# nolan-h-hamilton/ROCCO

Hardware: AMD Instinct MI355X
Metric: loci/sec to converged solve, hg38 50bp K=100; BED3 intervals bit-exact (higher is better)
Workload: dtype f64

## Files before the change

include/rocco_hip.h:

```cpp
#ifndef ROCCO_HIP_H
#define ROCCO_HIP_H

#include <stddef.h>
#include <stdint.h>

#ifdef __cplusplus
extern "C" {
#endif

#define ROCCO_HIP_OK 0
#define ROCCO_HIP_ENOMEM (-1)
#define ROCCO_HIP_EINVAL (-2)
#define ROCCO_HIP_EHIP (-3)

#define ROCCO_HIP_PATH_CERTIFIED 1
#define ROCCO_HIP_PATH_EXACT 2
#define ROCCO_HIP_PATH_TRIVIAL 3
#define ROCCO_HIP_PATH_SPINE 4

typedef struct rocco_hip_solver rocco_hip_solver;

int rocco_hip_abi_version(void);

const char *rocco_hip_last_error(void);

int rocco_hip_solver_create(rocco_hip_solver **solver_out, int device);
void rocco_hip_solver_destroy(rocco_hip_solver *solver);

int rocco_hip_solver_set(rocco_hip_solver *solver, const char *key, long long value);

int rocco_hip_score_median(rocco_hip_solver *solver, const void *matrix_dev, int dtype, size_t K,
                           size_t n, size_t row_stride, double *scores_dev, void *stream);

int rocco_hip_score_median_batch(rocco_hip_solver *solver, const void *const *matrices_dev, int dtype, size_t K,
                                 const size_t *n, const size_t *row_strides, double *const *scores_dev, size_t count,
                                 void *stream);

int rocco_hip_score_median_batch_stats(rocco_hip_solver *solver, const void *const *matrices_dev, int dtype, size_t K,
                                       const size_t *n, const size_t *row_strides, double *const *scores_dev,
                                       size_t count, double *stats_dev, void *stream);

int rocco_hip_score_order_statistic(rocco_hip_solver *solver, const void *matrix_dev, int dtype, size_t K, size_t n,
                                    size_t row_stride, int rank, double *scores_dev, void *stream);
int rocco_hip_score_mean(rocco_hip_solver *solver, const void *matrix_dev, int dtype, size_t K, size_t n,
                         size_t row_stride, double *scores_dev, void *stream);

int rocco_hip_score_trimmed_mean(rocco_hip_solver *solver, const void *matrix_dev, int dtype, size_t K, size_t n,
                                 size_t row_stride, int rank_lo, int rank_hi, double *scores_dev, void *stream);

int rocco_hip_power_f64(rocco_hip_solver *solver, const double *x_dev, double power, double *out_dev, size_t n, void *stream);

int rocco_hip_score_mad(rocco_hip_solver *solver, const void *matrix_dev, int dtype, size_t K, size_t n, size_t row_stride,
                        double *scores_dev, void *stream);

int rocco_hip_score_percentile_range(rocco_hip_solver *solver, const void *matrix_dev, int dtype, size_t K, size_t n,
                                     size_t row_stride, int index_lo, double g_lo, int index_hi, double g_hi,
                                     double *scores_dev, void *stream);

int rocco_hip_score_std(rocco_hip_solver *solver, const void *matrix_dev, int dtype, size_t K, size_t n, size_t row_stride,
                        int pairwise_order, double *scores_dev, void *stream);

int rocco_hip_score_trimmed_std(rocco_hip_solver *solver, const void *matrix_dev, int dtype, size_t K, size_t n,
                                size_t row_stride, int rank_lo, int rank_hi, int take_root, double *scores_dev, void *stream);

int rocco_hip_solve_penalized_chain_f64(rocco_hip_solver *solver, const double *scores_dev,
                                        const double *switch_costs_dev, double gamma, size_t n,
                                        double selection_penalty, uint8_t *solution_dev,
                                        double *value_out, long long *count_out, int *path_out,
                                        void *stream);

typedef struct {
    const double *scores_dev;
    const double *switch_costs_dev;
    double gamma;
    size_t n;
    long long target_count;
    double sum_costs;
    int max_iter;
    uint8_t *solution_dev;
} rocco_hip_budget_task;

typedef struct {
    double selection_penalty;
    double penalized_value;
    long long selected_count;
    int evaluations;
    int path;
    int passes;
    int zone_iters;
    long long n_diff;
    int maps;
} rocco_hip_budget_result;

int rocco_hip_solve_budget_batch_f64(rocco_hip_solver *solver, size_t n_tasks,
                                     const rocco_hip_budget_task *tasks,
                                     rocco_hip_budget_result *results, void *stream);

int rocco_hip_solve_budget_batch_stats_f64(rocco_hip_solver *solver, size_t n_tasks,
                                           const rocco_hip_budget_task *tasks, const double *score_stats_host,
                                           rocco_hip_budget_result *results, void *stream);

typedef struct {
    long long count;
    long long uncertain;
    long long effect;
    long long max_run;
} rocco_hip_probe_stats;

int rocco_hip_delta_probe_f64(rocco_hip_solver *solver, const double *scores_dev,
                              const double *switch_costs_dev, double gamma, size_t n,
                              const uint8_t *emap_dev, const double *lambdas, size_t n_lambdas,
                              rocco_hip_probe_stats *stats_out, void *stream);

int rocco_hip_delta_build_map_f64(rocco_hip_solver *solver, const double *scores_dev,
                                  const double *switch_costs_dev, double gamma, size_t n,
                                  double lambda_ref, double margin, uint8_t *emap_dev, void *stream);

int rocco_hip_delta_build_map_lean_f64(rocco_hip_solver *solver, const double *scores_dev, double gamma, size_t n,
                                       double lambda_ref, double margin, uint8_t *emap_dev, void *stream);

typedef struct {
    long long count_lo, count_hi;
    long long n_diff;
    int diff_adjacent;
    int overflow;
    long long max_run;
    long long diff_locus[16];
    double diff_margin_lo[16], diff_margin_hi[16];
    long long diff_run[16];
    int diff_cls_lo[16], diff_cls_hi[16];
} rocco_hip_window_stats;

int rocco_hip_delta_window_f64(rocco_hip_solver *solver, const double *scores_dev,
                               const double *switch_costs_dev, double gamma, size_t n,
                               const uint8_t *emap_dev, double lambda_lo, double lambda_hi,
                               uint8_t *solution_dev, rocco_hip_window_stats *stats_out, void *stream);

int rocco_hip_delta_model_lean_f64(rocco_hip_solver *solver, const double *scores_dev, double gamma, size_t n,
                                   const uint8_t *emap_dev, const double *lambdas, size_t n_lambdas,
                                   long long *counts_out, long long *open_out, void *stream);

int rocco_hip_delta_bound_rounds_f64(rocco_hip_solver *solver, const double *scores_dev, double gamma, size_t n,
                                     const double *lambdas, const int *round_sizes, int n_rounds,
                                     double *lambdas_used_out, long long *counts_out, long long *level_len_out,
                                     void *stream);

int rocco_hip_delta_spine_f64(rocco_hip_solver *solver, const double *scores_dev,
                              const double *switch_costs_dev, double gamma, size_t n,
                              const uint8_t *emap_dev, const double *lambdas, size_t n_lambdas,
                              int solution_index, uint8_t *solution_dev, long long *counts_out,
                              void *stream);

int rocco_hip_objective_value_f64(rocco_hip_solver *solver, const uint8_t *solution_dev,
                                  const double *scores_dev, const double *switch_costs_dev,
                                  double gamma, size_t n, double *objective_out, void *stream);

int rocco_hip_decode_runs(rocco_hip_solver *solver, const uint8_t *solution_dev, size_t n,
                          int64_t *run_begin_dev, int64_t *run_end_dev, size_t capacity,
                          size_t *n_runs_out, void *stream);

int rocco_hip_decode_runs_table(rocco_hip_solver *solver, size_t count, const uint8_t *const *solutions_dev, const size_t *n,
                                const long long *units, int64_t *table_dev, size_t capacity_rows, size_t eager_rows,
                                size_t *row_offsets_out, const int64_t **table_host_out, void *stream);
int rocco_hip_decode_runs_batch(rocco_hip_solver *solver, size_t count, const uint8_t *const *solutions_dev, const size_t *n,
                                int64_t *const *run_begin_dev, int64_t *const *run_end_dev, const size_t *capacities,
                                size_t *n_runs_out, void *stream);

int rocco_hip_crossfit_whittaker_baseline_matrix_f64(rocco_hip_solver *solver, const double *matrix_dev,
                                                     size_t rows, size_t cols, double penalty_lambda,
                                                     double *baseline_out_dev, void *stream);
int rocco_hip_crossfit_whittaker_baseline_batch_f64(rocco_hip_solver *solver, size_t count, const double *const *matrices_dev,
                                                    const size_t *rows, const size_t *cols, double penalty_lambda,
                                                    double *const *baselines_dev, void *stream);
int rocco_hip_crossfit_whittaker_residual_batch_f64(rocco_hip_solver *solver, size_t count, const double *const *matrices_dev,
                                                    const double *const *row_offsets_dev, const size_t *rows, const size_t *cols,
                                                    double penalty_lambda, double *const *centered_out_dev, void *stream);

size_t rocco_hip_whittaker_batch_scratch_bytes(size_t count, const size_t *rows, const size_t *cols);
int rocco_hip_crossfit_whittaker_residual_batch_scratch_f64(rocco_hip_solver *solver, size_t count, const double *const *matrices_dev,
                                                            const double *const *row_offsets_dev, const size_t *rows,
                                                            const size_t *cols, double penalty_lambda, double *const *centered_out_dev,
                                                            void *scratch_dev, size_t scratch_bytes, void *stream);

int rocco_hip_score_centered_wls_f64(rocco_hip_solver *solver, const double *centered_dev, size_t K, size_t n,
                                     double lower_bound_z, double prior_df, double min_effect, int use_min_effect,
                                     int spatial_window, double precision_floor_ratio, double *mean_dev,
                                     double *raw_var_dev, double *prior_var_dev, double *mod_var_dev, double *se_dev,
                                     double *scores_dev, double *df_out, int *window_out, void *stream);
int rocco_hip_wls_rolling_variances_batch_f64(rocco_hip_solver *solver, size_t count, const double *const *centered_dev,
                                              const size_t *K, const size_t *n, int spatial_window, double *const *variances_dev,
                                              void *stream);
int rocco_hip_score_centered_wls_given_variances_f64(rocco_hip_solver *solver, const double *centered_dev, size_t K, size_t n,
                                                     double lower_bound_z, double prior_df, double min_effect, int use_min_effect,
                                                     int spatial_window, double precision_floor_ratio, const double *variances_dev,
                                                     double *mean_dev, double *raw_var_dev, double *prior_var_dev, double *mod_var_dev,
                                                     double *se_dev, double *scores_dev, double *df_out, int *window_out, void *stream);

int rocco_hip_log2_selfcheck(rocco_hip_solver *solver, int family, unsigned long long seed, unsigned long long first, size_t count,
                             unsigned long long *mismatches_out, void *stream);

int rocco_hip_wls_sorted_rows(const rocco_hip_solver *solver);

int rocco_hip_log_scale_f64(rocco_hip_solver *solver, const double *values_dev, size_t count, double pseudocount, double *out_dev,
                            void *stream);

int rocco_hip_log_scale_center_rows_f64(rocco_hip_solver *solver, const double *counts_dev, size_t K, size_t n,
                                        double pseudocount, int apply_log2, double *centered_out_dev,
                                        double *row_offsets_out_dev, void *stream);

int rocco_hip_log_scale_row_offsets_f64(rocco_hip_solver *solver, const double *counts_dev, size_t K, size_t n,
                                        double pseudocount, int apply_log2, double *log_out_dev, double *row_offsets_out_dev,
                                        void *stream);

int rocco_hip_subtract_f64(rocco_hip_solver *solver, const double *a_dev, const double *b_dev, double *out_dev,
                           size_t count, void *stream);
int rocco_hip_subtract_finite_f64(rocco_hip_solver *solver, const double *a_dev, const double *b_dev, double *out_dev,
                                  size_t count, void *stream);

int rocco_hip_narrowpeak_summit_offsets(rocco_hip_solver *solver, const int64_t *intervals_dev, size_t n_intervals,
                                        const int64_t *centers_dev, const double *effect_mean_dev, size_t n_mean, const int64_t *peak_start_dev,
                                        const int64_t *peak_end_dev, size_t n_peaks, int64_t *offsets_out_dev,
                                        void *stream);

int rocco_hip_union_intervals(rocco_hip_solver *solver, const int64_t *values_dev, size_t count,
                              int64_t *unique_out_dev, size_t *n_unique_out, int *fixed_step_out, void *stream);
int rocco_hip_scatter_tracks(rocco_hip_solver *solver, const int64_t *common_dev, size_t m,
                             const int64_t *intervals_concat_dev, const double *vals_concat_dev,
                             const size_t *offsets_host, size_t K, int out_dtype, void *matrix_out_dev, void *stream);

int rocco_hip_numpy_sum_f64(rocco_hip_solver *solver, const double *x_dev, size_t n, double *sum_out, void *stream);
int rocco_hip_budget_null_draw_stats_f64(rocco_hip_solver *solver, const double *scores_dev, size_t n,
                                         double null_center, double null_soft_scale, double null_threshold,
                                         double *stats_out, void *stream);
int rocco_hip_multiply_f64(rocco_hip_solver *solver, const double *a_dev, const double *b_dev, double *out_dev,
                           size_t count, void *stream);
int rocco_hip_subtract_positive_row_f64(rocco_hip_solver *solver, const double *matrix_dev, const double *row_dev,
                                        size_t K, size_t n, double *out_dev, void *stream);

int rocco_hip_count_path_reserve(rocco_hip_solver *solver, size_t count, const size_t *rows, const size_t *cols,
                                 double penalty_lambda, void *stream);
int rocco_hip_count_path_reserve_ex(rocco_hip_solver *solver, size_t count, const size_t *rows, const size_t *cols,
                                    double penalty_lambda, int sweeps_scratch_is_the_callers, void *stream);
long long rocco_hip_buffer_growths(void);
long long rocco_hip_whittaker_seam_repairs(void);
long long rocco_hip_solver_device_bytes(const rocco_hip_solver *solver);
void rocco_hip_model_chain_counters(long long out[4]);
void rocco_hip_model_chain_written_counters(long long out[2]);

int rocco_hip_pcg64_standard_normal_f64(rocco_hip_solver *solver, unsigned long long state_hi, unsigned long long state_lo,
                                        unsigned long long inc_hi, unsigned long long inc_lo, size_t count, double *values_dev,
                                        unsigned long long *raw_draws_out, void *stream);
int rocco_hip_bartlett_multipliers_f64(rocco_hip_solver *solver, const double *innovations_dev, size_t rows, size_t n,
                                       const double *taps_host, size_t n_taps, double *weights_dev, int *degenerate_out,
                                       void *stream);

int rocco_hip_sort_f64(rocco_hip_solver *solver, const double *x_dev, size_t n, double *sorted_out_dev, void *stream);
int rocco_hip_sorted_probe_f64(rocco_hip_solver *solver, const double *sorted_dev, size_t n, const long long *ranks,
                               size_t n_ranks, double *values_out, double shift, const double *thresholds,
                               size_t n_thresholds, long long *counts_le_out, long long *counts_lt_out, void *stream);
int rocco_hip_autocovariance_sums_f64(rocco_hip_solver *solver, const double *x_dev, size_t n, double mean, int max_lag,
                                      double *sums_out, void *stream);
int rocco_hip_negative_part_f64(rocco_hip_solver *solver, const double *scores_dev, double *out_dev, size_t n, void *stream);
int rocco_hip_soft_counts_f64(rocco_hip_solver *solver, const double *scores_dev, double center, double scale, double *out_dev,
                              size_t n, void *stream);

int rocco_hip_peak_signal_stat_f64(rocco_hip_solver *solver, const double *counts_dev, const double *lengths_dev, size_t n_peaks,
                                   size_t n_samples, double row_scale, double pc, double percentile, double *stat_out_dev, void *stream);
int rocco_hip_ecdf_survival_f64(rocco_hip_solver *solver, const double *stat_dev, const int *bin_dev, const double *null_values_dev,
                                const long long *null_offsets_dev, size_t n_peaks, double *pvals_out_dev, void *stream);
int rocco_hip_bh_adjust_f64(rocco_hip_solver *solver, const double *pvals_dev, size_t m, double *qvals_out_dev, void *stream);

int rocco_hip_select_ranks_batch_f64(rocco_hip_solver *solver, size_t count, const double *const *vectors_dev, const size_t *n,
                                     size_t n_ranks, const long long *ranks, int mode, const double *centers,
                                     double *values_out_dev, long long *counts_out_dev, void *stream);
int rocco_hip_bh_last_passing_rank_f64(rocco_hip_solver *solver, const double *sorted_dev, size_t m, double fdr,
                                       long long *rank_out_dev, void *stream);
int rocco_hip_threshold_mask_f64(rocco_hip_solver *solver, const double *x_dev, size_t n, double divisor, double threshold,
                                 double floor_value, int use_floor, uint8_t *mask_out_dev, void *stream);
int rocco_hip_at_most_mask_f64(rocco_hip_solver *solver, const double *x_dev, size_t n, double cutoff, uint8_t *mask_out_dev,
                               void *stream);
int rocco_hip_divide_finite_f64(rocco_hip_solver *solver, const double *x_dev, size_t n, double divisor, double *out_dev,
                                void *stream);

int rocco_hip_bigwig_dense_fill_f64(rocco_hip_solver *solver, const int64_t *starts_dev, const int64_t *ends_dev,
                                    const double *vals_dev, size_t count, double const_scale, int round_digits,
                                    double *full_out_dev, size_t capacity, int64_t *first_start_out, int64_t *step_out,
                                    size_t *n_full_out, int *flags_out, void *stream);

typedef struct rocco_hip_count_options {
    int32_t flag_include, flag_exclude, min_mapq, read_length, extend_bp, paired_end_mode, min_template_length,
        max_insert_size, shift_fwd, shift_rev, one_read_per_bin;
} rocco_hip_count_options;
typedef struct rocco_hip_count_region {
    int32_t start, end, step, n_bins;
} rocco_hip_count_region;
#define ROCCO_COUNT_CHUNK_RECORDS 512
#define ROCCO_COUNT_MAX_GRID 512
#define ROCCO_COUNT_SCAN_TILE 2048
#define ROCCO_COUNT_WINDOW_BINS 1024
int rocco_hip_count_alignment_records_batch(rocco_hip_solver *solver, const int32_t *pos_dev, const int32_t *end_dev,
                                            const int32_t *isize_dev, const uint16_t *flag_dev, const uint8_t *mapq_dev,
                                            const uint8_t *mate_same_dev, const int64_t *rec_offsets_host, size_t K,
                                            const rocco_hip_count_options *options_host,
                                            const rocco_hip_count_region *regions_host, const int64_t *out_offsets_host,
                                            int accumulate, float *out_dev, int64_t *max_magnitude_out_host, void *stream);
void rocco_hip_count_alignment_shape(int *shape_out);
int rocco_hip_alignment_chrom_range(rocco_hip_solver *solver, const int32_t *pos_dev, const int32_t *end_dev,
                                    const uint16_t *flag_dev, size_t n, int64_t chrom_len, int flag_exclude,
                                    int64_t *start_out, int64_t *end_out, void *stream);
int rocco_hip_alignment_count_tail_f64(rocco_hip_solver *solver, const float *counts_dev, size_t n, double norm_scale,
                                       int scale_by_step, double step, double const_scale, int round_digits,
                                       double *vals_out_dev, int64_t *first_out, int64_t *last_out, void *stream);

#define ROCCO_TRACK_MATRIX_THREADS 256
#define ROCCO_TRACK_MATRIX_UNIT 1024
#define ROCCO_TRACK_MATRIX_MAX_GRID 2048
#define ROCCO_TRACK_MATRIX_ROW_WORDS 6
int rocco_hip_alignment_chrom_range_batch(rocco_hip_solver *solver, const int32_t *pos_dev, const int32_t *end_dev,
                                          const uint16_t *flag_dev, const int64_t *rec_offsets_host, size_t K, int64_t chrom_len,
                                          int flag_exclude, int64_t *range_out_host, void *stream);
int rocco_hip_track_supports(rocco_hip_solver *solver, const int32_t *pos_dev, const int32_t *end_dev, const int32_t *isize_dev,
                             const uint16_t *flag_dev, const uint8_t *mapq_dev, const uint8_t *mate_same_dev,
                             const int64_t *rec_offsets_host, size_t K, const rocco_hip_count_options *options_host,
                             const rocco_hip_count_region *regions_host, const int64_t *out_offsets_host,
                             const double *norm_scale_host, int scale_by_step, double step, double const_scale, float *out_dev,
                             int64_t *max_magnitude_out_host, int64_t *support_out_host, void *stream);
int rocco_hip_track_matrix_fill(rocco_hip_solver *solver, const float *counts_dev, size_t counts_len, const int64_t *rows_dev,
                                size_t n_rows, const int64_t *segs_dev, size_t n_segs, size_t m, int scale_by_step, double step,
                                double const_scale, int round_digits, int out_dtype, void *matrix_out_dev, void *stream);
void rocco_hip_track_matrix_shape(int *out);

#define ROCCO_COUNT_INTERVALS_UNIT 256
#define ROCCO_COUNT_INTERVALS_MAX_GRID 1024
#define ROCCO_COUNT_INTERVALS_WAVES_PER_GROUP 4
int rocco_hip_count_alignment_intervals_batch(rocco_hip_solver *solver, const int32_t *pos_dev, const int32_t *end_dev,
                                              const int32_t *isize_dev, const uint16_t *flag_dev, const uint8_t *mapq_dev,
                                              const uint8_t *mate_same_dev, const int64_t *rec_offsets_host, size_t F, size_t C,
                                              const rocco_hip_count_options *options_host, const int32_t *contig_id_dev,
                                              const int32_t *start_dev, const int32_t *end_region_dev, size_t P, int32_t *out_dev,
                                              int32_t *track_facts_out_host, void *stream);
void rocco_hip_count_intervals_shape(int *shape_out);

#define ROCCO_FRAGMENT_THREADS 256
#define ROCCO_FRAGMENT_DENSITY_RECORDS 2048
#define ROCCO_FRAGMENT_DENSITY_WINDOW 2048
#define ROCCO_FRAGMENT_MAX_BLOCK_SIZE 20224
int rocco_hip_record_flag_facts(rocco_hip_solver *solver, const int32_t *pos_dev, const uint16_t *flag_dev,
                                const int64_t *rec_offsets_host, size_t T, int64_t *mapped_out_host, int32_t *unsorted_out_host,
                                void *stream);
int rocco_hip_fragment_block_centers(rocco_hip_solver *solver, const int32_t *pos_dev, const uint16_t *flag_dev,
                                     const int64_t *rec_offsets_host, size_t T, const int64_t *contig_len_host, int flag_exclude,
                                     int max_iterations, int block_size, int rolling_chunk_size, int32_t *centers_out_host,
                                     int32_t *center_count_out_host, const int64_t *chunk_offsets_host, int32_t *density_out_dev,
                                     int32_t *rank_out_dev, void *stream);
int rocco_hip_strand_xcorr_blocks(rocco_hip_solver *solver, const int32_t *pos_dev, const int32_t *end_dev, const uint16_t *flag_dev,
                                  const int64_t *rec_offsets_host, size_t T, const int32_t *block_track_host,
                                  const int64_t *block_start_host, size_t n_blocks, const int32_t *min_lag_host, int flag_exclude,
                                  int block_size, int max_insert_size, int lag_step, int32_t *best_lag_out_host,
                                  double *best_score_out_host, int32_t *fwd_sum_out_host, int32_t *rev_sum_out_host, void *stream);
int rocco_hip_template_lengths(rocco_hip_solver *solver, const int32_t *isize_dev, const uint16_t *flag_dev, const uint8_t *mate_same_dev,
                               const int64_t *rec_offsets_host, size_t T, const int32_t *min_insert_host, int flag_exclude,
                               int max_insert_size, int32_t *lengths_tmp_dev, int32_t *lengths_out_dev, int64_t *count_out_host,
                               void *stream);
void rocco_hip_fragment_length_shape(int *shape_out);

#define ROCCO_BAM_GUESS_DEPTH 3
#define ROCCO_BAM_SEGMENT_BYTES 16384
#define ROCCO_BAM_RUNOFF_BYTES 65536
#define ROCCO_BAM_THREADS 256
#define ROCCO_BAM_WALK_REPORT 8
#define ROCCO_BAM_ERR_BLOCK_SIZE 1
#define ROCCO_BAM_ERR_TRUNCATED 2
#define ROCCO_BAM_ERR_SIZES 3
#define ROCCO_BAM_ERR_READ_NAME 4
#define ROCCO_BAM_ERR_REF_ID 5
#define ROCCO_BAM_ERR_CIGAR_SEQ 6
#define ROCCO_BAM_ERR_POSITION 7
#define ROCCO_BAM_ERR_END 8
#define ROCCO_BAM_ERR_CG_TAG 9
#define ROCCO_BAM_ERR_ORDER 10
#define ROCCO_BAM_ERR_OFFSET 11
int rocco_hip_bam_walk_records(rocco_hip_solver *solver, const uint8_t *bytes_dev, size_t n_bytes, int64_t entry0, int n_ref,
                               size_t segment_bytes, int guess_mode, int64_t *offsets_out_dev, size_t capacity,
                               int64_t *segment_entry_out_dev, int64_t *report_out_host, void *stream);
int rocco_hip_bam_record_fields(rocco_hip_solver *solver, const uint8_t *bytes_dev, size_t n_bytes, const int64_t *offsets_dev, size_t n,
                                int n_ref, int32_t *tid_out_dev, int32_t *pos_out_dev, int32_t *end_out_dev, int32_t *isize_out_dev,
                                uint16_t *flag_out_dev, uint8_t *mapq_out_dev, uint8_t *mate_same_out_dev, int32_t *qlen_out_dev,
                                int64_t *contig_first_out_host, int64_t *report_out_host, void *stream);
void rocco_hip_bam_shape(int *shape_out);

#define ROCCO_BGZF_THREADS 64
#define ROCCO_BGZF_TABLE_COLUMNS 5
#define ROCCO_BGZF_MAX_ISIZE 65536
#define ROCCO_BGZF_REPORT 4
#define ROCCO_BGZF_STREAM_REASONS 12
#define ROCCO_BGZF_ERR_STREAM 1
#define ROCCO_BGZF_ERR_LENGTH 2
#define ROCCO_BGZF_ERR_CRC 3
#define ROCCO_BGZF_ERR_TABLE 4
#define ROCCO_BGZF_MAX_GRID (1 << 20)
// ... 29 lines not shown
```

rocco_amd/_native.py:

```python
from __future__ import annotations

import contextlib
import ctypes
import os
import threading
from typing import Optional

_HERE = os.path.dirname(os.path.abspath(__file__))
LIB_PATH = os.environ.get("ROCCO_HIP_LIBRARY") or os.path.join(_HERE, "librocco_hip.so")

OK, ENOMEM, EINVAL, EHIP = 0, -1, -2, -3
PATH_CERTIFIED, PATH_EXACT, PATH_TRIVIAL, PATH_SPINE = 1, 2, 3, 4

c_double_p = ctypes.POINTER(ctypes.c_double)
c_ll_p = ctypes.POINTER(ctypes.c_longlong)
c_int_p = ctypes.POINTER(ctypes.c_int)
c_size_p = ctypes.POINTER(ctypes.c_size_t)


class BudgetTask(ctypes.Structure):
    _fields_ = [
        ("scores_dev", ctypes.c_void_p),
        ("switch_costs_dev", ctypes.c_void_p),
        ("gamma", ctypes.c_double),
        ("n", ctypes.c_size_t),
        ("target_count", ctypes.c_longlong),
        ("sum_costs", ctypes.c_double),
        ("max_iter", ctypes.c_int),
        ("solution_dev", ctypes.c_void_p),
    ]


class BudgetResult(ctypes.Structure):
    _fields_ = [
        ("selection_penalty", ctypes.c_double),
        ("penalized_value", ctypes.c_double),
        ("selected_count", ctypes.c_longlong),
        ("evaluations", ctypes.c_int),
        ("path", ctypes.c_int),
        ("passes", ctypes.c_int),
        ("zone_iters", ctypes.c_int),
        ("n_diff", ctypes.c_longlong),
        ("maps", ctypes.c_int),
    ]


class ProbeStats(ctypes.Structure):
    _fields_ = [
        ("count", ctypes.c_longlong),
        ("uncertain", ctypes.c_longlong),
        ("effect", ctypes.c_longlong),
        ("max_run", ctypes.c_longlong),
    ]


class WindowStats(ctypes.Structure):
    _fields_ = [
        ("count_lo", ctypes.c_longlong),
        ("count_hi", ctypes.c_longlong),
        ("n_diff", ctypes.c_longlong),
        ("diff_adjacent", ctypes.c_int),
        ("overflow", ctypes.c_int),
        ("max_run", ctypes.c_longlong),
        ("diff_locus", ctypes.c_longlong * 16),
        ("diff_margin_lo", ctypes.c_double * 16),
        ("diff_margin_hi", ctypes.c_double * 16),
        ("diff_run", ctypes.c_longlong * 16),
        ("diff_cls_lo", ctypes.c_int * 16),
        ("diff_cls_hi", ctypes.c_int * 16),
    ]


PROTOTYPES = [
    ("rocco_hip_abi_version", ctypes.c_int, []),
    ("rocco_hip_last_error", ctypes.c_char_p, []),
    ("rocco_hip_solver_create", ctypes.c_int, [ctypes.POINTER(ctypes.c_void_p), ctypes.c_int]),
    ("rocco_hip_solver_destroy", None, [ctypes.c_void_p]),
    ("rocco_hip_solver_set", ctypes.c_int, [ctypes.c_void_p, ctypes.c_char_p, ctypes.c_longlong]),
    ("rocco_hip_score_trimmed_mean", ctypes.c_int,
     [ctypes.c_void_p, ctypes.c_void_p, ctypes.c_int, ctypes.c_size_t, ctypes.c_size_t, ctypes.c_size_t, ctypes.c_int, ctypes.c_int,
      ctypes.c_void_p, ctypes.c_void_p]),
    ("rocco_hip_power_f64", ctypes.c_int,
     [ctypes.c_void_p, ctypes.c_void_p, ctypes.c_double, ctypes.c_void_p, ctypes.c_size_t, ctypes.c_void_p]),
    ("rocco_hip_score_median_batch", ctypes.c_int,
     [ctypes.c_void_p, ctypes.POINTER(ctypes.c_void_p), ctypes.c_int, ctypes.c_size_t, c_size_p, c_size_p,
      ctypes.POINTER(ctypes.c_void_p), ctypes.c_size_t, ctypes.c_void_p]),
    ("rocco_hip_score_median_batch_stats", ctypes.c_int,
     [ctypes.c_void_p, ctypes.POINTER(ctypes.c_void_p), ctypes.c_int, ctypes.c_size_t, c_size_p, c_size_p,
      ctypes.POINTER(ctypes.c_void_p), ctypes.c_size_t, ctypes.c_void_p, ctypes.c_void_p]),
    ("rocco_hip_score_median", ctypes.c_int,
     [ctypes.c_void_p, ctypes.c_void_p, ctypes.c_int, ctypes.c_size_t, ctypes.c_size_t, ctypes.c_size_t,
      ctypes.c_void_p, ctypes.c_void_p]),
    ("rocco_hip_score_order_statistic", ctypes.c_int,
     [ctypes.c_void_p, ctypes.c_void_p, ctypes.c_int, ctypes.c_size_t, ctypes.c_size_t, ctypes.c_size_t, ctypes.c_int,
      ctypes.c_void_p, ctypes.c_void_p]),
    ("rocco_hip_score_mean", ctypes.c_int,
     [ctypes.c_void_p, ctypes.c_void_p, ctypes.c_int, ctypes.c_size_t, ctypes.c_size_t, ctypes.c_size_t,
      ctypes.c_void_p, ctypes.c_void_p]),
    ("rocco_hip_score_mad", ctypes.c_int,
     [ctypes.c_void_p, ctypes.c_void_p, ctypes.c_int, ctypes.c_size_t, ctypes.c_size_t, ctypes.c_size_t,
      ctypes.c_void_p, ctypes.c_void_p]),
    ("rocco_hip_score_percentile_range", ctypes.c_int,
     [ctypes.c_void_p, ctypes.c_void_p, ctypes.c_int, ctypes.c_size_t, ctypes.c_size_t, ctypes.c_size_t, ctypes.c_int,
      ctypes.c_double, ctypes.c_int, ctypes.c_double, ctypes.c_void_p, ctypes.c_void_p]),
    ("rocco_hip_score_std", ctypes.c_int,
     [ctypes.c_void_p, ctypes.c_void_p, ctypes.c_int, ctypes.c_size_t, ctypes.c_size_t, ctypes.c_size_t, ctypes.c_int,
      ctypes.c_void_p, ctypes.c_void_p]),
    ("rocco_hip_score_trimmed_std", ctypes.c_int,
     [ctypes.c_void_p, ctypes.c_void_p, ctypes.c_int, ctypes.c_size_t, ctypes.c_size_t, ctypes.c_size_t, ctypes.c_int, ctypes.c_int,
      ctypes.c_int, ctypes.c_void_p, ctypes.c_void_p]),
    ("rocco_hip_solve_penalized_chain_f64", ctypes.c_int,
     [ctypes.c_void_p, ctypes.c_void_p, ctypes.c_void_p, ctypes.c_double, ctypes.c_size_t,
      ctypes.c_double, ctypes.c_void_p, c_double_p, c_ll_p, c_int_p, ctypes.c_void_p]),
    ("rocco_hip_solve_budget_batch_f64", ctypes.c_int,
     [ctypes.c_void_p, ctypes.c_size_t, ctypes.POINTER(BudgetTask), ctypes.POINTER(BudgetResult),
      ctypes.c_void_p]),
    ("rocco_hip_solve_budget_batch_stats_f64", ctypes.c_int,
     [ctypes.c_void_p, ctypes.c_size_t, ctypes.POINTER(BudgetTask), ctypes.c_void_p, ctypes.POINTER(BudgetResult),
      ctypes.c_void_p]),
    ("rocco_hip_delta_model_lean_f64", ctypes.c_int,
     [ctypes.c_void_p, ctypes.c_void_p, ctypes.c_double, ctypes.c_size_t, ctypes.c_void_p, c_double_p, ctypes.c_size_t,
      c_ll_p, c_ll_p, ctypes.c_void_p]),
    ("rocco_hip_delta_probe_f64", ctypes.c_int,
     [ctypes.c_void_p, ctypes.c_void_p, ctypes.c_void_p, ctypes.c_double, ctypes.c_size_t, ctypes.c_void_p,
      c_double_p, ctypes.c_size_t, ctypes.POINTER(ProbeStats), ctypes.c_void_p]),
    ("rocco_hip_delta_build_map_f64", ctypes.c_int,
     [ctypes.c_void_p, ctypes.c_void_p, ctypes.c_void_p, ctypes.c_double, ctypes.c_size_t,
      ctypes.c_double, ctypes.c_double, ctypes.c_void_p, ctypes.c_void_p]),
    ("rocco_hip_delta_build_map_lean_f64", ctypes.c_int,
     [ctypes.c_void_p, ctypes.c_void_p, ctypes.c_double, ctypes.c_size_t, ctypes.c_double, ctypes.c_double, ctypes.c_void_p,
      ctypes.c_void_p]),
    ("rocco_hip_delta_bound_rounds_f64", ctypes.c_int,
     [ctypes.c_void_p, ctypes.c_void_p, ctypes.c_double, ctypes.c_size_t, c_double_p, c_int_p, ctypes.c_int,
      c_double_p, c_ll_p, c_ll_p, ctypes.c_void_p]),
    ("rocco_hip_delta_spine_f64", ctypes.c_int,
     [ctypes.c_void_p, ctypes.c_void_p, ctypes.c_void_p, ctypes.c_double, ctypes.c_size_t, ctypes.c_void_p,
      c_double_p, ctypes.c_size_t, ctypes.c_int, ctypes.c_void_p, c_ll_p, ctypes.c_void_p]),
    ("rocco_hip_delta_window_f64", ctypes.c_int,
     [ctypes.c_void_p, ctypes.c_void_p, ctypes.c_void_p, ctypes.c_double, ctypes.c_size_t, ctypes.c_void_p,
      ctypes.c_double, ctypes.c_double, ctypes.c_void_p, ctypes.POINTER(WindowStats), ctypes.c_void_p]),
    ("rocco_hip_objective_value_f64", ctypes.c_int,
     [ctypes.c_void_p, ctypes.c_void_p, ctypes.c_void_p, ctypes.c_void_p, ctypes.c_double,
      ctypes.c_size_t, c_double_p, ctypes.c_void_p]),
    ("rocco_hip_sort_f64", ctypes.c_int, [ctypes.c_void_p, ctypes.c_void_p, ctypes.c_size_t, ctypes.c_void_p, ctypes.c_void_p]),
    ("rocco_hip_sorted_probe_f64", ctypes.c_int,
     [ctypes.c_void_p, ctypes.c_void_p, ctypes.c_size_t, c_ll_p, ctypes.c_size_t, c_double_p, ctypes.c_double, c_double_p,
      ctypes.c_size_t, c_ll_p, c_ll_p, ctypes.c_void_p]),
    ("rocco_hip_select_ranks_batch_f64", ctypes.c_int,
     [ctypes.c_void_p, ctypes.c_size_t, ctypes.POINTER(ctypes.c_void_p), c_size_p, ctypes.c_size_t, c_ll_p, ctypes.c_int, c_double_p,
      ctypes.c_void_p, ctypes.c_void_p, ctypes.c_void_p]),
    ("rocco_hip_bh_last_passing_rank_f64", ctypes.c_int,
     [ctypes.c_void_p, ctypes.c_void_p, ctypes.c_size_t, ctypes.c_double, ctypes.c_void_p, ctypes.c_void_p]),
    ("rocco_hip_threshold_mask_f64", ctypes.c_int,
     [ctypes.c_void_p, ctypes.c_void_p, ctypes.c_size_t, ctypes.c_double, ctypes.c_double, ctypes.c_double, ctypes.c_int,
      ctypes.c_void_p, ctypes.c_void_p]),
    ("rocco_hip_at_most_mask_f64", ctypes.c_int,
     [ctypes.c_void_p, ctypes.c_void_p, ctypes.c_size_t, ctypes.c_double, ctypes.c_void_p, ctypes.c_void_p]),
    ("rocco_hip_divide_finite_f64", ctypes.c_int,
     [ctypes.c_void_p, ctypes.c_void_p, ctypes.c_size_t, ctypes.c_double, ctypes.c_void_p, ctypes.c_void_p]),
    ("rocco_hip_autocovariance_sums_f64", ctypes.c_int,
     [ctypes.c_void_p, ctypes.c_void_p, ctypes.c_size_t, ctypes.c_double, ctypes.c_int, c_double_p, ctypes.c_void_p]),
    ("rocco_hip_negative_part_f64", ctypes.c_int, [ctypes.c_void_p, ctypes.c_void_p, ctypes.c_void_p, ctypes.c_size_t, ctypes.c_void_p]),
    ("rocco_hip_soft_counts_f64", ctypes.c_int,
     [ctypes.c_void_p, ctypes.c_void_p, ctypes.c_double, ctypes.c_double, ctypes.c_void_p, ctypes.c_size_t, ctypes.c_void_p]),
    ("rocco_hip_peak_signal_stat_f64", ctypes.c_int,
     [ctypes.c_void_p, ctypes.c_void_p, ctypes.c_void_p, ctypes.c_size_t, ctypes.c_size_t, ctypes.c_double, ctypes.c_double,
      ctypes.c_double, ctypes.c_void_p, ctypes.c_void_p]),
    ("rocco_hip_ecdf_survival_f64", ctypes.c_int,
     [ctypes.c_void_p, ctypes.c_void_p, ctypes.c_void_p, ctypes.c_void_p, ctypes.c_void_p, ctypes.c_size_t, ctypes.c_void_p,
      ctypes.c_void_p]),
    ("rocco_hip_bh_adjust_f64", ctypes.c_int, [ctypes.c_void_p, ctypes.c_void_p, ctypes.c_size_t, ctypes.c_void_p, ctypes.c_void_p]),
    ("rocco_hip_log_scale_f64", ctypes.c_int,
     [ctypes.c_void_p, ctypes.c_void_p, ctypes.c_size_t, ctypes.c_double, ctypes.c_void_p, ctypes.c_void_p]),
    ("rocco_hip_decode_runs_table", ctypes.c_int,
     [ctypes.c_void_p, ctypes.c_size_t, ctypes.POINTER(ctypes.c_void_p), c_size_p, c_ll_p, ctypes.c_void_p, ctypes.c_size_t,
      ctypes.c_size_t, c_size_p, ctypes.POINTER(ctypes.c_void_p), ctypes.c_void_p]),
    ("rocco_hip_decode_runs_batch", ctypes.c_int,
     [ctypes.c_void_p, ctypes.c_size_t, ctypes.POINTER(ctypes.c_void_p), c_size_p, ctypes.POINTER(ctypes.c_void_p),
      ctypes.POINTER(ctypes.c_void_p), c_size_p, c_size_p, ctypes.c_void_p]),
    ("rocco_hip_decode_runs", ctypes.c_int,
     [ctypes.c_void_p, ctypes.c_void_p, ctypes.c_size_t, ctypes.c_void_p, ctypes.c_void_p,
      ctypes.c_size_t, c_size_p, ctypes.c_void_p]),
    ("rocco_hip_crossfit_whittaker_baseline_batch_f64", ctypes.c_int,
     [ctypes.c_void_p, ctypes.c_size_t, ctypes.POINTER(ctypes.c_void_p), c_size_p, c_size_p, ctypes.c_double,
      ctypes.POINTER(ctypes.c_void_p), ctypes.c_void_p]),
    ("rocco_hip_crossfit_whittaker_residual_batch_f64", ctypes.c_int,
     [ctypes.c_void_p, ctypes.c_size_t, ctypes.POINTER(ctypes.c_void_p), ctypes.POINTER(ctypes.c_void_p), c_size_p, c_size_p,
      ctypes.c_double, ctypes.POINTER(ctypes.c_void_p), ctypes.c_void_p]),
    ("rocco_hip_crossfit_whittaker_baseline_matrix_f64", ctypes.c_int,
     [ctypes.c_void_p, ctypes.c_void_p, ctypes.c_size_t, ctypes.c_size_t, ctypes.c_double, ctypes.c_void_p,
      ctypes.c_void_p]),
    ("rocco_hip_score_centered_wls_f64", ctypes.c_int,
     [ctypes.c_void_p, ctypes.c_void_p, ctypes.c_size_t, ctypes.c_size_t, ctypes.c_double, ctypes.c_double,
      ctypes.c_double, ctypes.c_int, ctypes.c_int, ctypes.c_double, ctypes.c_void_p, ctypes.c_void_p,
      ctypes.c_void_p, ctypes.c_void_p, ctypes.c_void_p, ctypes.c_void_p, c_double_p, c_int_p, ctypes.c_void_p]),
    ("rocco_hip_wls_rolling_variances_batch_f64", ctypes.c_int,
     [ctypes.c_void_p, ctypes.c_size_t, ctypes.POINTER(ctypes.c_void_p), c_size_p, c_size_p, ctypes.c_int,
      ctypes.POINTER(ctypes.c_void_p), ctypes.c_void_p]),
    ("rocco_hip_score_centered_wls_given_variances_f64", ctypes.c_int,
     [ctypes.c_void_p, ctypes.c_void_p, ctypes.c_size_t, ctypes.c_size_t, ctypes.c_double, ctypes.c_double,
      ctypes.c_double, ctypes.c_int, ctypes.c_int, ctypes.c_double, ctypes.c_void_p, ctypes.c_void_p, ctypes.c_void_p,
      ctypes.c_void_p, ctypes.c_void_p, ctypes.c_void_p, ctypes.c_void_p, c_double_p, c_int_p, ctypes.c_void_p]),
    ("rocco_hip_log_scale_center_rows_f64", ctypes.c_int,
     [ctypes.c_void_p, ctypes.c_void_p, ctypes.c_size_t, ctypes.c_size_t, ctypes.c_double, ctypes.c_int,
      ctypes.c_void_p, ctypes.c_void_p, ctypes.c_void_p]),
    ("rocco_hip_log_scale_row_offsets_f64", ctypes.c_int,
     [ctypes.c_void_p, ctypes.c_void_p, ctypes.c_size_t, ctypes.c_size_t, ctypes.c_double, ctypes.c_int,
      ctypes.c_void_p, ctypes.c_void_p, ctypes.c_void_p]),
    ("rocco_hip_wls_sorted_rows", ctypes.c_int, [ctypes.c_void_p]),
    ("rocco_hip_log2_selfcheck", ctypes.c_int,
     [ctypes.c_void_p, ctypes.c_int, ctypes.c_uint64, ctypes.c_uint64, ctypes.c_size_t, ctypes.POINTER(ctypes.c_uint64), ctypes.c_void_p]),
    ("rocco_hip_subtract_finite_f64", ctypes.c_int,
     [ctypes.c_void_p, ctypes.c_void_p, ctypes.c_void_p, ctypes.c_void_p, ctypes.c_size_t, ctypes.c_void_p]),
    ("rocco_hip_subtract_f64", ctypes.c_int,
     [ctypes.c_void_p, ctypes.c_void_p, ctypes.c_void_p, ctypes.c_void_p, ctypes.c_size_t, ctypes.c_void_p]),
    ("rocco_hip_narrowpeak_summit_offsets", ctypes.c_int,
     [ctypes.c_void_p, ctypes.c_void_p, ctypes.c_size_t, ctypes.c_void_p, ctypes.c_void_p, ctypes.c_size_t,
      ctypes.c_void_p, ctypes.c_void_p, ctypes.c_size_t, ctypes.c_void_p, ctypes.c_void_p]),
    ("rocco_hip_union_intervals", ctypes.c_int,
     [ctypes.c_void_p, ctypes.c_void_p, ctypes.c_size_t, ctypes.c_void_p, c_size_p, c_int_p, ctypes.c_void_p]),
    ("rocco_hip_scatter_tracks", ctypes.c_int,
     [ctypes.c_void_p, ctypes.c_void_p, ctypes.c_size_t, ctypes.c_void_p, ctypes.c_void_p, c_size_p, ctypes.c_size_t,
      ctypes.c_int, ctypes.c_void_p, ctypes.c_void_p]),
    ("rocco_hip_numpy_sum_f64", ctypes.c_int,
     [ctypes.c_void_p, ctypes.c_void_p, ctypes.c_size_t, c_double_p, ctypes.c_void_p]),
    ("rocco_hip_budget_null_draw_stats_f64", ctypes.c_int,
     [ctypes.c_void_p, ctypes.c_void_p, ctypes.c_size_t, ctypes.c_double, ctypes.c_double, ctypes.c_double,
      c_double_p, ctypes.c_void_p]),
    ("rocco_hip_count_path_reserve", ctypes.c_int,
     [ctypes.c_void_p, ctypes.c_size_t, ctypes.POINTER(ctypes.c_size_t), ctypes.POINTER(ctypes.c_size_t), ctypes.c_double,
      ctypes.c_void_p]),
    ("rocco_hip_count_path_reserve_ex", ctypes.c_int,
     [ctypes.c_void_p, ctypes.c_size_t, ctypes.POINTER(ctypes.c_size_t), ctypes.POINTER(ctypes.c_size_t), ctypes.c_double,
      ctypes.c_int, ctypes.c_void_p]),
    ("rocco_hip_whittaker_batch_scratch_bytes", ctypes.c_size_t, [ctypes.c_size_t, c_size_p, c_size_p]),
    ("rocco_hip_crossfit_whittaker_residual_batch_scratch_f64", ctypes.c_int,
     [ctypes.c_void_p, ctypes.c_size_t, ctypes.POINTER(ctypes.c_void_p), ctypes.POINTER(ctypes.c_void_p), c_size_p, c_size_p,
      ctypes.c_double, ctypes.POINTER(ctypes.c_void_p), ctypes.c_void_p, ctypes.c_size_t, ctypes.c_void_p]),
    ("rocco_hip_buffer_growths", ctypes.c_longlong, []),
    ("rocco_hip_whittaker_seam_repairs", ctypes.c_longlong, []),
    ("rocco_hip_model_chain_counters", None, [ctypes.POINTER(ctypes.c_longlong)]),
    ("rocco_hip_model_chain_written_counters", None, [ctypes.POINTER(ctypes.c_longlong)]),
    ("rocco_hip_solver_device_bytes", ctypes.c_longlong, [ctypes.c_void_p]),
    ("rocco_hip_pcg64_standard_normal_f64", ctypes.c_int,
     [ctypes.c_void_p, ctypes.c_ulonglong, ctypes.c_ulonglong, ctypes.c_ulonglong, ctypes.c_ulonglong, ctypes.c_size_t,
      ctypes.c_void_p, ctypes.POINTER(ctypes.c_ulonglong), ctypes.c_void_p]),
    ("rocco_hip_bartlett_multipliers_f64", ctypes.c_int,
     [ctypes.c_void_p, ctypes.c_void_p, ctypes.c_size_t, ctypes.c_size_t, c_double_p, ctypes.c_size_t, ctypes.c_void_p,
      ctypes.POINTER(ctypes.c_int), ctypes.c_void_p]),
    ("rocco_hip_multiply_f64", ctypes.c_int,
     [ctypes.c_void_p, ctypes.c_void_p, ctypes.c_void_p, ctypes.c_void_p, ctypes.c_size_t, ctypes.c_void_p]),
    ("rocco_hip_subtract_positive_row_f64", ctypes.c_int,
     [ctypes.c_void_p, ctypes.c_void_p, ctypes.c_void_p, ctypes.c_size_t, ctypes.c_size_t, ctypes.c_void_p,
      ctypes.c_void_p]),
    ("rocco_hip_bigwig_dense_fill_f64", ctypes.c_int,
     [ctypes.c_void_p, ctypes.c_void_p, ctypes.c_void_p, ctypes.c_void_p, ctypes.c_size_t, ctypes.c_double, ctypes.c_int,
      ctypes.c_void_p, ctypes.c_size_t, c_ll_p, c_ll_p, c_size_p, c_int_p, ctypes.c_void_p]),
    ("rocco_hip_count_alignment_records_batch", ctypes.c_int,
     [ctypes.c_void_p, ctypes.c_void_p, ctypes.c_void_p, ctypes.c_void_p, ctypes.c_void_p, ctypes.c_void_p, ctypes.c_void_p,
      c_ll_p, ctypes.c_size_t, ctypes.c_void_p, ctypes.c_void_p, c_ll_p, ctypes.c_int, ctypes.c_void_p, c_ll_p,
      ctypes.c_void_p]),
    ("rocco_hip_count_alignment_shape", None, [c_int_p]),
    ("rocco_hip_alignment_chrom_range", ctypes.c_int,
     [ctypes.c_void_p, ctypes.c_void_p, ctypes.c_void_p, ctypes.c_void_p, ctypes.c_size_t, ctypes.c_longlong, ctypes.c_int,
      c_ll_p, c_ll_p, ctypes.c_void_p]),
    ("rocco_hip_alignment_count_tail_f64", ctypes.c_int,
     [ctypes.c_void_p, ctypes.c_void_p, ctypes.c_size_t, ctypes.c_double, ctypes.c_int, ctypes.c_double, ctypes.c_double,
      ctypes.c_int, ctypes.c_void_p, c_ll_p, c_ll_p, ctypes.c_void_p]),
    ("rocco_hip_alignment_chrom_range_batch", ctypes.c_int,
     [ctypes.c_void_p, ctypes.c_void_p, ctypes.c_void_p, ctypes.c_void_p, c_ll_p, ctypes.c_size_t, ctypes.c_longlong, ctypes.c_int,
      c_ll_p, ctypes.c_void_p]),
    ("rocco_hip_track_supports", ctypes.c_int,
     [ctypes.c_void_p, ctypes.c_void_p, ctypes.c_void_p, ctypes.c_void_p, ctypes.c_void_p, ctypes.c_void_p, ctypes.c_void_p,
      c_ll_p, ctypes.c_size_t, ctypes.c_void_p, ctypes.c_void_p, c_ll_p, ctypes.POINTER(ctypes.c_double), ctypes.c_int,
      ctypes.c_double, ctypes.c_double, ctypes.c_void_p, c_ll_p, c_ll_p, ctypes.c_void_p]),
    ("rocco_hip_track_matrix_fill", ctypes.c_int,
     [ctypes.c_void_p, ctypes.c_void_p, ctypes.c_size_t, ctypes.c_void_p, ctypes.c_size_t, ctypes.c_void_p, ctypes.c_size_t,
      ctypes.c_size_t, ctypes.c_int, ctypes.c_double, ctypes.c_double, ctypes.c_int, ctypes.c_int, ctypes.c_void_p, ctypes.c_void_p]),
    ("rocco_hip_track_matrix_shape", None, [c_int_p]),
    ("rocco_hip_count_alignment_intervals_batch", ctypes.c_int,
     [ctypes.c_void_p, ctypes.c_void_p, ctypes.c_void_p, ctypes.c_void_p, ctypes.c_void_p, ctypes.c_void_p, ctypes.c_void_p,
      c_ll_p, ctypes.c_size_t, ctypes.c_size_t, ctypes.c_void_p, ctypes.c_void_p, ctypes.c_void_p, ctypes.c_void_p,
      ctypes.c_size_t, ctypes.c_void_p, c_int_p, ctypes.c_void_p]),
    ("rocco_hip_count_intervals_shape", None, [c_int_p]),
    ("rocco_hip_record_flag_facts", ctypes.c_int,
     [ctypes.c_void_p, ctypes.c_void_p, ctypes.c_void_p, c_ll_p, ctypes.c_size_t, c_ll_p, c_int_p, ctypes.c_void_p]),
    ("rocco_hip_fragment_block_centers", ctypes.c_int,
     [ctypes.c_void_p, ctypes.c_void_p, ctypes.c_void_p, c_ll_p, ctypes.c_size_t, c_ll_p, ctypes.c_int, ctypes.c_int, ctypes.c_int,
      ctypes.c_int, c_int_p, c_int_p, c_ll_p, ctypes.c_void_p, ctypes.c_void_p, ctypes.c_void_p]),
    ("rocco_hip_strand_xcorr_blocks", ctypes.c_int,
     [ctypes.c_void_p, ctypes.c_void_p, ctypes.c_void_p, ctypes.c_void_p, c_ll_p, ctypes.c_size_t, c_int_p, c_ll_p, ctypes.c_size_t,
      c_int_p, ctypes.c_int, ctypes.c_int, ctypes.c_int, ctypes.c_int, c_int_p, c_double_p, c_int_p, c_int_p, ctypes.c_void_p]),
    ("rocco_hip_template_lengths", ctypes.c_int,
     [ctypes.c_void_p, ctypes.c_void_p, ctypes.c_void_p, ctypes.c_void_p, c_ll_p, ctypes.c_size_t, c_int_p, ctypes.c_int, ctypes.c_int,
      ctypes.c_void_p, ctypes.c_void_p, c_ll_p, ctypes.c_void_p]),
    ("rocco_hip_fragment_length_shape", None, [c_int_p]),
    ("rocco_hip_bam_walk_records", ctypes.c_int,
     [ctypes.c_void_p, ctypes.c_void_p, ctypes.c_size_t, ctypes.c_longlong, ctypes.c_int, ctypes.c_size_t, ctypes.c_int, ctypes.c_void_p,
      ctypes.c_size_t, ctypes.c_void_p, c_ll_p, ctypes.c_void_p]),
    ("rocco_hip_bam_record_fields", ctypes.c_int,
     [ctypes.c_void_p, ctypes.c_void_p, ctypes.c_size_t, ctypes.c_void_p, ctypes.c_size_t, ctypes.c_int, ctypes.c_void_p, ctypes.c_void_p,
      ctypes.c_void_p, ctypes.c_void_p, ctypes.c_void_p, ctypes.c_void_p, ctypes.c_void_p, ctypes.c_void_p, c_ll_p, c_ll_p,
      ctypes.c_void_p]),
    ("rocco_hip_bam_shape", None, [c_int_p]),
    ("rocco_hip_bgzf_inflate", ctypes.c_int,
     [ctypes.c_void_p, ctypes.c_void_p, ctypes.c_size_t, ctypes.c_void_p, ctypes.c_size_t, ctypes.c_void_p, ctypes.c_size_t,
      ctypes.c_void_p, c_ll_p, ctypes.c_void_p]),
    ("rocco_hip_bgzf_inflate_host", ctypes.c_int,
     [ctypes.c_void_p, ctypes.c_void_p, ctypes.c_size_t, ctypes.c_void_p, ctypes.c_size_t, ctypes.c_void_p, ctypes.c_size_t,
      ctypes.c_void_p, c_ll_p]),
    ("rocco_hip_bgzf_shape", None, [c_int_p]),
    ("rocco_hip_launch_caps", None, [c_int_p]),
    ("rocco_hip_synth_matrix", ctypes.c_int,
     [ctypes.c_void_p, ctypes.c_void_p, ctypes.c_int, ctypes.c_size_t, ctypes.c_size_t,
      ctypes.c_size_t, ctypes.c_uint64, ctypes.c_void_p]),
]

LAUNCH_CAP_NAMES = (
    "select_grid_target", "select_chunk_values", "select_threads", "bh_max_grid", "bh_threads", "chrom_range_max_grid",
    "count_tail_max_grid", "count_threads", "interval_facts_max_grid", "count_intervals_threads", "fragment_max_grid",
    "fragment_threads", "fragment_density_records", "fragment_density_window", "bam_max_grid", "bam_threads")

class _Library:

    def __init__(self, cdll: ctypes.CDLL):
        object.__setattr__(self, "_cdll", cdll)
        object.__setattr__(self, "_wrapped", {})

    def __getattr__(self, name):
        wrapped = self._wrapped.get(name)
        if wrapped is not None:
            return wrapped
        fn = getattr(self._cdll, name)
        if getattr(fn, "restype", None) is not ctypes.c_int:
            self._wrapped[name] = fn
            return fn

        def call(*args, _fn=fn):
            rc = _fn(*args)
            if rc == ENOMEM:
                import torch

                if torch.cuda.is_available():
                    torch.cuda.synchronize()
                    torch.cuda.empty_cache()
                    rc = _fn(*args)
            return rc

        call.__name__ = name
        self._wrapped[name] = call
        return call


_lib: Optional[_Library] = None


def load() -> _Library:
    global _lib
    if _lib is not None:
        return _lib
    import torch

    if not os.path.isfile(LIB_PATH):
        raise RuntimeError(
            "Make sure native HIP extension is built and available "
            f"({LIB_PATH} missing; run `python -c 'import __graft_entry__ as g; g.build()'`)")
    try:
        lib = ctypes.CDLL(LIB_PATH)
    except OSError as exc:
        raise RuntimeError(f"Make sure native HIP extension is built and available: {exc}") from exc
    for name, restype, argtypes in PROTOTYPES:
        fn = getattr(lib, name)
        fn.restype = restype
        fn.argtypes = argtypes
    _lib = _Library(lib)
    return _lib


def launch_caps() -> dict:
    caps = (ctypes.c_int * len(LAUNCH_CAP_NAMES))()
    load().rocco_hip_launch_caps(caps)
    return {name: int(value) for name, value in zip(LAUNCH_CAP_NAMES, caps)}


def last_error() -> str:
    msg = load().rocco_hip_last_error()
    return msg.decode("utf-8", "replace") if msg else ""


def check(rc: int, what: str) -> None:
    if rc == OK:
        return
    if rc == ENOMEM:
        raise MemoryError(f"{what}: device/host allocation failed ({last_error()})")
    if rc == EINVAL:
# ... 67 lines not shown
```

rocco_amd/csrc/api.hip:

```cpp
#include <map>
#include <memory>
#include <mutex>
#include "kernels.h"
#include <atomic>

#include "budget.h"

#include <algorithm>
#include <cmath>
#include <new>

namespace rocco {

static thread_local std::string g_last_error;

void set_last_error(const std::string &msg) { g_last_error = msg; }

static std::atomic<long long> g_buffer_growths{0};

int DeviceBuffer::reserve(size_t want)
{
    if (want <= bytes) {
        return ROCCO_HIP_OK;
    }
// ... 208 lines not shown
                           size_t n, size_t row_stride, double *scores_dev, void *stream)
{
    if (solver == nullptr || matrix_dev == nullptr || scores_dev == nullptr || K == 0 ||
        row_stride < n || (dtype != 0 && dtype != 1)) {
        return ROCCO_HIP_EINVAL;
    }
    ROCCO_HIP_TRY(hipSetDevice(solver->device)); (void)hipGetLastError();
    return launch_median(matrix_dev, dtype, K, n, row_stride, scores_dev, (hipStream_t)stream);
}

int rocco_hip_score_order_statistic(rocco_hip_solver *solver, const void *matrix_dev, int dtype, size_t K, size_t n,
                                    size_t row_stride, int rank, double *scores_dev, void *stream)
{
    if (solver == nullptr || (n > 0 && (matrix_dev == nullptr || scores_dev == nullptr)) || K == 0 || row_stride < n ||
        (dtype != 0 && dtype != 1) || rank < 0 || (size_t)rank >= K) {
        return ROCCO_HIP_EINVAL;
    }
    ROCCO_HIP_TRY(hipSetDevice(solver->device)); (void)hipGetLastError();
    return launch_order_statistic(matrix_dev, dtype, K, n, row_stride, rank, scores_dev, (hipStream_t)stream);
}

int rocco_hip_score_trimmed_mean(rocco_hip_solver *solver, const void *matrix_dev, int dtype, size_t K, size_t n,
                                 size_t row_stride, int rank_lo, int rank_hi, double *scores_dev, void *stream)
{
    if (solver == nullptr || matrix_dev == nullptr || scores_dev == nullptr || K == 0 || row_stride < n ||
        (dtype != 0 && dtype != 1) || rank_lo < 0 || rank_hi < rank_lo || rank_hi >= (int)K) {
        return ROCCO_HIP_EINVAL;
    }
    ROCCO_HIP_TRY(hipSetDevice(solver->device)); (void)hipGetLastError();
    return launch_trimmed_mean(matrix_dev, dtype, K, n, row_stride, rank_lo, rank_hi, scores_dev, (hipStream_t)stream);
}

int rocco_hip_power_f64(rocco_hip_solver *solver, const double *x_dev, double power, double *out_dev, size_t n, void *stream)
{
    if (solver == nullptr || (n > 0 && (x_dev == nullptr || out_dev == nullptr))) {
        return ROCCO_HIP_EINVAL;
    }
    ROCCO_HIP_TRY(hipSetDevice(solver->device)); (void)hipGetLastError();
    return launch_power(x_dev, power, out_dev, n, (hipStream_t)stream);
}

int rocco_hip_score_mean(rocco_hip_solver *solver, const void *matrix_dev, int dtype, size_t K, size_t n,
                         size_t row_stride, double *scores_dev, void *stream)
{
    if (solver == nullptr || (n > 0 && (matrix_dev == nullptr || scores_dev == nullptr)) || K == 0 || row_stride < n ||
        (dtype != 0 && dtype != 1)) {
        return ROCCO_HIP_EINVAL;
    }
    ROCCO_HIP_TRY(hipSetDevice(solver->device)); (void)hipGetLastError();
    return launch_column_mean(matrix_dev, dtype, K, n, row_stride, scores_dev, (hipStream_t)stream);
}

static bool dispersion_args_ok(const rocco_hip_solver *solver, const void *matrix_dev, int dtype, size_t K, size_t n, size_t row_stride,
                               const double *scores_dev)
{
    return solver != nullptr && (n == 0 || (matrix_dev != nullptr && scores_dev != nullptr)) && K >= 2 && K <= 0x7FFFFFFF &&
           row_stride >= n && (dtype == 0 || dtype == 1);
}

int rocco_hip_score_mad(rocco_hip_solver *solver, const void *matrix_dev, int dtype, size_t K, size_t n, size_t row_stride,
                        double *scores_dev, void *stream)
{
    if (!dispersion_args_ok(solver, matrix_dev, dtype, K, n, row_stride, scores_dev)) {
        return ROCCO_HIP_EINVAL;
    }
    ROCCO_HIP_TRY(hipSetDevice(solver->device)); (void)hipGetLastError();
    return launch_mad(matrix_dev, dtype, K, n, row_stride, scores_dev, (hipStream_t)stream);
}

int rocco_hip_score_percentile_range(rocco_hip_solver *solver, const void *matrix_dev, int dtype, size_t K, size_t n,
                                     size_t row_stride, int index_lo, double g_lo, int index_hi, double g_hi,
                                     double *scores_dev, void *stream)
{
    if (!dispersion_args_ok(solver, matrix_dev, dtype, K, n, row_stride, scores_dev) || index_lo < 0 || index_hi < 0 ||
        (size_t)index_lo >= K || (size_t)index_hi >= K || !(g_lo >= 0.0 && g_lo < 1.0) || !(g_hi >= 0.0 && g_hi < 1.0)) {
        return ROCCO_HIP_EINVAL;
    }
    ROCCO_HIP_TRY(hipSetDevice(solver->device)); (void)hipGetLastError();
    return launch_percentile_range(matrix_dev, dtype, K, n, row_stride, index_lo, g_lo, index_hi, g_hi, scores_dev,
                                   (hipStream_t)stream);
}

int rocco_hip_score_std(rocco_hip_solver *solver, const void *matrix_dev, int dtype, size_t K, size_t n, size_t row_stride,
                        int pairwise_order, double *scores_dev, void *stream)
{
    if (!dispersion_args_ok(solver, matrix_dev, dtype, K, n, row_stride, scores_dev)) {
        return ROCCO_HIP_EINVAL;
    }
    ROCCO_HIP_TRY(hipSetDevice(solver->device)); (void)hipGetLastError();
    return launch_std(matrix_dev, dtype, K, n, row_stride, pairwise_order, scores_dev, (hipStream_t)stream);
}

int rocco_hip_score_trimmed_std(rocco_hip_solver *solver, const void *matrix_dev, int dtype, size_t K, size_t n,
                                size_t row_stride, int rank_lo, int rank_hi, int take_root, double *scores_dev, void *stream)
{
    if (!dispersion_args_ok(solver, matrix_dev, dtype, K, n, row_stride, scores_dev) || rank_lo < 0 || rank_hi < rank_lo ||
        (size_t)rank_hi >= K) {
        return ROCCO_HIP_EINVAL;
    }
    ROCCO_HIP_TRY(hipSetDevice(solver->device)); (void)hipGetLastError();
    return launch_trimmed_std(matrix_dev, dtype, K, n, row_stride, rank_lo, rank_hi, take_root, scores_dev, (hipStream_t)stream);
}

int rocco_hip_solve_penalized_chain_f64(rocco_hip_solver *solver, const double *scores_dev,
                                        const double *switch_costs_dev, double gamma, size_t n,
                                        double selection_penalty, uint8_t *solution_dev,
                                        double *value_out, long long *count_out, int *path_out,
                                        void *stream)
{
    if (solver == nullptr || scores_dev == nullptr || n == 0 || n >= ((size_t)1 << 31)) {
        return ROCCO_HIP_EINVAL;
    }
    ROCCO_HIP_TRY(hipSetDevice(solver->device)); (void)hipGetLastError();
    return solve_fixed_penalty(solver, scores_dev, switch_costs_dev, gamma, n, selection_penalty,
                               solution_dev, value_out, count_out, path_out, (hipStream_t)stream);
}

int rocco_hip_solve_budget_batch_f64(rocco_hip_solver *solver, size_t n_tasks,
                                     const rocco_hip_budget_task *tasks,
                                     rocco_hip_budget_result *results, void *stream)
{
    if (solver == nullptr || (n_tasks > 0 && (tasks == nullptr || results == nullptr))) {
        return ROCCO_HIP_EINVAL;
    }
    for (size_t t = 0; t < n_tasks; ++t) {
        if (tasks[t].scores_dev == nullptr || tasks[t].n == 0 || tasks[t].n >= ((size_t)1 << 31) ||
            tasks[t].solution_dev == nullptr || tasks[t].max_iter < 0) {
            return ROCCO_HIP_EINVAL;
        }
    }
    ROCCO_HIP_TRY(hipSetDevice(solver->device)); (void)hipGetLastError();
    return solve_budget_batch(solver, n_tasks, tasks, results, (hipStream_t)stream);
}

int rocco_hip_solve_budget_batch_stats_f64(rocco_hip_solver *solver, size_t n_tasks, const rocco_hip_budget_task *tasks,
                                           const double *score_stats_host, rocco_hip_budget_result *results, void *stream)
{
    if (solver == nullptr || (n_tasks > 0 && (tasks == nullptr || results == nullptr))) {
        return ROCCO_HIP_EINVAL;
    }
    for (size_t t = 0; t < n_tasks; ++t) {
        if (tasks[t].scores_dev == nullptr || tasks[t].n == 0 || tasks[t].n >= ((size_t)1 << 31) ||
            tasks[t].solution_dev == nullptr || tasks[t].max_iter < 0) {
            return ROCCO_HIP_EINVAL;
        }
        if (score_stats_host != nullptr && !(score_stats_host[3 * t] <= score_stats_host[3 * t + 1])) {
            return ROCCO_HIP_EINVAL;
        }
    }
    ROCCO_HIP_TRY(hipSetDevice(solver->device)); (void)hipGetLastError();
    return solve_budget_batch(solver, n_tasks, tasks, results, (hipStream_t)stream, score_stats_host);
}

int rocco_hip_delta_model_lean_f64(rocco_hip_solver *solver, const double *scores_dev, double gamma, size_t n,
                                   const uint8_t *emap_dev, const double *lambdas, size_t n_lambdas, long long *counts_out,
                                   long long *open_out, void *stream)
{
    if (solver == nullptr || scores_dev == nullptr || emap_dev == nullptr || n < 2 || n >= ((size_t)1 << 31) ||
        (n_lambdas > 0 && (lambdas == nullptr || counts_out == nullptr || open_out == nullptr))) {
        return ROCCO_HIP_EINVAL;
    }
    ROCCO_HIP_TRY(hipSetDevice(solver->device)); (void)hipGetLastError();
    return delta_model_lean(solver, scores_dev, gamma, n, emap_dev, lambdas, n_lambdas, counts_out, open_out, (hipStream_t)stream);
}

int rocco_hip_delta_probe_f64(rocco_hip_solver *solver, const double *scores_dev,
                              const double *switch_costs_dev, double gamma, size_t n,
                              const uint8_t *emap_dev, const double *lambdas, size_t n_lambdas,
                              rocco_hip_probe_stats *stats_out, void *stream)
{
    if (solver == nullptr || scores_dev == nullptr || n == 0 || n >= ((size_t)1 << 31) ||
        (n_lambdas > 0 && (lambdas == nullptr || stats_out == nullptr))) {
        return ROCCO_HIP_EINVAL;
    }
    ROCCO_HIP_TRY(hipSetDevice(solver->device)); (void)hipGetLastError();
    return delta_probe(solver, scores_dev, switch_costs_dev, gamma, n, emap_dev, lambdas, n_lambdas,
                       stats_out, (hipStream_t)stream);
}

int rocco_hip_delta_bound_rounds_f64(rocco_hip_solver *solver, const double *scores_dev, double gamma, size_t n,
                                     const double *lambdas, const int *round_sizes, int n_rounds,
                                     double *lambdas_used_out, long long *counts_out, long long *level_len_out,
                                     void *stream)
{
    if (solver == nullptr || scores_dev == nullptr || n < 2 || n >= ((size_t)1 << 31) || n_rounds < 0 ||
        (n_rounds > 0 && (lambdas == nullptr || round_sizes == nullptr || lambdas_used_out == nullptr ||
                          counts_out == nullptr || level_len_out == nullptr))) {
        return ROCCO_HIP_EINVAL;
    }
    ROCCO_HIP_TRY(hipSetDevice(solver->device)); (void)hipGetLastError();
    return delta_bound_rounds(solver, scores_dev, gamma, n, lambdas, round_sizes, n_rounds, lambdas_used_out, counts_out,
                              level_len_out, (hipStream_t)stream);
}

int rocco_hip_delta_spine_f64(rocco_hip_solver *solver, const double *scores_dev,
                              const double *switch_costs_dev, double gamma, size_t n,
                              const uint8_t *emap_dev, const double *lambdas, size_t n_lambdas,
                              int solution_index, uint8_t *solution_dev, long long *counts_out,
                              void *stream)
{
    if (solver == nullptr || scores_dev == nullptr || n == 0 || n >= ((size_t)1 << 31) || emap_dev == nullptr ||
        lambdas == nullptr || counts_out == nullptr || n_lambdas == 0 || n_lambdas > 64 ||
        solution_index >= (int)n_lambdas || (solution_index >= 0 && solution_dev == nullptr)) {
        return ROCCO_HIP_EINVAL;
    }
    ROCCO_HIP_TRY(hipSetDevice(solver->device)); (void)hipGetLastError();
    return delta_spine(solver, scores_dev, switch_costs_dev, gamma, n, emap_dev, lambdas, n_lambdas,
                       solution_index, solution_dev, counts_out, (hipStream_t)stream);
}

int rocco_hip_delta_build_map_f64(rocco_hip_solver *solver, const double *scores_dev,
                                  const double *switch_costs_dev, double gamma, size_t n,
                                  double lambda_ref, double margin, uint8_t *emap_dev, void *stream)
{
    if (solver == nullptr || scores_dev == nullptr || n == 0 || n >= ((size_t)1 << 31) || emap_dev == nullptr ||
        !(margin >= 0.0)) {
        return ROCCO_HIP_EINVAL;
    }
    ROCCO_HIP_TRY(hipSetDevice(solver->device)); (void)hipGetLastError();
    return delta_build_map(solver, scores_dev, switch_costs_dev, gamma, n, lambda_ref, margin, emap_dev,
                           (hipStream_t)stream);
}

int rocco_hip_delta_build_map_lean_f64(rocco_hip_solver *solver, const double *scores_dev, double gamma, size_t n,
                                       double lambda_ref, double margin, uint8_t *emap_dev, void *stream)
{
    if (solver == nullptr || scores_dev == nullptr || n < 2 || n >= ((size_t)1 << 31) || emap_dev == nullptr || !(margin >= 0.0)) {
        return ROCCO_HIP_EINVAL;
    }
    ROCCO_HIP_TRY(hipSetDevice(solver->device)); (void)hipGetLastError();
    return delta_build_map_lean(solver, scores_dev, gamma, n, lambda_ref, margin, emap_dev, (hipStream_t)stream);
}

int rocco_hip_delta_window_f64(rocco_hip_solver *solver, const double *scores_dev,
                               const double *switch_costs_dev, double gamma, size_t n,
                               const uint8_t *emap_dev, double lambda_lo, double lambda_hi,
                               uint8_t *solution_dev, rocco_hip_window_stats *stats_out, void *stream)
{
    if (solver == nullptr || scores_dev == nullptr || n == 0 || n >= ((size_t)1 << 31) ||
        solution_dev == nullptr || stats_out == nullptr || !(lambda_lo <= lambda_hi)) {
        return ROCCO_HIP_EINVAL;
    }
    ROCCO_HIP_TRY(hipSetDevice(solver->device)); (void)hipGetLastError();
    return delta_window(solver, scores_dev, switch_costs_dev, gamma, n, emap_dev, lambda_lo, lambda_hi,
                        solution_dev, stats_out, (hipStream_t)stream);
}

int rocco_hip_objective_value_f64(rocco_hip_solver *solver, const uint8_t *solution_dev,
                                  const double *scores_dev, const double *switch_costs_dev,
                                  double gamma, size_t n, double *objective_out, void *stream)
{
    if (solver == nullptr || objective_out == nullptr || (n > 0 && (solution_dev == nullptr || scores_dev == nullptr))) {
        return ROCCO_HIP_EINVAL;
    }
    ROCCO_HIP_TRY(hipSetDevice(solver->device)); (void)hipGetLastError();
    int rc = solver->dev_misc.reserve(objective_scratch_bytes(n));
    if (rc != ROCCO_HIP_OK) {
        return rc;
    }
    rc = solver->host_back.reserve(64);
    if (rc != ROCCO_HIP_OK) {
        return rc;
    }
    double *back = (double *)solver->host_back.ptr;
    rc = launch_objective(solution_dev, scores_dev, switch_costs_dev, gamma, n, solver->dev_misc.ptr,
                          back, (hipStream_t)stream);
    if (rc == ROCCO_HIP_OK) {
        *objective_out = *back;
    }
    return rc;
}

int rocco_hip_peak_signal_stat_f64(rocco_hip_solver *solver, const double *counts_dev, const double *lengths_dev, size_t n_peaks,
                                   size_t n_samples, double row_scale, double pc, double percentile, double *stat_out_dev, void *stream)
{
    if (solver == nullptr || n_samples == 0 || n_samples > 4096 || !(percentile >= 0.0 && percentile <= 100.0) ||
        (n_peaks > 0 && (counts_dev == nullptr || lengths_dev == nullptr || stat_out_dev == nullptr))) {
        return ROCCO_HIP_EINVAL;
    }
    ROCCO_HIP_TRY(hipSetDevice(solver->device)); (void)hipGetLastError();
    const int rc = solver->dev_misc.reserve(n_peaks * n_samples * sizeof(double) + 256);
    if (rc != ROCCO_HIP_OK) return rc;
    return launch_peak_signal(counts_dev, lengths_dev, n_peaks, n_samples, row_scale, pc, percentile, stat_out_dev, solver->dev_misc.ptr,
                              (hipStream_t)stream);
}

int rocco_hip_ecdf_survival_f64(rocco_hip_solver *solver, const double *stat_dev, const int *bin_dev, const double *null_values_dev,
                                const long long *null_offsets_dev, size_t n_peaks, double *pvals_out_dev, void *stream)
{
    if (solver == nullptr || (n_peaks > 0 && (stat_dev == nullptr || bin_dev == nullptr || null_values_dev == nullptr ||
                                              null_offsets_dev == nullptr || pvals_out_dev == nullptr))) {
        return ROCCO_HIP_EINVAL;
    }
    ROCCO_HIP_TRY(hipSetDevice(solver->device)); (void)hipGetLastError();
    return launch_ecdf_survival(stat_dev, bin_dev, null_values_dev, null_offsets_dev, n_peaks, pvals_out_dev, (hipStream_t)stream);
}

int rocco_hip_bh_adjust_f64(rocco_hip_solver *solver, const double *pvals_dev, size_t m, double *qvals_out_dev, void *stream)
{
    if (solver == nullptr || m >= ((size_t)1 << 31) || (m > 0 && (pvals_dev == nullptr || qvals_out_dev == nullptr))) {
        return ROCCO_HIP_EINVAL;
    }
    ROCCO_HIP_TRY(hipSetDevice(solver->device)); (void)hipGetLastError();
    const int rc = solver->dev_misc.reserve(bh_scratch_bytes(m));
    if (rc != ROCCO_HIP_OK) return rc;
    return launch_bh_adjust(pvals_dev, m, qvals_out_dev, solver->dev_misc.ptr, (hipStream_t)stream);
// ... 359 lines not shown

int whittaker_batch(rocco_hip_solver *solver, size_t count, const double *const *matrices_dev, const double *const *offsets_dev,
                    const size_t *rows, const size_t *cols, double penalty_lambda, double *const *baselines_dev, int residual,
                    void *stream, void *scratch_dev = nullptr, size_t scratch_bytes = 0)
{
    if (solver == nullptr || (count > 0 && (matrices_dev == nullptr || rows == nullptr || cols == nullptr || baselines_dev == nullptr))) {
        return ROCCO_HIP_EINVAL;
    }
    size_t longest = 0;
    for (size_t i = 0; i < count; ++i) {
        if (rows[i] * cols[i] > 0 && (matrices_dev[i] == nullptr || baselines_dev[i] == nullptr || (residual != 0 && baselines_dev[i] == matrices_dev[i]))) {
            return ROCCO_HIP_EINVAL;
        }
        if (rows[i] > 0) {
            longest = std::max(longest, cols[i]);
        }
    }
    ROCCO_HIP_TRY(hipSetDevice(solver->device)); (void)hipGetLastError();
    int rc;
    if (scratch_dev != nullptr) {
        if (scratch_bytes < whittaker_batch_scratch_bytes(rows, cols, count) || ((uintptr_t)scratch_dev & 255u) != 0) {
            set_last_error("the sweeps' scratch block is too small or not aligned to 256 bytes");
            return ROCCO_HIP_EINVAL;
        }
    } else if ((rc = solver->dev_misc.reserve(whittaker_batch_scratch_bytes(rows, cols, count))) != ROCCO_HIP_OK) {
        return rc;
    }
    if ((rc = solver->host_stage.reserve(whittaker_batch_stage_bytes(rows, cols, count))) != ROCCO_HIP_OK) return rc;
    if ((rc = ensure_whittaker_factor(solver, longest, penalty_lambda, (hipStream_t)stream)) != ROCCO_HIP_OK) return rc;
    const rocco::SharedFactor *factor = (longest >= 25) ? solver->factor.get() : nullptr;
    rc = launch_crossfit_whittaker_batch(matrices_dev, rows, cols, count, penalty_lambda,
                                         factor != nullptr ? (const double *)factor->buf.ptr : nullptr,
                                         factor != nullptr ? factor->cap : 0, baselines_dev,
                                         scratch_dev != nullptr ? scratch_dev : solver->dev_misc.ptr,
                                         solver->host_stage.ptr, (hipStream_t)stream, offsets_dev, residual);
    if (rc != ROCCO_HIP_OK) {
        return rc;
    }
    ROCCO_HIP_TRY(hipStreamSynchronize((hipStream_t)stream));
    if (whittaker_collect_repairs(solver->host_stage.ptr) != 0 && residual != 0) {
        set_last_error("Local baseline fit produced non-finite values");
        return ROCCO_HIP_EINVAL;
    }
    return ROCCO_HIP_OK;
}

}

int rocco_hip_crossfit_whittaker_baseline_batch_f64(rocco_hip_solver *solver, size_t count, const double *const *matrices_dev,
                                                    const size_t *rows, const size_t *cols, double penalty_lambda,
                                                    double *const *baselines_dev, void *stream)
{
    return whittaker_batch(solver, count, matrices_dev, nullptr, rows, cols, penalty_lambda, baselines_dev, 0, stream);
}

int rocco_hip_crossfit_whittaker_residual_batch_f64(rocco_hip_solver *solver, size_t count, const double *const *matrices_dev,
                                                    const double *const *row_offsets_dev, const size_t *rows, const size_t *cols,
                                                    double penalty_lambda, double *const *centered_out_dev, void *stream)
{
    return whittaker_batch(solver, count, matrices_dev, row_offsets_dev, rows, cols, penalty_lambda, centered_out_dev, 1, stream);
}

size_t rocco_hip_whittaker_batch_scratch_bytes(size_t count, const size_t *rows, const size_t *cols)
{
    return (rows == nullptr || cols == nullptr) ? 0 : whittaker_batch_scratch_bytes(rows, cols, count);
}

int rocco_hip_crossfit_whittaker_residual_batch_scratch_f64(rocco_hip_solver *solver, size_t count, const double *const *matrices_dev,
                                                            const double *const *row_offsets_dev, const size_t *rows,
                                                            const size_t *cols, double penalty_lambda, double *const *centered_out_dev,
                                                            void *scratch_dev, size_t scratch_bytes, void *stream)
{
    if (scratch_dev == nullptr) {
        return ROCCO_HIP_EINVAL;
    }
    return whittaker_batch(solver, count, matrices_dev, row_offsets_dev, rows, cols, penalty_lambda, centered_out_dev, 1, stream,
                           scratch_dev, scratch_bytes);
}

int rocco_hip_crossfit_whittaker_baseline_matrix_f64(rocco_hip_solver *solver, const double *matrix_dev,
                                                     size_t rows, size_t cols, double penalty_lambda,
                                                     double *baseline_out_dev, void *stream)
{
    if (solver == nullptr || ((matrix_dev == nullptr || baseline_out_dev == nullptr) && rows * cols > 0)) {
        return ROCCO_HIP_EINVAL;
    }
    return rocco_hip_crossfit_whittaker_baseline_batch_f64(solver, 1, &matrix_dev, &rows, &cols, penalty_lambda, &baseline_out_dev,
                                                           stream);
}

int rocco_hip_wls_rolling_variances_batch_f64(rocco_hip_solver *solver, size_t count, const double *const *centered_dev,
                                              const size_t *K, const size_t *n, int spatial_window, double *const *variances_dev,
                                              void *stream)
{
    if (solver == nullptr || (count > 0 && (centered_dev == nullptr || K == nullptr || n == nullptr || variances_dev == nullptr))) {
        return ROCCO_HIP_EINVAL;
    }
    ROCCO_HIP_TRY(hipSetDevice(solver->device)); (void)hipGetLastError();
    size_t rows = 0;
    for (size_t i = 0; i < count; ++i) {
        const int window = wls_spatial_window(n[i], spatial_window);
        if (window > wls_max_window()) {
            set_last_error("rocco_hip_wls_rolling_variances_batch_f64: spatial windows above 63 loci go through the single-matrix call");
            return ROCCO_HIP_EINVAL;
        }
        if (window > 0 && n[i] >= 4) {
            if (centered_dev[i] == nullptr || variances_dev[i] == nullptr) {
                return ROCCO_HIP_EINVAL;
            }
            rows += K[i];
        }
    }
    if (rows == 0) {
        return ROCCO_HIP_OK;
    }
    wls_set_rolling_group_min(solver->rolling_group_min);
    const size_t group = (size_t)wls_rolling_group_rows(rows);
    int rc;
    if ((rc = solver->dev_tasks.reserve(rows * sizeof(WlsRollingTask))) != ROCCO_HIP_OK) return rc;
    if ((rc = solver->host_stage.reserve(rows * sizeof(WlsRollingTask))) != ROCCO_HIP_OK) return rc;
    WlsRollingTask *host = (WlsRollingTask *)solver->host_stage.ptr;
    size_t t = 0;
    for (size_t i = 0; i < count; ++i) {
        const int window = wls_spatial_window(n[i], spatial_window);
        if (window <= 0 || n[i] < 4) {
            continue;
        }
        const size_t stride = n[i] - (size_t)window + 1;
        for (size_t k = 0; k < K[i]; k += group, ++t) {
            host[t].row = centered_dev[i] + k * n[i];
            host[t].n = (long long)n[i];
            host[t].window = window;
            host[t].rows = (int)std::min(group, K[i] - k);
            host[t].out = variances_dev[i] + k * stride;
        }
    }
    ROCCO_HIP_TRY(hipMemcpyAsync(solver->dev_tasks.ptr, host, t * sizeof(WlsRollingTask), hipMemcpyHostToDevice, (hipStream_t)stream));
    if ((rc = launch_wls_rolling_batch((const WlsRollingTask *)solver->dev_tasks.ptr, t, (int)group, (hipStream_t)stream)) != ROCCO_HIP_OK) return rc;
    ROCCO_HIP_TRY(hipStreamSynchronize((hipStream_t)stream));
    return ROCCO_HIP_OK;
}

long long rocco_hip_buffer_growths(void) { return g_buffer_growths.load(std::memory_order_relaxed); }

long long rocco_hip_whittaker_seam_repairs(void) { return whittaker_seam_repairs(); }

void rocco_hip_model_chain_counters(long long out[4])
{
    if (out != nullptr) {
        rocco::model_chain_counters(out);
    }
}

void rocco_hip_model_chain_written_counters(long long out[2])
{
    if (out != nullptr) {
        rocco::model_chain_written_counters(out);
    }
}

long long rocco_hip_solver_device_bytes(const rocco_hip_solver *solver)
{
    if (solver == nullptr) {
        return 0;
    }
    const rocco::DeviceBuffer *all[] = {&solver->dev_tasks, &solver->dev_params, &solver->dev_results, &solver->dev_bits, &solver->dev_misc,
                                        &solver->dev_median_partials, &solver->dev_solution, &solver->dev_maps, &solver->dev_frozen,
                                        &solver->dev_lean_pool, &solver->dev_lean_round, &solver->dev_lean_look, &solver->dev_lean_desc,
                                        &solver->dev_lean_wcap, &solver->dev_chain};
    long long total = 0;
    for (const rocco::DeviceBuffer *b : all) {
        total += (long long)b->bytes;
    }
    return total;
}

int rocco_hip_count_path_reserve(rocco_hip_solver *solver, size_t count, const size_t *rows, const size_t *cols, double penalty_lambda,
                                 void *stream)
{
    return rocco_hip_count_path_reserve_ex(solver, count, rows, cols, penalty_lambda, 0, stream);
}

int rocco_hip_count_path_reserve_ex(rocco_hip_solver *solver, size_t count, const size_t *rows, const size_t *cols, double penalty_lambda,
                                    int sweeps_scratch_is_the_callers, void *stream)
{
    if (solver == nullptr || (count > 0 && (rows == nullptr || cols == nullptr))) {
        return ROCCO_HIP_EINVAL;
    }
    ROCCO_HIP_TRY(hipSetDevice(solver->device)); (void)hipGetLastError();
    size_t misc = (sweeps_scratch_is_the_callers != 0) ? 0 : whittaker_batch_scratch_bytes(rows, cols, count);
    size_t stage_single = 0, total_rows = 0, most_rows = 0, longest = 0;
    for (size_t i = 0; i < count; ++i) {
        if (rows[i] == 0 || cols[i] == 0) {
            continue;
        }
        misc = std::max(misc, wls_scratch_bytes(rows[i], cols[i], 31, true));
        misc = std::max(misc, wls_scratch_bytes(rows[i], cols[i], 31, false));
        misc = std::max(misc, log_scale_scratch_bytes(rows[i], cols[i]));
        if (sweeps_scratch_is_the_callers == 0) {
            misc = std::max(misc, whittaker_batch_scratch_bytes(&rows[i], &cols[i], 1));
        }
        stage_single = std::max(stage_single, whittaker_batch_stage_bytes(&rows[i], &cols[i], 1));
        total_rows += rows[i];
        most_rows = std::max(most_rows, rows[i]);
        longest = std::max(longest, cols[i]);
    }
    int rc;
    if ((rc = solver->dev_misc.reserve(misc)) != ROCCO_HIP_OK) return rc;
    if ((rc = solver->dev_tasks.reserve(total_rows * sizeof(WlsRollingTask) + 256)) != ROCCO_HIP_OK) return rc;
    if ((rc = solver->host_stage.reserve(std::max(std::max(whittaker_batch_stage_bytes(rows, cols, count), stage_single), total_rows * sizeof(WlsRollingTask) + 256))) != ROCCO_HIP_OK) return rc;
    if ((rc = solver->host_back.reserve(256 + most_rows * sizeof(int))) != ROCCO_HIP_OK) return rc;
    if ((rc = solver->dev_results.reserve(256)) != ROCCO_HIP_OK) return rc;
    if (penalty_lambda > 0.0 && (rc = ensure_whittaker_factor(solver, longest, penalty_lambda, (hipStream_t)stream)) != ROCCO_HIP_OK) return rc;
    return ROCCO_HIP_OK;
}

int rocco_hip_score_centered_wls_f64(rocco_hip_solver *solver, const double *centered_dev, size_t K, size_t n,
                                     double lower_bound_z, double prior_df, double min_effect, int use_min_effect,
                                     int spatial_window, double precision_floor_ratio, double *mean_dev,
                                     double *raw_var_dev, double *prior_var_dev, double *mod_var_dev, double *se_dev,
                                     double *scores_dev, double *df_out, int *window_out, void *stream)
{
    return rocco_hip_score_centered_wls_given_variances_f64(solver, centered_dev, K, n, lower_bound_z, prior_df, min_effect,
                                                            use_min_effect, spatial_window, precision_floor_ratio, nullptr, mean_dev,
                                                            raw_var_dev, prior_var_dev, mod_var_dev, se_dev, scores_dev, df_out,
                                                            window_out, stream);
}

int rocco_hip_score_centered_wls_given_variances_f64(rocco_hip_solver *solver, const double *centered_dev, size_t K, size_t n,
                                                     double lower_bound_z, double prior_df, double min_effect, int use_min_effect,
                                                     int spatial_window, double precision_floor_ratio, const double *variances_dev,
                                                     double *mean_dev, double *raw_var_dev, double *prior_var_dev, double *mod_var_dev,
                                                     double *se_dev, double *scores_dev, double *df_out, int *window_out, void *stream)
{
    if (solver == nullptr || centered_dev == nullptr || mean_dev == nullptr || raw_var_dev == nullptr ||
        prior_var_dev == nullptr || mod_var_dev == nullptr || se_dev == nullptr || scores_dev == nullptr || K == 0 ||
        n == 0 || n > (size_t)0x7fffffff) {
        set_last_error("rocco_hip_score_centered_wls_f64: null buffer, empty matrix or more than 2^31-1 loci");
        return ROCCO_HIP_EINVAL;
    }
    ROCCO_HIP_TRY(hipSetDevice(solver->device)); (void)hipGetLastError();
    int rc;
    if ((rc = solver->dev_misc.reserve(wls_scratch_bytes(K, n, spatial_window, variances_dev == nullptr))) != ROCCO_HIP_OK) {
        return rc;
    }
    if ((rc = solver->host_back.reserve(256 + K * sizeof(int))) != ROCCO_HIP_OK) {
        return rc;
    }
    if (variances_dev != nullptr && wls_spatial_window(n, spatial_window) > wls_max_window()) {
        set_last_error("rocco_hip_score_centered_wls_given_variances_f64: windows above 63 loci compute their own variances");
        return ROCCO_HIP_EINVAL;
    }
    wls_set_rolling_group_min(solver->rolling_group_min);
    return launch_score_centered_wls(centered_dev, K, n, lower_bound_z, prior_df, min_effect, use_min_effect,
                                     spatial_window, precision_floor_ratio, mean_dev, raw_var_dev, prior_var_dev,
                                     mod_var_dev, se_dev, scores_dev, solver->dev_misc.ptr, df_out, window_out,
                                     (hipStream_t)stream, (int *)solver->host_back.ptr, variances_dev, &solver->wls_sorted_rows);
}

int rocco_hip_wls_sorted_rows(const rocco_hip_solver *solver) { return solver != nullptr ? solver->wls_sorted_rows : -1; }

int rocco_hip_log2_selfcheck(rocco_hip_solver *solver, int family, unsigned long long seed, unsigned long long first, size_t count,
                             unsigned long long *mismatches_out, void *stream)
{
    if (solver == nullptr || mismatches_out == nullptr || family < 0 || family > 4 || count > ((size_t)1 << 39)) {
        return ROCCO_HIP_EINVAL;
    }
    ROCCO_HIP_TRY(hipSetDevice(solver->device)); (void)hipGetLastError();
    int rc;
    if ((rc = solver->dev_results.reserve(256)) != ROCCO_HIP_OK) return rc;
    if ((rc = solver->host_back.reserve(256)) != ROCCO_HIP_OK) return rc;
    unsigned long long *out = (unsigned long long *)solver->dev_results.ptr;
    ROCCO_HIP_TRY(hipMemsetAsync(out, 0, sizeof(unsigned long long), (hipStream_t)stream));
    if ((rc = launch_log2_selfcheck(family, seed, first, count, out, (hipStream_t)stream)) != ROCCO_HIP_OK) return rc;
    ROCCO_HIP_TRY(hipMemcpyAsync(solver->host_back.ptr, out, sizeof(unsigned long long), hipMemcpyDeviceToHost, (hipStream_t)stream));
    ROCCO_HIP_TRY(hipStreamSynchronize((hipStream_t)stream));
    *mismatches_out = *(unsigned long long *)solver->host_back.ptr;
    return ROCCO_HIP_OK;
}

int rocco_hip_log_scale_f64(rocco_hip_solver *solver, const double *values_dev, size_t count, double pseudocount, double *out_dev,
                            void *stream)
{
    if (solver == nullptr || (count > 0 && (values_dev == nullptr || out_dev == nullptr))) {
        return ROCCO_HIP_EINVAL;
    }
    ROCCO_HIP_TRY(hipSetDevice(solver->device)); (void)hipGetLastError();
    int rc = solver->dev_results.reserve(256);
    if (rc != ROCCO_HIP_OK) return rc;
    int *bad = (int *)solver->dev_results.ptr;
    ROCCO_HIP_TRY(hipMemsetAsync(bad, 0, sizeof(int), (hipStream_t)stream));
    if ((rc = launch_log_scale(values_dev, out_dev, count, pseudocount, bad, (hipStream_t)stream)) != ROCCO_HIP_OK) return rc;
    if ((rc = solver->host_back.reserve(256)) != ROCCO_HIP_OK) return rc;
    int &bad_host = *(int *)solver->host_back.ptr;
    bad_host = 0;
    ROCCO_HIP_TRY(hipMemcpyAsync(&bad_host, bad, sizeof(int), hipMemcpyDeviceToHost, (hipStream_t)stream));
    ROCCO_HIP_TRY(hipStreamSynchronize((hipStream_t)stream));
    if (bad_host != 0) {
        set_last_error("`chrom_matrix` contains non-finite values");
        return ROCCO_HIP_EINVAL;
    }
    return ROCCO_HIP_OK;
}

int rocco_hip_log_scale_center_rows_f64(rocco_hip_solver *solver, const double *counts_dev, size_t K, size_t n,
                                        double pseudocount, int apply_log2, double *centered_out_dev,
// ... 571 lines not shown
```

rocco_amd/csrc/budget.h:

```cpp
#pragma once

#include "kernels.h"

namespace rocco {

int solve_fixed_penalty(rocco_hip_solver *solver, const double *scores_dev,
                        const double *switch_costs_dev, double gamma, size_t n, double lambda,
                        uint8_t *solution_dev, double *value_out, long long *count_out, int *path_out,
                        hipStream_t stream);

int solve_budget_batch(rocco_hip_solver *solver, size_t n_tasks, const rocco_hip_budget_task *tasks,
                       rocco_hip_budget_result *results, hipStream_t stream, const double *score_stats_host = nullptr);

}

namespace rocco {

int delta_probe(rocco_hip_solver *solver, const double *scores_dev, const double *switch_costs_dev,
                double gamma, size_t n, const uint8_t *emap_dev, const double *lambdas, size_t n_lambdas,
                rocco_hip_probe_stats *stats_out, hipStream_t stream);

int delta_spine(rocco_hip_solver *solver, const double *scores_dev, const double *switch_costs_dev,
                double gamma, size_t n, const uint8_t *emap_dev, const double *lambdas, size_t n_lambdas,
                int solution_index, uint8_t *solution_dev, long long *counts_out, hipStream_t stream);

int delta_build_map(rocco_hip_solver *solver, const double *scores_dev, const double *switch_costs_dev,
                    double gamma, size_t n, double lambda_ref, double margin, uint8_t *emap_dev,
                    hipStream_t stream);

int delta_bound_rounds(rocco_hip_solver *solver, const double *scores_dev, double gamma, size_t n,
                       const double *lambdas, const int *round_sizes, int n_rounds, double *lambdas_used_out,
                       long long *counts_out, long long *level_len_out, hipStream_t stream);

int delta_window(rocco_hip_solver *solver, const double *scores_dev, const double *switch_costs_dev,
                 double gamma, size_t n, const uint8_t *emap_dev, double lambda_lo, double lambda_hi,
                 uint8_t *solution_dev, rocco_hip_window_stats *stats_out, hipStream_t stream);

int delta_model_lean(rocco_hip_solver *solver, const double *scores_dev, double gamma, size_t n, const uint8_t *emap_dev,
                     const double *lambdas, size_t n_lambdas, long long *counts_out, long long *open_out, hipStream_t stream);

int delta_build_map_lean(rocco_hip_solver *solver, const double *scores_dev, double gamma, size_t n, double lambda_ref,
                         double margin, uint8_t *emap_dev, hipStream_t stream);

void model_chain_counters(long long out[4]);
void model_chain_written_counters(long long out[2]);

}
```

rocco_amd/csrc/budget.hip:

```cpp
#include "budget.h"

#include <algorithm>
#include <atomic>
#include <chrono>
#include <cmath>
#include <cstdio>
#include <cstdlib>
#include <cstring>
#include <thread>

#include "chain.h"
#include "model_chain.h"
#include "chain_fast.h"
#include "lean.h"
#include "lean_tasks.h"
#include "search.h"

namespace rocco {

namespace {

struct DevProblem {
    const double *scores = nullptr;
    const double *costs = nullptr;
    double gamma = 0.0;
    size_t n = 0;
    uint8_t *solution = nullptr;
    int qexp = 0;
    double cmax = 0.0, sabs = 0.0;
    uint8_t *emap = nullptr;
    FrozenArrays frz = {};
    bool frz_valid = false;
    double frz_lo = 0.0, frz_hi = 0.0;
    std::vector<uint8_t> frz_flags;
    std::vector<int> active_blocks;
    double smin = 0.0, smax = 0.0;
    bool compacted = false;
    bool solution_in_orig = false;
    bool scattered = false;
    const double *orig_scores = nullptr;
    size_t orig_n = 0;
    uint8_t *orig_solution = nullptr;
    const int *lean_orig = nullptr;
    int map_version = 0;
    int wcap_version = -1;
};

struct LeanLevel {
    const double *s = nullptr;
    const int *orig = nullptr;
    long long m = 0;
    double base = -INFINITY;
    double sep = 0.0;
    bool has_eval = false;
    std::vector<double> pts;
    std::vector<long long> child_len;
    unsigned *bits = nullptr;
    unsigned *tile_off = nullptr;
    int cap_points = 0;
    size_t pool_mark = 0;
};

struct LeanState {
    std::vector<LeanLevel> levels;
    size_t pool_begin = 0, pool_end = 0, pool_at = 0;
};

struct LeanReq {
    size_t problem = 0;
    std::vector<double> lambdas;
    ProbeRequest *probe = nullptr;
    CompactRequest *comp = nullptr;
    bool pilot = false;
    bool model = false;
    double pilot_scale = 1.0;
    int result_begin = 0;
    double *out_s = nullptr;
    int *out_orig = nullptr;
    long long capacity = 0;
    double sep = 0.0;
    size_t mark = 0;
};

bool lambda_ties_some_grid(double lambda, int qexp)
{
    if (lambda == 0.0) {
        return false;
    }
    for (int e = qexp + 52; e <= 62; ++e) {
        const double magic_u = std::ldexp(1.5, e);
        volatile double t = -lambda + magic_u;
        const double r = t - magic_u;
        if (std::fabs(-lambda - r) == std::ldexp(1.0, e - 53)) {
            return true;
        }
    }
    return false;
}

int grid_exponent(double cmax, double lo, double hi)
{
    const double r = cmax + (hi - lo) + 2.0;
    return (int)std::ceil(std::log2(8.0 * r)) - 52;
}

std::atomic<long long> g_model_chain_counters[6];

class HipEvaluator : public Evaluator {
public:
    HipEvaluator(rocco_hip_solver *solver, hipStream_t stream) : solver_(solver), stream_(stream) {}

    mutable std::vector<std::pair<const char *, const char *>> env_cache_;
    const char *env(const char *name) const
    {
        for (const auto &e : env_cache_) {
            if (e.first == name || std::strcmp(e.first, name) == 0) {
                return e.second;
            }
        }
        const char *value = std::getenv(name);
        env_cache_.emplace_back(name, value);
        return value;
    }
    bool env_set(const char *name) const { return env(name) != nullptr; }
    int env_int(const char *name, int unset) const
    {
        const char *e = env(name);
        return e != nullptr ? std::atoi(e) : unset;
    }
    long long env_ll(const char *name, long long unset) const
    {
        const char *e = env(name);
        return e != nullptr ? std::atoll(e) : unset;
    }
    bool env_flag(const char *name, bool unset) const { return env_int(name, unset ? 1 : 0) != 0; }
    double env_double(const char *name, double unset) const
    {
        const char *e = env(name);
        return e != nullptr ? std::atof(e) : unset;
    }
    bool env_list(const char *name, std::vector<double> &out) const
    {
        const char *e = env(name);
        if (e == nullptr) {
            return false;
        }
        out.clear();
        for (const char *q = e; *q != '\0';) {
            char *end = nullptr;
            const double v = std::strtod(q, &end);
            if (end == q) break;
            if (v > 0.0) out.push_back(v);
            q = (*end == ',') ? end + 1 : end;
        }
        return true;
    }

    std::vector<DevProblem> probs;

    struct RoundTask {
        size_t problem = 0;
        bool window = false;
        bool map = false;
        bool record = false;
        bool survey = false;
        bool bound = false;
        bool use_frozen = false;
        int solution_index = -1;
        int select_depth = 0;
        bool select_has_upper = true;
        long long select_target = 0;
        double margin = 0.0;
        std::vector<double> lambdas;
        ProbeRequest *probe = nullptr;
        WindowRequest *win = nullptr;
        SpineRequest *spine = nullptr;
    };

    void add_probe_tasks(std::vector<ProbeRequest> &reqs, std::vector<RoundTask> &tasks)
    {
        for (ProbeRequest &r : reqs) {
            if (lean_takes(*this, r)) {
                continue;
            }
            r.results.assign(r.lambdas.size(), ProbeResult());
            if (r.lambdas.empty()) {
                continue;
            }
            RoundTask t;
            t.problem = r.problem;
            t.window = false;
            t.bound = r.bound;
            t.lambdas = r.lambdas;
            t.probe = &r;
            tasks.push_back(t);
        }
    }

    int probe(std::vector<ProbeRequest> &reqs) override
    {
        std::vector<CompactRequest> none;
        int rc;
        if ((rc = lean_submit(none, reqs)) != ROCCO_HIP_OK) return rc;
        std::vector<RoundTask> tasks;
        add_probe_tasks(reqs, tasks);
        if (tasks.empty()) {
            if (lean_wait_needed()) {
                ROCCO_HIP_TRY(hipStreamSynchronize(stream_));
            }
        } else if ((rc = run_round(tasks)) != ROCCO_HIP_OK) {
            return rc;
        }
        if ((rc = lean_consume()) != ROCCO_HIP_OK) return rc;
        return model_fallback();
    }

    std::vector<char> window_answered_;

    void add_window_tasks(std::vector<WindowRequest> &reqs, std::vector<RoundTask> &tasks)
    {
        for (size_t i = 0; i < reqs.size(); ++i) {
            WindowRequest &r = reqs[i];
            if (i < window_answered_.size() && window_answered_[i]) {
                continue;
            }
            RoundTask t;
            t.problem = r.problem;
            t.window = true;
            t.lambdas = {r.lambda_lo, r.lambda_hi};
            t.win = &r;
            tasks.push_back(t);
        }
    }

    int window(std::vector<WindowRequest> &reqs) override
    {
        window_answered_.clear();
        std::vector<RoundTask> tasks;
        add_window_tasks(reqs, tasks);
        return run_round(tasks);
    }

    int add_survey_tasks(std::vector<WindowRequest> &reqs, std::vector<RoundTask> &tasks)
    {
        if (solver_->active_set == 0 || reqs.empty()) {
            return ROCCO_HIP_OK;
        }
        int rc;
        if (!frozen_allocated_) {
            size_t total_blocks = 0;
            for (const DevProblem &p : probs) {
                total_blocks += align_up((p.n + kFastBlockLoci - 1) / kFastBlockLoci, 32);
            }
            const size_t per_block = 8 * 8 + 4 * 4 + 3;
            if ((rc = solver_->dev_frozen.reserve(total_blocks * per_block + 4096)) != ROCCO_HIP_OK) return rc;
            char *base = (char *)solver_->dev_frozen.ptr;
            double *dbl = (double *)base;
            int *i32 = (int *)(base + total_blocks * 64);
            uint8_t *u8 = (uint8_t *)(base + total_blocks * 80);
// ... 1621 lines not shown
                        all = facts_answer(q, res);
                    }
                    if (all) {
                        q.results = res;
                        model_chain_hits += (long long)q.lambdas.size();
                        lean_model_points += (long long)q.lambdas.size();
                        model_tiles_answered_ += lean_tiles(probs[q.problem].n);
                        continue;
                    }
                }
                LeanReq r;
                r.problem = q.problem;
                r.lambdas = q.lambdas;
                r.probe = &q;
                r.model = !q.bound;
                r.pilot = q.bound && q.pilot && can_pilot(q.problem);
                reqs.push_back(r);
            }
        }
        if (reqs.empty() && model_tiles_answered_ > 0) {
            model_tiles_last_round_ = model_tiles_answered_;
        }
        return lean_enqueue(reqs);
    }

    static bool lean_takes(const HipEvaluator &ev, const ProbeRequest &q)
    {
        if (q.lambdas.empty() || q.lambdas.size() > (size_t)kLeanMaxPoints) {
            return false;
        }
        return q.bound ? ev.lean_eligible(q.problem) : (!q.pilot && ev.model_eligible(q.problem));
    }

    int round_all(std::vector<CompactRequest> &compacts, std::vector<MapRequest> &maps, std::vector<WindowRequest> &surveys,
                  std::vector<ProbeRequest> &probes, std::vector<WindowRequest> &windows,
                  std::vector<SpineRequest> &spines) override
    {
        int rc;
        const double tr0 = now_us();
        struct Total {
            double &acc;
            double t0;
            ~Total() { acc += now_us() - t0; }
        } total{t_round_, tr0};
        mark("round begins");
        if ((rc = lean_submit(compacts, probes)) != ROCCO_HIP_OK) return rc;
        mark("round: lean part submitted");
        window_answered_.assign(windows.size(), 0);
        std::vector<size_t> answered_problems;
        if (!windows.empty()) {
            bool any_in_chain = false;
            for (const WindowRequest &w : windows) {
                any_in_chain = any_in_chain || in_running_chain(w.problem);
            }
            if (any_in_chain && (rc = model_chain_drain()) != ROCCO_HIP_OK) return rc;
            for (size_t i = 0; i < windows.size(); ++i) {
                WindowRequest &w = windows[i];
                if (w.problem < written_.size() && written_[w.problem].valid && w.lambda_lo == w.lambda_hi &&
                    w.lambda_lo == written_[w.problem].penalty) {
                    w.result = WindowResult();
                    w.result.count_lo = w.result.count_hi = written_[w.problem].count;
                    w.result.n_diff = 0;
                    window_answered_[i] = 1;
                    answered_problems.push_back(w.problem);
                    ++model_chain_windows_answered;
                }
            }
        }
        std::vector<RoundTask> tasks;
        if ((rc = add_map_tasks(maps, tasks)) != ROCCO_HIP_OK) return rc;
        if ((rc = add_survey_tasks(surveys, tasks)) != ROCCO_HIP_OK) return rc;
        add_probe_tasks(probes, tasks);
        add_window_tasks(windows, tasks);
        if ((rc = add_spine_tasks(spines, tasks)) != ROCCO_HIP_OK) return rc;
        if (tasks.empty()) {
            if (lean_wait_needed()) {
                const double ts0 = now_us();
                ROCCO_HIP_TRY(hipStreamSynchronize(stream_));
                t_wait_ += now_us() - ts0;
            }
        } else {
            std::vector<size_t> final_problems;
            const size_t open_windows = windows.size() - answered_problems.size();
            if (env_flag("ROCCO_HIP_PREFETCH_OBJECTIVE", true) && open_windows > 0 && tasks.size() == open_windows && lean_inflight_.empty()) {
                for (size_t i = 0; i < windows.size(); ++i) {
                    if (!window_answered_[i] && windows[i].lambda_lo == windows[i].lambda_hi) {
                        final_problems.push_back(windows[i].problem);
                    }
                }
                if (final_problems.size() != open_windows) {
                    final_problems.clear();
                }
            }
            if ((rc = run_round(tasks, !lean_wait_needed(), final_problems.empty() ? nullptr : &final_problems)) != ROCCO_HIP_OK) {
                return rc;
            }
            if (!final_problems.empty()) {
                std::vector<char> certified;
                for (size_t i = 0; i < windows.size(); ++i) {
                    if (!window_answered_[i]) {
                        certified.push_back((!windows[i].result.overflow && windows[i].result.n_diff == 0) ? 1 : 0);
                    }
                }
                objective_collect(certified);
            }
        }
        const double tc0 = now_us();
        mark("round: device work waited for");
        if ((rc = lean_consume()) != ROCCO_HIP_OK) return rc;
        if ((rc = model_fallback()) != ROCCO_HIP_OK) return rc;
        adopt_maps(maps);
        t_consume_ += now_us() - tc0;
        mark("round ends");
        ++rounds_all;
        return ROCCO_HIP_OK;
    }

    int compute_stats(std::vector<double> &out)
    {
        const size_t B = probs.size();
        out.assign(5 * B, 0.0);
        if (B == 0) {
            return ROCCO_HIP_OK;
        }
        std::vector<int2> blockmap;
        for (size_t b = 0; b < B; ++b) {
            const int nb = (int)((probs[b].n + kFastBlockLoci - 1) / kFastBlockLoci);
            for (int k = 0; k < nb; ++k) {
                blockmap.push_back(make_int2((int)b, k));
            }
        }
        const size_t nbt = blockmap.size();
        const size_t bytes_tasks = align_up(B * sizeof(StatsTask), 256);
        const size_t bytes_map = align_up(nbt * sizeof(int2), 256);
        const size_t bytes_part = align_up(nbt * 5 * sizeof(double), 256);
        const size_t bytes_out = align_up(B * 5 * sizeof(double), 256);
        int rc;
        if ((rc = solver_->dev_misc.reserve(bytes_tasks + bytes_map + bytes_part + bytes_out)) != ROCCO_HIP_OK) return rc;
        if ((rc = stage_wait()) != ROCCO_HIP_OK) return rc;
        if ((rc = solver_->host_stage.reserve(bytes_tasks + bytes_map)) != ROCCO_HIP_OK) return rc;
        if ((rc = solver_->host_back.reserve(bytes_out)) != ROCCO_HIP_OK) return rc;
        char *h = (char *)solver_->host_stage.ptr;
        StatsTask *ht = (StatsTask *)h;
        for (size_t b = 0; b < B; ++b) {
            ht[b].scores = probs[b].scores;
            ht[b].switch_costs = probs[b].costs;
            ht[b].n = (long long)probs[b].n;
        }
        std::memcpy(h + bytes_tasks, blockmap.data(), nbt * sizeof(int2));
        char *dv = (char *)solver_->dev_misc.ptr;
        ROCCO_HIP_TRY(hipMemcpyAsync(dv, h, bytes_tasks + bytes_map, hipMemcpyHostToDevice, stream_));
        double *d_part = (double *)(dv + bytes_tasks + bytes_map);
        double *d_out = (double *)(dv + bytes_tasks + bytes_map + bytes_part);
        if ((rc = launch_stats((const StatsTask *)dv, (int)B, (const int2 *)(dv + bytes_tasks), (int)nbt, d_part,
                               d_out, stream_)) != ROCCO_HIP_OK) {
            return rc;
        }
        ROCCO_HIP_TRY(hipMemcpyAsync(solver_->host_back.ptr, d_out, B * 5 * sizeof(double), hipMemcpyDeviceToHost, stream_));
        ROCCO_HIP_TRY(hipStreamSynchronize(stream_));
        std::memcpy(out.data(), solver_->host_back.ptr, B * 5 * sizeof(double));
        return ROCCO_HIP_OK;
    }

    int chain_rounds_run = 0;
    int chain_search(const std::vector<ChainProblem> &problems, const SearchOptions &opt, std::vector<double> &stats_out,
                     std::vector<Presearch> &pre, bool &ran)
    {
        ran = false;
        const double tc0 = now_us();
        const size_t B = probs.size();
        const bool forced = env_set("ROCCO_HIP_CHAIN");
        if (!env_flag("ROCCO_HIP_CHAIN", true) || solver_->lean == 0 || B == 0 || B > (size_t)kChainMaxProblems ||
            !opt.use_bounds || opt.force_exact || !opt.use_compaction) {
            return ROCCO_HIP_OK;
        }
        bool any = false;
        long long tiles0 = 0;
        for (size_t b = 0; b < B; ++b) {
            any = any || lean_eligible(b);
            tiles0 += lean_tiles(probs[b].n);
            if (probs[b].n >= ((size_t)1 << 31)) {
                return ROCCO_HIP_OK;
            }
        }
        if (!any) {
            return ROCCO_HIP_OK;
        }
        if (tiles0 < env_ll("ROCCO_HIP_CHAIN_MIN_TILES", 4096) && !forced) {
            return ROCCO_HIP_OK;
        }
        int rc;
        if ((rc = lean_prepare()) != ROCCO_HIP_OK) return rc;
        ChainTuning tune;
        tune.pilot_rounds = env_int("ROCCO_HIP_CHAIN_PILOT_ROUNDS", 6);
        tune.pilot_points = env_int("ROCCO_HIP_CHAIN_PILOT_POINTS", 8);
        if (opt.pilot_rounds <= 0) {
            tune.pilot_rounds = 0;
        }
        tune.wgs = std::max(64, env_int("ROCCO_HIP_CHAIN_WGS", 512));
        tune.pilot_wgs = std::max(64, env_int("ROCCO_HIP_CHAIN_PILOT_WGS", 512));
        tune.pilot_tiles = std::max(2, env_int("ROCCO_HIP_CHAIN_PILOT_TILES", 16));
        tune.big_points = env_int("ROCCO_HIP_CHAIN_BIG_POINTS", 2);
        tune.search_gate = opt.search_gate;
        tune.survey_gate = opt.survey_gate;
        tune.interpolate = env_int("ROCCO_HIP_CHAIN_INTERP", 0);
        tune.spread = env_double("ROCCO_HIP_CHAIN_SPREAD", 0.005);
        if (!(tune.spread > 0.0 && tune.spread < 0.5)) {
            tune.spread = 0.005;
        }
        tune.soft_mult = env_double("ROCCO_HIP_CHAIN_SOFT", 0.8);
        {
            std::vector<double> mults = {2.2, 1.2};
            env_list("ROCCO_HIP_CHAIN_LEVELS", mults);
            tune.n_mults = (int)std::min(mults.size(), (size_t)kChainMaxMults);
            for (int k = 0; k < kChainMaxMults; ++k) {
                tune.mults[k] = (k < tune.n_mults) ? mults[(size_t)k] : 0.0;
            }
        }
        const int R = std::max(1, env_int("ROCCO_HIP_CHAIN_ROUNDS", 12));

        std::vector<int2> blockmap;
        for (size_t b = 0; b < B; ++b) {
            const int nb = (int)((probs[b].n + kFastBlockLoci - 1) / kFastBlockLoci);
            for (int k = 0; k < nb; ++k) {
                blockmap.push_back(make_int2((int)b, k));
            }
        }
        const size_t nbt = blockmap.size();
        Layout lay;
        const size_t o_ctl = lay.at(sizeof(LeanRoundCtl));
        const size_t o_in = lay.at(B * sizeof(ChainInput));
        const size_t o_stasks = lay.at(B * sizeof(StatsTask));
        const size_t o_bmap = lay.at(nbt * sizeof(int2));
        lay.end_upload();
        const size_t up_bytes = lay.uploaded;
        const size_t o_probs = lay.at(B * sizeof(ChainProb));
        const size_t o_stats = lay.at(B * 5 * sizeof(double));
        const size_t o_ctl_back = lay.at(sizeof(LeanRoundCtl));
        const size_t down_bytes = lay.bytes() - o_probs;
        const size_t o_hot = lay.at(B * sizeof(ChainHot));
        const size_t o_pilot = lay.at(B * sizeof(ChainPilot));
        const size_t o_evals = lay.at(B * sizeof(ChainEvals));
        const size_t o_tasks = lay.at(B * sizeof(LeanTask));
        const size_t o_points = lay.at(B * kLeanMaxPoints * sizeof(double));
        const size_t o_results = lay.at(B * kLeanMaxPoints * sizeof(LeanResult));
        const size_t o_pre = lay.at(B * sizeof(LeanCompactTask));
        const size_t o_part = lay.at(nbt * 5 * sizeof(double));
        const bool want_trace = env_set("ROCCO_HIP_CHAIN_TRACE");
        const size_t o_trace = lay.at((size_t)(R + 2) * 8 * sizeof(long long));
        if ((rc = solver_->dev_chain.reserve(lay.bytes() + 256)) != ROCCO_HIP_OK) return rc;
        if ((rc = solver_->host_chain.reserve(std::max(up_bytes, down_bytes) + 256)) != ROCCO_HIP_OK) return rc;
        char *dv = (char *)solver_->dev_chain.ptr;
        char *h = (char *)solver_->host_chain.ptr;
        std::memset(h, 0, o_in);
        ChainInput *hin = (ChainInput *)(h + o_in);
        StatsTask *hst = (StatsTask *)(h + o_stasks);
        for (size_t b = 0; b < B; ++b) {
            const DevProblem &p = probs[b];
            hin[b].scores = p.scores;
            hin[b].n = (long long)p.n;
            hin[b].gamma = p.gamma;
            hin[b].target = std::max(0LL, std::min(problems[b].target_count, (long long)p.n));
            hin[b].pool_begin = lean_[b].pool_begin;
            hin[b].pool_end = lean_[b].pool_end;
            hin[b].allowed = lean_eligible(b) ? 1 : 0;
            hin[b].can_pilot = can_pilot(b) ? 1 : 0;
            hst[b].scores = p.scores;
            hst[b].switch_costs = p.costs;
            hst[b].n = (long long)p.n;
        }
        std::memcpy(h + o_bmap, blockmap.data(), nbt * sizeof(int2));
        ROCCO_HIP_TRY(hipMemcpyAsync(dv, h, up_bytes, hipMemcpyHostToDevice, stream_));
        if ((rc = launch_stats((const StatsTask *)(dv + o_stasks), (int)B, (const int2 *)(dv + o_bmap), (int)nbt, (double *)(dv + o_part),
                               (double *)(dv + o_stats), stream_)) != ROCCO_HIP_OK) {
            return rc;
        }

        const long long rec_cap = 8 * (tiles0 + (long long)tune.wgs) + 64 * (long long)B;
        if ((rc = reserve_round_scratch(rec_cap, false)) != ROCCO_HIP_OK) return rc;

        ChainArgs A;
        A.n_problems = (int)B;
        A.rec_capacity = (int)std::min<long long>(rec_cap, 0x7FFFFFFF);
        A.inputs = (const ChainInput *)(dv + o_in);
        A.probs = (ChainProb *)(dv + o_probs);
        A.hot = (ChainHot *)(dv + o_hot);
        A.pilot = (ChainPilot *)(dv + o_pilot);
        A.evals = (ChainEvals *)(dv + o_evals);
        A.stats = (const double *)(dv + o_stats);
        A.ctl = (LeanRoundCtl *)(dv + o_ctl);
        A.tasks = (LeanTask *)(dv + o_tasks);
        A.points = (double *)(dv + o_points);
        A.results = (LeanResult *)(dv + o_results);
        A.pre = (LeanCompactTask *)(dv + o_pre);
        A.pool = (char *)solver_->dev_lean_pool.ptr;
        A.trace = want_trace ? (long long *)(dv + o_trace) : nullptr;
        A.tune = tune;
        const bool follow = env_flag("ROCCO_HIP_CHAIN_FOLLOW", true);
        A.follow = nullptr;
        A.follow_words = (int)((o_ctl_back - o_probs) / 8);
        A.follow_ctl_word = A.follow_words;
        if (follow) {
            solver_->host_follow.coherent = true;
            if ((rc = solver_->host_follow.reserve(256 + down_bytes + 256)) != ROCCO_HIP_OK) return rc;
            A.follow = (unsigned long long *)solver_->host_follow.ptr;
            std::memset(solver_->host_follow.ptr, 0, 256);
        }

        LeanLaunch L = round_launch(A.tasks, A.points, A.results);
        L.ctl = A.ctl;
        const int eval_grid = (int)std::min<long long>(512, std::max<long long>(1, tiles0 * 8));
        const int compact_grid = (int)std::min<long long>(1024, std::max<long long>(1, tiles0));
        const int finish_grid = (int)std::min<size_t>(2048, B * (size_t)kLeanMaxPoints);
        solver_->lean_look_dirty = 1;
        for (int r = 0; r < R; ++r) {
            if ((rc = launch_chain_director(A, r, 0, stream_)) != ROCCO_HIP_OK) return rc;
            if ((rc = launch_lean_compact_chain(A.pre, A.ctl, compact_grid, stream_)) != ROCCO_HIP_OK) return rc;
            if ((rc = launch_lean_eval_chain(L, eval_grid, stream_)) != ROCCO_HIP_OK) return rc;
            if ((rc = launch_lean_finish_chain(L, finish_grid, stream_)) != ROCCO_HIP_OK) return rc;
        }
        if ((rc = launch_chain_director(A, R, 1, stream_)) != ROCCO_HIP_OK) return rc;
        ROCCO_HIP_TRY(hipGetLastError());
        const double ts0 = now_us();
        if (follow) {
            const unsigned long long *flag = A.follow;
            for (long long spins = 1;; ++spins) {
                if (__atomic_load_n(flag, __ATOMIC_ACQUIRE) != 0ull) {
                    break;
                }
                if (spins > 200000) {
                    std::this_thread::yield();
                }
                if ((spins & 1023) == 0) {
                    const hipError_t q = hipStreamQuery(stream_);
                    if (q != hipErrorNotReady) {
                        if (q == hipSuccess && __atomic_load_n(flag, __ATOMIC_ACQUIRE) != 0ull) {
                            break;
                        }
                        set_last_error(q != hipSuccess ? "chained search: the stream reports an error" : "chained search: the stream ended without the chain's report");
                        return ROCCO_HIP_EHIP;
                    }
                }
            }
            h = (char *)solver_->host_follow.ptr + 256;
        } else {
            ROCCO_HIP_TRY(hipMemcpyAsync(dv + o_ctl_back, dv + o_ctl, sizeof(LeanRoundCtl), hipMemcpyDeviceToDevice, stream_));
            ROCCO_HIP_TRY(hipMemcpyAsync(h, dv + o_probs, down_bytes, hipMemcpyDeviceToHost, stream_));
            ROCCO_HIP_TRY(hipStreamSynchronize(stream_));
        }
        const double ts1 = now_us();
        mark("threshold chain waited for");
        t_wait_ += ts1 - ts0;
        t_chain_submit_ = ts0 - tc0;
        t_chain_wait_ = ts1 - ts0;
        struct Parse {
            double &acc;
            double t0;
            ~Parse() { acc = now_us() - t0; }
        } parse{t_chain_parse_, ts1};
        solver_->lean_look_dirty = 0;
        const ChainProb *rep = (const ChainProb *)h;
        const double *hstats = (const double *)(h + (o_stats - o_probs));
        const LeanRoundCtl *ctl = (const LeanRoundCtl *)(h + (o_ctl_back - o_probs));
        if (ctl->error != 0u) {
            solver_->lean_look_dirty = 1;
            set_last_error((ctl->error & 1u) ? "chained search: a tile waited for its predecessor beyond the spin limit"
                                             : "chained search: a compaction overflowed its level");
            return ROCCO_HIP_EHIP;
        }
        ran = true;
        chain_rounds_run = ctl->round;
        if (want_trace) {
            std::vector<long long> tr((size_t)(R + 1) * 8);
            ROCCO_HIP_TRY(hipMemcpy(tr.data(), dv + o_trace, tr.size() * sizeof(long long), hipMemcpyDeviceToHost));
            for (int r = 0; r <= R; ++r) {
                const long long *t = tr.data() + 8 * r;
                std::fprintf(stderr, "[chain] director %d: state in %.2f us, results + compaction %.2f, groups %.2f, penalties %.2f, offsets %.2f, descriptors + state out %.2f; since the chain began %.2f\n",
                             r, 0.01 * (double)(t[1] - t[0]), 0.01 * (double)(t[2] - t[1]), 0.0, 0.01 * (double)(t[3] - t[2]),
                             0.01 * (double)(t[4] - t[3]), 0.01 * (double)(t[5] - t[4]), 0.01 * (double)(t[0] - tr[0]));
            }
        }
        stats_out.assign(hstats, hstats + 5 * B);
        pre.assign(B, Presearch());
        const bool debug = env_set("ROCCO_HIP_DEBUG");
        const bool chain_debug = env_set("ROCCO_HIP_CHAIN_DEBUG");
        bool grid_ok = true;
        for (size_t b = 0; b < B; ++b) {
            const ChainProb &r = rep[b];
            if (r.searching == 0) {
                continue;
            }
            const double cmax = (probs[b].costs != nullptr && probs[b].n > 1) ? hstats[5 * b + 3] : probs[b].gamma;
            if (r.qexp != grid_exponent(std::max(cmax, 0.0), hstats[5 * b + 0], hstats[5 * b + 1])) {
                grid_ok = false;
            }
        }
        if (!grid_ok) {
            if (debug) {
                std::fprintf(stderr, "[chain] grid exponent differs from the host's: the chain's work is discarded\n");
            }
            pre.assign(B, Presearch());
            return ROCCO_HIP_OK;
        }
        for (size_t b = 0; b < B; ++b) {
            const ChainProb &r = rep[b];
            if (r.searching == 0 || r.n_evals == 0) {
                continue;
            }
            Presearch &ps = pre[b];
            for (int i = 0; i < r.n_above; ++i) {
                ps.evals.emplace_back(r.above_x[i], r.above_c[i]);
            }
            for (int i = 0; i < r.n_below; ++i) {
                ps.evals.emplace_back(r.below_x[i], r.below_c[i]);
            }
            ps.rounds = r.rounds + r.pilots;
            ps.done = (r.done == 1);
            LeanState &ls = lean_[b];
            ls.levels.clear();
            for (int k = 0; k < r.n_levels; ++k) {
                LeanLevel lv;
                lv.s = r.levels[k].s;
                lv.orig = r.levels[k].orig;
                lv.m = r.levels[k].m;
                lv.base = r.levels[k].base;
                lv.sep = r.levels[k].sep;
                lv.has_eval = false;
                lv.bits = r.levels[k].bits;
                lv.tile_off = r.levels[k].tile_off;
                lv.cap_points = r.levels[k].cap_points;
                lv.pool_mark = (size_t)r.levels[k].pool_mark;
                ls.levels.push_back(lv);
            }
            ls.pool_at = (size_t)r.pool_at;
            if (chain_debug) {
                std::vector<ChainEvals> all(1);
                ROCCO_HIP_TRY(hipMemcpy(all.data(), dv + o_evals + b * sizeof(ChainEvals), sizeof(ChainEvals), hipMemcpyDeviceToHost));
                for (int i = 0; i < r.n_evals; ++i) {
                    std::fprintf(stderr, "[chain] problem %zu count(%.17g) = %lld%s\n", b, all[0].x[i], all[0].c[i],
                                 all[0].c[i] > std::max(0LL, std::min(problems[b].target_count, (long long)probs[b].n)) ? "  >" : "");
                }
            }
            if (debug) {
                std::fprintf(stderr, "[chain] problem %zu (n=%zu): %d pilot + %d certified rounds, %d counts, %d levels (deepest m=%lld, base %.17g)%s\n",
                             b, probs[b].n, r.pilots, r.rounds, r.n_evals, r.n_levels, r.levels[r.n_levels - 1].m,
                             r.levels[r.n_levels - 1].base, r.done == 1 ? ", ended" : (r.done == 2 ? ", given up" : ", out of rounds"));
            }
        }
        return ROCCO_HIP_OK;
    }

    int rounds = 0;
    long long blocks_launched = 0;

private:

public:
    double t_prep_ = 0.0, t_launch_ = 0.0, t_wait_ = 0.0, t_consume_ = 0.0, t_round_ = 0.0;
    double t_lean_cpu_ = 0.0, t_lean_h2d_ = 0.0, t_lean_launch_ = 0.0;
    double t_chain_submit_ = 0.0, t_chain_wait_ = 0.0, t_chain_parse_ = 0.0;
    int rounds_all = 0;
    static double now_us()
    {
        return std::chrono::duration<double, std::micro>(std::chrono::steady_clock::now().time_since_epoch()).count();
    }

private:
    int run_round(std::vector<RoundTask> &rt, bool may_defer = false, const std::vector<size_t> *prefetch = nullptr)
    {
        const size_t T = rt.size();
        if (T == 0) {
            return ROCCO_HIP_OK;
        }
        ++rounds;
        for (size_t t = 0; t < T; ++t) {
            objective_invalidate(rt[t].problem);
        }
        {
            const int rcw = stage_wait();
            if (rcw != ROCCO_HIP_OK) return rcw;
        }
        const double tt0 = now_us();
        std::vector<FastTask> tasks(T);
        std::vector<FastChain> chains;
        std::vector<FastSlot> slots;
        std::vector<int2> blockmap, blockmap_all;
        std::vector<std::vector<int>> launched(T);
        std::vector<char> launched_all(T, 0);
        std::vector<long long> skip_off(T, -1);
        std::vector<uint8_t> skip_bytes;
        long long chain_chunks = 0, chain_blocks = 0, slot_chunks = 0, slot_blocks = 0, rec_entries = 0;
        long long rec_groups = 0;
        bool any_record = false, any_select = false;
        std::vector<int> solution_slot(T, -1);
        bool any_costs = false, any_plain = false, any_window = false, any_map = false;
        for (size_t t = 0; t < T; ++t) {
            const DevProblem &p = probs[rt[t].problem];
            FastTask &ft = tasks[t];
            const long long nchunks = (long long)((p.n + kChunk - 1) / kChunk);
            const int nblocks = (int)((p.n + kFastBlockLoci - 1) / kFastBlockLoci);
            ft.scores = p.scores;
            ft.switch_costs = p.costs;
            ft.gamma = p.gamma;
            ft.n = (long long)p.n;
            ft.qexp = p.qexp;
            ft.emap = p.emap;
            ft.emap_out = rt[t].map ? map_ptrs_[rt[t].problem] : nullptr;
            ft.map_margin = rt[t].margin;
            ft.magic = std::ldexp(1.5, 52 + p.qexp);
            ft.big = std::ldexp(1.0, 50 + p.qexp);
            ft.qstep = std::ldexp(1.0, p.qexp);
            ft.cmax = p.cmax;
            ft.sabs = p.sabs;
            ft.n_blocks = nblocks;
            ft.solution = p.solution;
            ft.frz = FrozenArrays{};
            ft.frz_out = FrozenArrays{};
            bool use_frozen = p.frz_valid && !no_frozen_ && solver_->active_set != 0 && !rt[t].bound;
            if (use_frozen) {
                for (double lam : rt[t].lambdas) {
                    if (!(lam >= p.frz_lo && lam <= p.frz_hi) || lambda_ties_some_grid(lam, p.qexp)) {
                        use_frozen = false;
                    }
                }
            }
            rt[t].use_frozen = use_frozen;
            launched[t].clear();
            if (use_frozen) {
                ft.frz = p.frz;
                skip_off[t] = (long long)skip_bytes.size();
                std::vector<uint8_t> skip(p.frz_flags);
                if (rt[t].record) {
                    for (int k : p.active_blocks) {
                        if (k + 1 < nblocks) {
                            skip[k + 1] = 0;
                        }
// ... 324 lines not shown
            if (rt[t].map) {
                continue;
            }
            if (rt[t].record) {
                rt[t].spine->counts.resize(rt[t].lambdas.size());
                rt[t].spine->stepped.resize(rt[t].lambdas.size());
                for (int k = 0; k < ft.slot_count; ++k) {
                    rt[t].spine->counts[k] = hr[ft.slot_begin + k].count_lo;
                    rt[t].spine->stepped[k] = hr[ft.slot_begin + k].uncertain;
                }
                rt[t].spine->selected = (ft.sel_depth > 0) ? hr[ft.slot_begin].e_global : -1;
                if (env_set("ROCCO_HIP_DEBUG")) {
                    std::fprintf(stderr, "[spine] problem %zu: lane 0 stepped %lld chunks of %lld\n", rt[t].problem,
                                 (long long)hr[ft.slot_begin].uncertain, (long long)((p.n + kChunk - 1) / kChunk));
                    std::fprintf(stderr, "[spine] prof (100 MHz ticks): fetch %lld loop %lld (steps %lld) slow groups %lld\n",
                                 hr[ft.slot_begin].p16, hr[ft.slot_begin].npos, hr[ft.slot_begin].max_run,
                                 hr[ft.slot_begin].n_diff);
                }
                continue;
            }
            if (rt[t].window) {
                const FastSlotResult &r = hr[ft.slot_begin];
                WindowResult &w = rt[t].win->result;
                w.count_lo = r.count_lo;
                w.count_hi = r.count_hi;
                w.n_diff = r.n_diff;
                w.diff_adjacent = (r.nonadjacent == 0);
                w.overflow = (r.overflow != 0);
                w.max_run = r.max_run;
                w.diffs.clear();
                const long long listed = std::min<long long>(r.n_diff, kMaxDiffs);
                for (long long k = 0; k < listed; ++k) {
                    WindowDiff d;
                    d.locus = r.diffs[k].locus;
                    d.margin_lo = r.diffs[k].margin_lo;
                    d.margin_hi = r.diffs[k].margin_hi;
                    d.run = r.diffs[k].run;
                    d.cls_lo = r.diffs[k].cls_lo;
                    d.cls_hi = r.diffs[k].cls_hi;
                    w.diffs.push_back(d);
                }
                std::sort(w.diffs.begin(), w.diffs.end(),
                          [](const WindowDiff &a, const WindowDiff &b) { return a.locus < b.locus; });
            } else {
                for (int k = 0; k < ft.slot_count; ++k) {
                    const FastSlotResult &r = hr[ft.slot_begin + k];
                    ProbeResult &o = rt[t].probe->results[k];
                    o.count = r.count_lo;
                    o.uncertain = rt[t].bound ? 0 : r.uncertain;
                    o.effect = rt[t].bound ? 0 : (r.overflow ? (long long)p.n + 1 : r.effect);
                    o.max_run = r.max_run;
                }
            }
        }
        return ROCCO_HIP_OK;
    }

    rocco_hip_solver *solver_;
    hipStream_t stream_;
    bool maps_allocated_ = false;
    bool frozen_allocated_ = false;
    bool no_frozen_ = false;
    std::vector<uint8_t *> map_ptrs_;
};

int prepare(HipEvaluator &ev, std::vector<ChainProblem> &problems, const std::vector<double> *fixed_lambdas,
            const double *score_stats_host = nullptr, const std::vector<double> *stats5 = nullptr)
{
    std::vector<double> stats;
    if (stats5 != nullptr && stats5->size() == 5 * problems.size()) {
        stats = *stats5;
    }
    bool given = (score_stats_host != nullptr) && stats.empty();
    for (size_t b = 0; given && b < problems.size(); ++b) {
        given = (ev.probs[b].costs == nullptr || ev.probs[b].n <= 1);
    }
    if (given) {
        stats.assign(5 * problems.size(), 0.0);
        for (size_t b = 0; b < problems.size(); ++b) {
            stats[5 * b + 0] = score_stats_host[3 * b + 0];
            stats[5 * b + 1] = score_stats_host[3 * b + 1];
            stats[5 * b + 4] = score_stats_host[3 * b + 2];
        }
    } else if (stats.empty()) {
        const int rc = ev.compute_stats(stats);
        if (rc != ROCCO_HIP_OK) {
            return rc;
        }
    }
    for (size_t b = 0; b < problems.size(); ++b) {
        ChainProblem &p = problems[b];
        DevProblem &d = ev.probs[b];
        p.score_min = stats[5 * b + 0];
        p.score_max = stats[5 * b + 1];
        p.score_abs_sum = stats[5 * b + 4];
        if (d.costs != nullptr && d.n > 1) {
            p.cost_min = stats[5 * b + 2];
            p.cost_max = stats[5 * b + 3];
            p.has_cost_vector = true;
        } else {
            p.cost_min = p.cost_max = d.gamma;
            p.has_cost_vector = false;
        }
        double lo = p.score_min, hi = p.score_max;
        if (fixed_lambdas != nullptr) {
            lo = std::min(lo, (*fixed_lambdas)[b]);
            hi = std::max(hi, (*fixed_lambdas)[b]);
        }
        d.cmax = p.cost_max;
        d.smin = p.score_min;
        d.smax = p.score_max;
        d.sabs = std::max(std::fabs(p.score_min), std::fabs(p.score_max));
        d.qexp = (std::isfinite(lo) && std::isfinite(hi) && std::isfinite(p.cost_max))
                     ? grid_exponent(std::max(p.cost_max, 0.0), lo, hi)
                     : 0;
    }
    return ROCCO_HIP_OK;
}

struct SingleProblem {
    HipEvaluator ev;
    std::vector<ChainProblem> problems;
    SingleProblem(rocco_hip_solver *solver, hipStream_t stream, const double *scores_dev, const double *switch_costs_dev, double gamma,
                  size_t n, uint8_t *solution_dev = nullptr)
        : ev(solver, stream), problems(1)
    {
        DevProblem d;
        d.scores = scores_dev;
        d.costs = (n > 1) ? switch_costs_dev : nullptr;
        d.gamma = gamma;
        d.n = n;
        d.solution = solution_dev;
        ev.probs.push_back(d);
        problems[0].n = n;
        problems[0].gamma = gamma;
    }
    int prepare_problem(const std::vector<double> *fixed_lambdas = nullptr, const uint8_t *emap_dev = nullptr)
    {
        const int rc = prepare(ev, problems, fixed_lambdas);
        ev.probs[0].emap = const_cast<uint8_t *>(emap_dev);
        return rc;
    }
};

}

void model_chain_counters(long long out[4])
{
    for (int k = 0; k < 4; ++k) {
        out[k] = g_model_chain_counters[k].load(std::memory_order_relaxed);
    }
}

void model_chain_written_counters(long long out[2])
{
    out[0] = g_model_chain_counters[4].load(std::memory_order_relaxed);
    out[1] = g_model_chain_counters[5].load(std::memory_order_relaxed);
}

int solve_fixed_penalty(rocco_hip_solver *solver, const double *scores_dev,
                        const double *switch_costs_dev, double gamma, size_t n, double lambda,
                        uint8_t *solution_dev, double *value_out, long long *count_out, int *path_out,
                        hipStream_t stream)
{
    int rc;
    if (solution_dev == nullptr) {
        if ((rc = solver->dev_solution.reserve(n)) != ROCCO_HIP_OK) return rc;
        solution_dev = (uint8_t *)solver->dev_solution.ptr;
    }
    SingleProblem one(solver, stream, scores_dev, switch_costs_dev, gamma, n, solution_dev);
    HipEvaluator &ev = one.ev;
    std::vector<ChainProblem> &problems = one.problems;
    std::vector<double> lambdas = {lambda};
    if ((rc = one.prepare_problem(&lambdas)) != ROCCO_HIP_OK) return rc;
    SearchOptions opt;
    opt.force_exact = solver->force_exact != 0;
    std::vector<CalibrationResult> res;
    if ((rc = solve_fixed_batch(ev, problems, lambdas, opt, res)) != ROCCO_HIP_OK) return rc;
    if (value_out) *value_out = res[0].penalized_value;
    if (count_out) *count_out = res[0].selected_count;
    if (path_out) *path_out = res[0].path;
    return ROCCO_HIP_OK;
}

int delta_build_map(rocco_hip_solver *solver, const double *scores_dev, const double *switch_costs_dev,
                    double gamma, size_t n, double lambda_ref, double margin, uint8_t *emap_dev,
                    hipStream_t stream)
{
    SingleProblem one(solver, stream, scores_dev, switch_costs_dev, gamma, n);
    HipEvaluator &ev = one.ev;
    int rc;
    if ((rc = one.prepare_problem()) != ROCCO_HIP_OK) return rc;
    std::vector<MapRequest> reqs(1);
    reqs[0].problem = 0;
    reqs[0].lambda_ref = lambda_ref;
    reqs[0].margin = margin;
    if ((rc = ev.build_map(reqs)) != ROCCO_HIP_OK) return rc;
    ROCCO_HIP_TRY(hipMemcpyAsync(emap_dev, ev.probs[0].emap, (n + kChunk - 1) / kChunk, hipMemcpyDeviceToDevice, stream));
    ROCCO_HIP_TRY(hipStreamSynchronize(stream));
    return ROCCO_HIP_OK;
}

int delta_build_map_lean(rocco_hip_solver *solver, const double *scores_dev, double gamma, size_t n, double lambda_ref,
                         double margin, uint8_t *emap_dev, hipStream_t stream)
{
    SingleProblem one(solver, stream, scores_dev, nullptr, gamma, n);
    HipEvaluator &ev = one.ev;
    int rc;
    if ((rc = one.prepare_problem()) != ROCCO_HIP_OK) return rc;
    ev.force_lean_map_ = true;
    if (!ev.lean_map_takes(0)) {
        set_last_error("lean map: not available for this array (lean evaluation off, or fewer than two loci)");
        return ROCCO_HIP_EINVAL;
    }
    std::vector<MapRequest> reqs(1);
    reqs[0].problem = 0;
    reqs[0].lambda_ref = lambda_ref;
    reqs[0].margin = margin;
    if ((rc = ev.build_map(reqs)) != ROCCO_HIP_OK) return rc;
    ROCCO_HIP_TRY(hipMemcpyAsync(emap_dev, ev.probs[0].emap, (n + kChunk - 1) / kChunk, hipMemcpyDeviceToDevice, stream));
    ROCCO_HIP_TRY(hipStreamSynchronize(stream));
    return ev.lean_map_check();
}

int delta_spine(rocco_hip_solver *solver, const double *scores_dev, const double *switch_costs_dev,
                double gamma, size_t n, const uint8_t *emap_dev, const double *lambdas, size_t n_lambdas,
                int solution_index, uint8_t *solution_dev, long long *counts_out, hipStream_t stream)
{
    SingleProblem one(solver, stream, scores_dev, switch_costs_dev, gamma, n, solution_dev);
    HipEvaluator &ev = one.ev;
    int rc;
    if ((rc = one.prepare_problem(nullptr, emap_dev)) != ROCCO_HIP_OK) return rc;
    std::vector<SpineRequest> reqs(1);
    reqs[0].problem = 0;
    reqs[0].lambdas.assign(lambdas, lambdas + n_lambdas);
    reqs[0].solution_index = solution_index;
    if ((rc = ev.spine(reqs)) != ROCCO_HIP_OK) return rc;
    for (size_t i = 0; i < n_lambdas; ++i) {
        counts_out[i] = reqs[0].counts[i];
    }
    if (ev.env_set("ROCCO_HIP_DEBUG")) {
        fprintf(stderr, "[rocco_hip] spine: n=%zu chunks=%zu stepped[0]=%lld\n", n, (n + 31) / 32, reqs[0].stepped[0]);
    }
    return ROCCO_HIP_OK;
}

int delta_probe(rocco_hip_solver *solver, const double *scores_dev, const double *switch_costs_dev,
                double gamma, size_t n, const uint8_t *emap_dev, const double *lambdas, size_t n_lambdas,
                rocco_hip_probe_stats *stats_out, hipStream_t stream)
{
    SingleProblem one(solver, stream, scores_dev, switch_costs_dev, gamma, n);
    HipEvaluator &ev = one.ev;
    int rc;
    if ((rc = one.prepare_problem(nullptr, emap_dev)) != ROCCO_HIP_OK) return rc;
    std::vector<ProbeRequest> reqs(1);
    reqs[0].problem = 0;
    reqs[0].lambdas.assign(lambdas, lambdas + n_lambdas);
    if ((rc = ev.probe(reqs)) != ROCCO_HIP_OK) return rc;
    for (size_t i = 0; i < n_lambdas; ++i) {
        stats_out[i].count = reqs[0].results[i].count;
        stats_out[i].uncertain = reqs[0].results[i].uncertain;
        stats_out[i].effect = reqs[0].results[i].effect;
        stats_out[i].max_run = reqs[0].results[i].max_run;
    }
    return ROCCO_HIP_OK;
}

int delta_model_lean(rocco_hip_solver *solver, const double *scores_dev, double gamma, size_t n, const uint8_t *emap_dev,
                     const double *lambdas, size_t n_lambdas, long long *counts_out, long long *open_out, hipStream_t stream)
{
    SingleProblem one(solver, stream, scores_dev, nullptr, gamma, n);
    HipEvaluator &ev = one.ev;
    int rc;
    if ((rc = one.prepare_problem(nullptr, emap_dev)) != ROCCO_HIP_OK) return rc;
    ev.probs[0].map_version = 1;
    if ((rc = ev.lean_prepare()) != ROCCO_HIP_OK) return rc;
    ev.model_any_ = true;
    if (!ev.model_eligible(0)) {
        set_last_error("rocco_hip_delta_model_lean_f64: the lean evaluation is switched off for this solver");
        return ROCCO_HIP_EINVAL;
    }
    for (size_t at = 0; at < n_lambdas; at += (size_t)kLeanMaxPoints) {
        std::vector<ProbeRequest> reqs(1);
        reqs[0].problem = 0;
        const size_t k = std::min((size_t)kLeanMaxPoints, n_lambdas - at);
        reqs[0].lambdas.assign(lambdas + at, lambdas + at + k);
        if ((rc = ev.probe(reqs)) != ROCCO_HIP_OK) return rc;
        for (size_t i = 0; i < k; ++i) {
            counts_out[at + i] = reqs[0].results[i].count;
            open_out[at + i] = reqs[0].results[i].uncertain;
        }
    }
    return ROCCO_HIP_OK;
}

int delta_bound_rounds(rocco_hip_solver *solver, const double *scores_dev, double gamma, size_t n,
                       const double *lambdas, const int *round_sizes, int n_rounds, double *lambdas_used_out,
                       long long *counts_out, long long *level_len_out, hipStream_t stream)
{
    SingleProblem one(solver, stream, scores_dev, nullptr, gamma, n);
    HipEvaluator &ev = one.ev;
    int rc;
    if ((rc = one.prepare_problem()) != ROCCO_HIP_OK) return rc;
    if (!ev.lean_eligible(0)) {
        set_last_error("rocco_hip_delta_bound_rounds_f64: the lean evaluation is switched off for this solver");
        return ROCCO_HIP_EINVAL;
    }
    const int qexp = ev.probs[0].qexp;
    size_t at = 0;
    for (int r = 0; r < n_rounds; ++r) {
        std::vector<ProbeRequest> reqs(1);
        reqs[0].problem = 0;
        reqs[0].bound = true;
        for (int i = 0; i < round_sizes[r]; ++i) {
            const double x = std::ldexp(std::nearbyint(std::ldexp(lambdas[at + (size_t)i], -qexp)), qexp);
            reqs[0].lambdas.push_back(x);
            lambdas_used_out[at + (size_t)i] = x;
        }
        if (reqs[0].lambdas.empty() || reqs[0].lambdas.size() > (size_t)kLeanMaxPoints) {
            return ROCCO_HIP_EINVAL;
        }
        if ((rc = ev.probe(reqs)) != ROCCO_HIP_OK) return rc;
        for (int i = 0; i < round_sizes[r]; ++i) {
            counts_out[at + (size_t)i] = reqs[0].results[(size_t)i].count;
        }
        level_len_out[r] = ev.lean_[0].levels.back().m;
        at += (size_t)round_sizes[r];
    }
    return ROCCO_HIP_OK;
}

int delta_window(rocco_hip_solver *solver, const double *scores_dev, const double *switch_costs_dev,
                 double gamma, size_t n, const uint8_t *emap_dev, double lambda_lo, double lambda_hi,
                 uint8_t *solution_dev, rocco_hip_window_stats *stats_out, hipStream_t stream)
{
    SingleProblem one(solver, stream, scores_dev, switch_costs_dev, gamma, n, solution_dev);
    HipEvaluator &ev = one.ev;
    int rc;
    if ((rc = one.prepare_problem(nullptr, emap_dev)) != ROCCO_HIP_OK) return rc;
    std::vector<WindowRequest> reqs(1);
    reqs[0].problem = 0;
    reqs[0].lambda_lo = lambda_lo;
    reqs[0].lambda_hi = lambda_hi;
    if ((rc = ev.window(reqs)) != ROCCO_HIP_OK) return rc;
    const WindowResult &w = reqs[0].result;
    stats_out->count_lo = w.count_lo;
    stats_out->count_hi = w.count_hi;
    stats_out->n_diff = w.n_diff;
    stats_out->diff_adjacent = w.diff_adjacent ? 1 : 0;
    stats_out->overflow = w.overflow ? 1 : 0;
    stats_out->max_run = w.max_run;
    for (size_t k = 0; k < 16; ++k) {
        if (k < w.diffs.size()) {
            stats_out->diff_locus[k] = w.diffs[k].locus;
            stats_out->diff_margin_lo[k] = w.diffs[k].margin_lo;
            stats_out->diff_margin_hi[k] = w.diffs[k].margin_hi;
            stats_out->diff_run[k] = w.diffs[k].run;
            stats_out->diff_cls_lo[k] = w.diffs[k].cls_lo;
            stats_out->diff_cls_hi[k] = w.diffs[k].cls_hi;
        } else {
            stats_out->diff_locus[k] = -1;
            stats_out->diff_margin_lo[k] = stats_out->diff_margin_hi[k] = 0.0;
            stats_out->diff_run[k] = 0;
            stats_out->diff_cls_lo[k] = stats_out->diff_cls_hi[k] = 0;
        }
    }
    return ROCCO_HIP_OK;
}

int solve_budget_batch(rocco_hip_solver *solver, size_t n_tasks, const rocco_hip_budget_task *tasks,
                       rocco_hip_budget_result *results, hipStream_t stream, const double *score_stats_host)
{
    HipEvaluator ev(solver, stream);
    std::vector<ChainProblem> problems(n_tasks);
    for (size_t t = 0; t < n_tasks; ++t) {
        DevProblem d;
        d.scores = tasks[t].scores_dev;
        d.costs = (tasks[t].n > 1) ? tasks[t].switch_costs_dev : nullptr;
        d.gamma = tasks[t].gamma;
        d.n = tasks[t].n;
        d.solution = tasks[t].solution_dev;
        ev.probs.push_back(d);
        problems[t].n = tasks[t].n;
        problems[t].gamma = tasks[t].gamma;
        problems[t].target_count = tasks[t].target_count;
        problems[t].sum_costs = tasks[t].sum_costs;
        problems[t].max_iter = tasks[t].max_iter;
    }
    int rc;
    SearchOptions opt;
    opt.force_exact = solver->force_exact != 0;
    opt.spec_depth = solver->spec_depth;
    opt.big_round_loci = ev.env_double("ROCCO_HIP_BIG_ROUND", opt.big_round_loci);
    opt.small_round_loci = ev.env_double("ROCCO_HIP_SMALL_ROUND", opt.small_round_loci);
    opt.survey_gate = ev.env_double("ROCCO_HIP_SURVEY_GATE", opt.survey_gate);
    opt.tiny_round_loci = ev.env_double("ROCCO_HIP_TINY_ROUND", opt.tiny_round_loci);
    opt.map_rebuild_ratio = ev.env_double("ROCCO_HIP_MAP_REBUILD", opt.map_rebuild_ratio);
    opt.use_bounds = ev.env_flag("ROCCO_HIP_BOUNDS", opt.use_bounds);
    opt.search_gate = ev.env_double("ROCCO_HIP_SEARCH_GATE", opt.search_gate);
    if (ev.env_set("ROCCO_HIP_SEARCH_POINTS")) opt.search_points = std::max(1, ev.env_int("ROCCO_HIP_SEARCH_POINTS", 0));
    opt.search_interpolate = ev.env_flag("ROCCO_HIP_SEARCH_INTERP", opt.search_interpolate);
    std::vector<CalibrationResult> res;
    const double t_solve0 = HipEvaluator::now_us();
    ev.marks_on_ = ev.env_int("ROCCO_HIP_TIMING", 0) >= 2;
    ev.mark("solve begins");
    opt.use_compaction = ev.env_flag("ROCCO_HIP_COMPACT", opt.use_compaction);
    opt.pilot_rounds = ev.env_int("ROCCO_HIP_PILOT_ROUNDS", opt.pilot_rounds);
    opt.pilot_points = ev.env_int("ROCCO_HIP_PILOT_POINTS", opt.pilot_points);
    opt.align_maps = ev.env_flag("ROCCO_HIP_ALIGN_MAPS", opt.align_maps);
    opt.align_windows = ev.env_flag("ROCCO_HIP_ALIGN_WINDOWS", opt.align_windows);
    ev.env_list("ROCCO_HIP_PILOT_LEVELS", opt.pilot_levels);
    struct LeanOverride {
        rocco_hip_solver *solver;
        int saved;
        ~LeanOverride() { solver->lean = saved; }
    } lean_override{solver, solver->lean};
    if (ev.env_set("ROCCO_HIP_LEAN")) solver->lean = ev.env_flag("ROCCO_HIP_LEAN", true) ? 1 : 0;
    std::vector<double> chain_stats;
    std::vector<Presearch> presearch;
    bool chained = false;
    if (score_stats_host == nullptr) {
        if ((rc = ev.chain_search(problems, opt, chain_stats, presearch, chained)) != ROCCO_HIP_OK) return rc;
    }
    const double tp0 = HipEvaluator::now_us();
    ev.mark("threshold chain parsed");
    if ((rc = prepare(ev, problems, nullptr, score_stats_host, chained ? &chain_stats : nullptr)) != ROCCO_HIP_OK) return rc;
    const double tp1 = HipEvaluator::now_us();
    if ((rc = calibrate_batch(ev, problems, opt, res, chained ? &presearch : nullptr)) != ROCCO_HIP_OK) return rc;
    const double tp2 = HipEvaluator::now_us();
    ev.mark("calibration ends");
    if ((rc = ev.scatter_all()) != ROCCO_HIP_OK) return rc;
    ROCCO_HIP_TRY(hipStreamSynchronize(stream));
    const double t_prepare = tp1 - tp0, t_calibrate = tp2 - tp1, t_scatter = HipEvaluator::now_us() - tp2;
    g_model_chain_counters[0].fetch_add(ev.model_chains, std::memory_order_relaxed);
    g_model_chain_counters[1].fetch_add(ev.model_chain_facts, std::memory_order_relaxed);
    g_model_chain_counters[2].fetch_add(ev.model_chain_hits, std::memory_order_relaxed);
    g_model_chain_counters[3].fetch_add(ev.model_chain_misses, std::memory_order_relaxed);
    g_model_chain_counters[4].fetch_add(ev.model_chain_written, std::memory_order_relaxed);
    g_model_chain_counters[5].fetch_add(ev.model_chain_windows_answered, std::memory_order_relaxed);
    if (ev.env_set("ROCCO_HIP_DEBUG") || ev.env_set("ROCCO_HIP_TIMING")) {
        const double total = HipEvaluator::now_us() - t_solve0;
        std::fprintf(stderr, "[host] solve %.0f us: %d rounds (%d with rounding-model kernels): in the rounds %.0f us = waiting for the device %.0f "
                             "+ reading results %.0f + preparing and submitting %.0f; search logic and the rest %.0f us\n",
                     total, ev.rounds_all, ev.rounds, ev.t_round_, ev.t_wait_, ev.t_consume_,
                     ev.t_round_ - ev.t_wait_ - ev.t_consume_, total - ev.t_round_);
        std::fprintf(stderr, "[host] lean rounds: building the descriptors %.0f us, their upload call %.0f, the launch calls %.0f; general rounds: "
                             "preparing %.0f, launching %.0f\n",
                     ev.t_lean_cpu_, ev.t_lean_h2d_, ev.t_lean_launch_, ev.t_prep_, ev.t_launch_);
        std::fprintf(stderr, "[host] chained search: queued in %.0f us, waited for %.0f, report read in %.0f; statistics -> problems %.0f; "
                             "calibration after it %.0f; scatter and the last wait %.0f\n",
                     ev.t_chain_submit_, ev.t_chain_wait_, ev.t_chain_parse_, t_prepare, t_calibrate, t_scatter);
        std::fprintf(stderr, "[host] chained rounding-model rounds: %lld chains queued in %.0f us, their rounds waited for %.0f us; %lld counts taken "
                             "over, %lld requests answered from them, %lld not\n",
                     ev.model_chains, ev.t_mchain_submit_, ev.t_mchain_wait_, ev.model_chain_facts, ev.model_chain_hits, ev.model_chain_misses);
        std::fprintf(stderr, "[host] objectives fetched behind final windows: %lld rounds, %lld sums used; solutions written by the chains: %lld, "
                             "final windows answered from them: %lld\n",
                     ev.objective_prefetches, ev.objective_prefetch_hits, ev.model_chain_written, ev.model_chain_windows_answered);
        ev.mark("solve ends");
        for (size_t k = 0; k < ev.marks_.size(); ++k) {
            std::fprintf(stderr, "[mark] %8.1f  +%6.1f  %s\n", ev.marks_[k].second - t_solve0,
                         k ? ev.marks_[k].second - ev.marks_[k - 1].second : 0.0, ev.marks_[k].first);
        }
    }
    for (size_t t = 0; t < n_tasks; ++t) {
        results[t].selection_penalty = res[t].selection_penalty;
        results[t].penalized_value = res[t].penalized_value;
        results[t].selected_count = res[t].selected_count;
        results[t].evaluations = res[t].evaluations;
        results[t].path = res[t].path;
        results[t].passes = res[t].passes;
        results[t].zone_iters = res[t].zone_iters;
        results[t].n_diff = res[t].n_diff;
        results[t].maps = res[t].maps;
    }
    return ROCCO_HIP_OK;
}

}
```

rocco_amd/csrc/chain.h:

```cpp
#pragma once

#include "lean.h"

namespace rocco {

constexpr int kChainMaxProblems = 128;
constexpr int kChainMaxLevels = 8;
constexpr int kChainMaxEvals = 384;
constexpr int kChainMaxPilot = 192;
constexpr int kChainMaxMults = 4;
constexpr int kChainKeep = 4;

struct ChainInput {
    const double *scores;
    long long n;
    double gamma;
    long long target;
    unsigned long long pool_begin, pool_end;
    int allowed;
    int can_pilot;
};

struct ChainLevelReport {
    const double *s;
    const int *orig;
    long long m;
    double base, sep;
    unsigned long long pool_mark;
    unsigned *bits;
    unsigned *tile_off;
    int cap_points;
    int pad;
};

struct ChainProb {
    double smin, smax, sabs_sum;
    double eps;
    int qexp;
    int searching;
    int done;
    int rounds;
    int pilots;
    int n_evals;
    int n_levels;
    int pad;
    unsigned long long pool_at;
    ChainLevelReport levels[kChainMaxLevels];
    int n_above, n_below;
    double above_x[kChainKeep], below_x[kChainKeep];
    long long above_c[kChainKeep], below_c[kChainKeep];
};

struct ChainEvals {
    double x[kChainMaxEvals];
    long long c[kChainMaxEvals];
};

struct ChainHot {
    const double *scores;
    long long n;
    double gamma;
    long long target;
    unsigned long long pool_end, pool_at;
    double smin, smax, sabs_sum, eps;
    double pg, pl, pilot_scale;
    double est_pg, est_pl;
    double G, L;
    long long cG, cL;
    long long open_before;
    double soft_hi, soft_span, pilot_res, soft_count;
    const double *lv_s;
    const int *lv_orig;
    long long lv_m;
    unsigned *lv_bits;
    unsigned *lv_tile_off;
    int lv_cap;
    int n_levels;
    int qexp, searching, done, rounds, pilots, n_evals;
    int phase;
    int pilot_left, pilot_hint, n_pilot;
    int G_real, L_real;
    int kind;
    int np;
    int have_soft;
    int can_pilot;
    int pilot_ready;
    int pad;
};
static_assert(sizeof(ChainHot) % 8 == 0, "ChainHot is moved as 8-byte words");

struct ChainPilot {
    double x[kChainMaxPilot], c[kChainMaxPilot];
};

struct ChainTuning {
    int pilot_rounds;
    int pilot_points;
    int n_mults;
    int pilot_wgs;
    int pilot_tiles;
    int wgs;
    double mults[kChainMaxMults];
    double search_gate, survey_gate;
    int big_points;
    int interpolate;
    double spread;
    double soft_mult;
};

struct ChainArgs {
    int n_problems;
    int rec_capacity;
    const ChainInput *inputs;
    ChainProb *probs;
    ChainHot *hot;
    ChainPilot *pilot;
    ChainEvals *evals;
    const double *stats;
    LeanRoundCtl *ctl;
    LeanTask *tasks;
    double *points;
    LeanResult *results;
    LeanCompactTask *pre;
    char *pool;
    long long *trace;
    unsigned long long *follow;
    int follow_words;
    int follow_ctl_word;
    ChainTuning tune;
};

int launch_chain_director(const ChainArgs &A, int round, int last, hipStream_t stream);

}
```

rocco_amd/csrc/chain.hip:

```cpp
#include "chain.h"

#include <cmath>

namespace rocco {

namespace {

constexpr int kDirectorWaves = 16;
constexpr int kDirectorThreads = 64 * kDirectorWaves;

__device__ __forceinline__ double snap_to_grid(double x, int qexp) { return ldexp(rint(ldexp(x, -qexp)), qexp); }

__device__ __forceinline__ int ceil_log2_exact(double x)
{
    const int e = ilogb(x);
    return (x == ldexp(1.0, e)) ? e : e + 1;
}

__device__ __forceinline__ unsigned long long align_up_dev(unsigned long long x, unsigned long long a) { return (x + a - 1) / a * a; }

__device__ __forceinline__ char *pool_alloc(const ChainArgs &A, ChainHot &H, unsigned long long bytes)
{
    const unsigned long long at = align_up_dev(H.pool_at, 256);
    if (at + bytes > H.pool_end) {
        return nullptr;
    }
    H.pool_at = at + bytes;
    return A.pool + at;
}

__device__ bool pilot_crossing(const ChainPilot &W, int n_pilot, double want, int lane, double *x_out)
{
    for (int base = 0; base + 1 < n_pilot; base += 64) {
        const int i = base + lane;
        const bool valid = i + 1 < n_pilot;
        const double x0 = valid ? W.x[i] : 0.0, x1 = valid ? W.x[i + 1] : 0.0;
        const double c0 = valid ? W.c[i] : 0.0, c1 = valid ? W.c[i + 1] : 0.0;
        const unsigned long long hit = __ballot(valid && c0 >= want && c1 < want);
        if (hit != 0ull) {
            const double l0 = log(fmax(c0, 0.5)), l1 = log(fmax(c1, 0.5));
            const double f = (l0 > l1) ? (l0 - log(want)) / (l0 - l1) : 0.5;
            *x_out = __shfl(x0 + f * (x1 - x0), __builtin_ctzll(hit));
            return true;
        }
    }
    return false;
}

__device__ void init_problem(const ChainArgs &A, int b, ChainHot &H)
{
    const ChainInput in = A.inputs[b];
    const double smin = A.stats[5 * b + 0], smax = A.stats[5 * b + 1], sabs_sum = A.stats[5 * b + 4];
    H.scores = in.scores;
    H.n = in.n;
    H.gamma = in.gamma;
    H.target = in.target;
    H.pool_end = in.pool_end;
    H.pool_at = in.pool_begin;
    H.smin = smin;
    H.smax = smax;
    H.sabs_sum = sabs_sum;
    H.eps = 0.0;
    H.pg = H.pl = 0.0;
    H.pilot_scale = 1.0;
    H.est_pg = (double)in.n;
    H.est_pl = 0.0;
    H.G = H.L = 0.0;
    H.cG = H.cL = 0;
    H.open_before = 0x7FFFFFFFFFFFFFFFLL;
    H.soft_hi = H.soft_span = H.pilot_res = H.soft_count = 0.0;
    H.lv_s = in.scores;
    H.lv_orig = nullptr;
    H.lv_m = in.n;
    H.lv_bits = nullptr;
    H.lv_tile_off = nullptr;
    H.lv_cap = 0;
    H.n_levels = 0;
    H.qexp = 0;
    H.searching = 0;
    H.done = 0;
    H.rounds = 0;
    H.pilots = 0;
    H.n_evals = 0;
    H.phase = 0;
    H.pilot_left = 0;
    H.pilot_hint = 0;
    H.n_pilot = 0;
    H.G_real = H.L_real = 0;
    H.kind = 0;
    H.np = 0;
    H.have_soft = 0;
    H.can_pilot = in.can_pilot;
    H.pilot_ready = 0;
    H.pad = 0;
    if (in.allowed == 0 || in.n < 2 || !(in.target < in.n) || in.target < 0) {
        return;
    }
    const double c = in.gamma;
    const double sabs = fmax(fabs(smin), fabs(smax));
    if (!(c >= 1.0e-3) || !(c <= 1.0e6) || !isfinite(smin) || !isfinite(smax) || !(smax - smin <= 1.0e9) || !(sabs <= 1.0e12)) {
        return;
    }
    const double lambda = smin - 1.0;
    const double n = (double)in.n;
    const double sum_abs = sabs_sum * (1.0 + 1e-9) + 1.0;
    const double pos = sum_abs + n * fmax(0.0, -lambda);
    const double pb = 2.0 * (pos + n * 0.0625 + fmax(c, 0.0) + sabs + fabs(lambda) + 1.0);
    if (!(pb > 0.0) || !isfinite(pb)) {
        return;
    }
    const int e = ilogb(pb);
    const double r = fmax(c, 0.0) + (smax - smin) + 2.0;
    const int qexp = ceil_log2_exact(8.0 * r) - 52;
    const double hb = ldexp(1.0, e + 2 - 53);
    const double q = ldexp(1.0, qexp);
    if (!(hb >= q)) {
        return;
    }
    H.qexp = qexp;
    H.eps = 16.0 * hb + 4.0 * q;
    H.searching = 1;
    H.G = smin - 1.0;
    H.L = smax + 1.0;
    H.cG = in.n;
    H.cL = 0;
    H.pg = H.G;
    H.pl = H.L;
    H.n_levels = 1;
    ChainLevelReport l0;
    l0.s = in.scores;
    l0.orig = nullptr;
    l0.m = in.n;
    l0.base = -INFINITY;
    l0.sep = 0.0;
    l0.pool_mark = in.pool_begin;
    l0.bits = nullptr;
    l0.tile_off = nullptr;
    l0.cap_points = 0;
    l0.pad = 0;
    A.probs[b].levels[0] = l0;
    A.probs[b].n_above = 0;
    A.probs[b].n_below = 0;
    H.phase = 2;
    if (A.tune.pilot_rounds > 0 && in.target > 0 && in.can_pilot != 0 && (H.pl - H.pg > 64.0 * H.eps)) {
        H.phase = 1;
        H.pilot_left = A.tune.pilot_rounds;
    }
}

__device__ __forceinline__ void give_up(ChainHot &H)
{
    H.done = 2;
    H.phase = 3;
}

__device__ int consume(const ChainArgs &A, int b, ChainHot &H, double x, long long count, long long child, int lane,
                       LeanCompactTask *ct, bool plan_next)
{
    ChainProb &P = A.probs[b];
    const int np = H.np, kind = H.kind;
    const long long target = H.target;
    const double eps = H.eps;
    const bool on = lane < np;
    if (kind == 1) {
        ChainPilot &W = A.pilot[b];
        const int n_old = H.n_pilot;
        const double x_first = __shfl(x, 0);
        const double est = (double)llrint((double)count * H.pilot_scale);
        int at = 0;
        double keep_x[kChainMaxPilot / 64], keep_c[kChainMaxPilot / 64];
#pragma unroll
        for (int k = 0; k < kChainMaxPilot / 64; ++k) {
            const int i = k * 64 + lane;
            keep_x[k] = (i < n_old) ? W.x[i] : 0.0;
            keep_c[k] = (i < n_old) ? W.c[i] : 0.0;
            at += __builtin_popcountll(__ballot(i < n_old && keep_x[k] < x_first));
        }
        const int room = min(np, kChainMaxPilot - n_old);
#pragma unroll
        for (int k = 0; k < kChainMaxPilot / 64; ++k) {
            const int i = k * 64 + lane;
            if (i < n_old && i >= at) {
                W.x[i + room] = keep_x[k];
                W.c[i + room] = keep_c[k];
            }
        }
        if (lane < room) {
            W.x[at + lane] = x;
            W.c[at + lane] = est;
        }
        const bool more = on && est > (double)target;
        const unsigned long long more_b = __ballot(more), less_b = __ballot(on && !more);
        const int i_up = more_b ? 63 - __builtin_clzll(more_b) : 0, i_down = less_b ? __builtin_ctzll(less_b) : 0;
        const double up = more_b ? __shfl(x, i_up) : -INFINITY, down = less_b ? __shfl(x, i_down) : INFINITY;
        const double est_up = __shfl(est, i_up), est_down = __shfl(est, i_down);
        if (lane == 0) {
            ++H.pilots;
            H.n_pilot = n_old + room;
            if (up > H.pg) {
                H.pg = up;
                H.est_pg = est_up;
            }
            if (down < H.pl) {
                H.pl = down;
                H.est_pl = est_down;
            }
            const double pg = H.pg, pl = H.pl;
            const int left = H.pilot_left - 1;
            H.pilot_left = left;
            const bool smooth = H.est_pg <= 2.5 * fmax(H.est_pl, 1.0);
            H.pilot_ready = (left <= 0 || !(pl - pg > 64.0 * eps) || smooth) ? 1 : 0;
        }
        return 0;
    }
    const int n_evals = H.n_evals;
    if (on && n_evals + lane < kChainMaxEvals) {
        A.evals[b].x[n_evals + lane] = x;
        A.evals[b].c[n_evals + lane] = count;
    }
    const unsigned long long more = __ballot(on && count > target), less = __ballot(on && count <= target);
    const int i_more = more ? 63 - __builtin_clzll(more) : 0, i_less = less ? __builtin_ctzll(less) : 0;
    const double x_more = __shfl(x, i_more), x_less = __shfl(x, i_less);
    const long long c_more = __shfl(count, i_more), c_less = __shfl(count, i_less);
    const long long child_more = __shfl(child, i_more);
    {
        const int n_more = __builtin_popcountll(more), n_less = __builtin_popcountll(less);
        const int take_more = min(n_more, kChainKeep), take_less = min(n_less, kChainKeep);
        const int old_above = P.n_above, old_below = P.n_below;
        const int keep_above = min(old_above, kChainKeep - take_more), keep_below = min(old_below, kChainKeep - take_less);
        double ax = 0.0, bx = 0.0;
        long long ac = 0, bc = 0;
        if (lane < keep_above) {
            ax = P.above_x[old_above - keep_above + lane];
            ac = P.above_c[old_above - keep_above + lane];
        }
        if (lane < keep_below) {
            bx = P.below_x[old_below - keep_below + lane];
            bc = P.below_c[old_below - keep_below + lane];
        }
        if (lane < keep_above) {
            P.above_x[lane] = ax;
            P.above_c[lane] = ac;
        }
        if (lane < keep_below) {
            P.below_x[lane] = bx;
            P.below_c[lane] = bc;
        }
        const int rank_more = __builtin_popcountll(more & ((1ull << lane) - 1ull));
        if (((more >> lane) & 1ull) && rank_more >= n_more - take_more) {
            const int slot = keep_above + (rank_more - (n_more - take_more));
            P.above_x[slot] = x;
            P.above_c[slot] = count;
        }
// ... 546 lines not shown
```

rocco_amd/csrc/median.hip:

```cpp
#include "kernels.h"
#include "select_network.h"

#include <limits>

#ifndef ROCCO_MEDIAN_NT
#define ROCCO_MEDIAN_NT 0
#endif

namespace rocco {

namespace {

template <typename T, int KP, bool EXACT>
__device__ __forceinline__ double median_column(const T *__restrict__ m, int K_runtime, long long n, long long stride,
                                                double *__restrict__ out, long long col0, unsigned lane)
{
    const long long j = col0 + lane;
    if (j >= n) {
        return 0.0;
    }
    const int K = EXACT ? KP : K_runtime;
    const int pad = KP - K;
    const int n_lo = pad / 2;
    double v[KP];
    double sum = 0.0;
    const T *row = m + col0;
#pragma unroll
    for (int k = 0; k < KP; ++k) {
        if (EXACT) {
#if ROCCO_MEDIAN_NT
            v[k] = (double)__builtin_nontemporal_load(row + lane);
#else
            v[k] = (double)row[lane];
#endif
            row += stride;
        } else {
            v[k] = (double)row[lane];
            row += (k + 1 < K) ? stride : 0;
        }
    }
#pragma unroll
    for (int k = 0; k < KP; ++k) {
        if (EXACT || k < K) {
            sum += v[k];
        } else {
            v[k] = (k - K < n_lo) ? -std::numeric_limits<double>::infinity()
                                  : std::numeric_limits<double>::infinity();
        }
    }
    bool has_nan = false;
    if (is_nan_bits(sum)) {
#pragma unroll
        for (int k = 0; k < KP; ++k) {
            if (EXACT || k < K) {
                const bool bad = is_nan_bits(v[k]);
                has_nan |= bad;
                v[k] = bad ? std::numeric_limits<double>::infinity() : v[k];
            }
        }
    }
    select_middle<KP>(v);
    double r;
    if (K & 1) {
        r = v[KP / 2 - 1];
    } else {
        r = (v[KP / 2 - 1] + v[KP / 2]) / 2.0;
    }
    r = has_nan ? __longlong_as_double(0x7FF8000000000000LL) : r;
    out[j] = r;
    return r;
}

template <typename T, int KP, bool EXACT>
__global__ __launch_bounds__(256) void median_kernel(const T *__restrict__ m, int K_runtime, long long n,
                                                     long long stride, double *__restrict__ out)
{
    median_column<T, KP, EXACT>(m, K_runtime, n, stride, out, (long long)xcd_contiguous_block() * 256, threadIdx.x);
}

template <typename T, int KP, bool EXACT>
__global__ __launch_bounds__(256) void median_batch_kernel(MedianBatch batch)
{
    const unsigned logical = xcd_contiguous_block();
    int ti = -1;
#pragma unroll
    for (int i = 0; i < kMedianBatchMax; ++i) {
        ti += (batch.block_begin[i] <= logical) ? 1 : 0;
    }
    const MedianTask &task = batch.tasks[ti];
    const long long col0 = (long long)(logical - task.block_begin) * 256;
    const long long j = col0 + threadIdx.x;
    const double r = median_column<T, KP, EXACT>((const T *)task.matrix, batch.K, task.n, task.stride, task.out, col0, threadIdx.x);
    if (task.partials != nullptr) {
        const bool valid = j < task.n;
        const bool nan = valid && is_nan_bits(r);
        const double inf = std::numeric_limits<double>::infinity();
        double mn = (valid && !nan) ? r : inf, mx = (valid && !nan) ? r : -inf, ab = (valid && !nan) ? fabs(r) : 0.0;
#pragma unroll
        for (int off = 32; off > 0; off >>= 1) {
            mn = fmin(mn, __shfl_xor(mn, off));
            mx = fmax(mx, __shfl_xor(mx, off));
            ab += __shfl_xor(ab, off);
        }
        const bool any_nan = __ballot(nan) != 0ull;
        if ((threadIdx.x & 63) == 0) {
            double *p = task.partials + 3LL * (4LL * (logical - task.block_begin) + (threadIdx.x >> 6));
            p[0] = mn;
            p[1] = mx;
            p[2] = any_nan ? __longlong_as_double(0x7FF8000000000000LL) : ab;
        }
    }
}

constexpr int kStatsSlices = 64;
struct MedianStatsTask {
    const double *partials;
    long long n_partials;
};
struct MedianStatsBatch {
    MedianStatsTask tasks[kMedianBatchMax];
};

__device__ __forceinline__ void stats_block_reduce(double mn, double mx, double ab, bool nan, double *__restrict__ out)
{
    __shared__ double red[4][3];
#pragma unroll
    for (int off = 32; off > 0; off >>= 1) {
        mn = fmin(mn, __shfl_xor(mn, off));
        mx = fmax(mx, __shfl_xor(mx, off));
        ab += __shfl_xor(ab, off);
    }
    const bool any_nan = __syncthreads_or(nan ? 1 : 0) != 0;
    const int lane = threadIdx.x & 63, wave = threadIdx.x >> 6;
    if (lane == 0) {
        red[wave][0] = mn;
        red[wave][1] = mx;
        red[wave][2] = ab;
    }
    __syncthreads();
    if (threadIdx.x == 0) {
        out[0] = fmin(fmin(red[0][0], red[1][0]), fmin(red[2][0], red[3][0]));
        out[1] = fmax(fmax(red[0][1], red[1][1]), fmax(red[2][1], red[3][1]));
        const double sum = (red[0][2] + red[1][2]) + (red[2][2] + red[3][2]);
        out[2] = any_nan ? __longlong_as_double(0x7FF8000000000000LL) : sum;
    }
}

__global__ __launch_bounds__(256) void median_stats_slice_kernel(MedianStatsBatch batch, double *__restrict__ slices)
{
    const MedianStatsTask task = batch.tasks[blockIdx.y];
    const long long per = (task.n_partials + kStatsSlices - 1) / kStatsSlices;
    const long long lo = per * blockIdx.x, hi = min(task.n_partials, lo + per);
    const double inf = std::numeric_limits<double>::infinity();
    double mn = inf, mx = -inf, ab = 0.0;
    bool nan = false;
    for (long long b = lo + threadIdx.x; b < hi; b += 256) {
        mn = fmin(mn, task.partials[3 * b + 0]);
        mx = fmax(mx, task.partials[3 * b + 1]);
        const double a = task.partials[3 * b + 2];
        const bool bad = is_nan_bits(a);
        nan |= bad;
        ab += bad ? 0.0 : a;
    }
    stats_block_reduce(mn, mx, ab, nan, slices + 3LL * ((long long)blockIdx.y * kStatsSlices + blockIdx.x));
}

__global__ __launch_bounds__(256) void median_stats_final_kernel(const double *__restrict__ slices, double *__restrict__ out)
{
    const double inf = std::numeric_limits<double>::infinity();
    double mn = inf, mx = -inf, ab = 0.0;
    bool nan = false;
    if (threadIdx.x < kStatsSlices) {
        const double *p = slices + 3LL * ((long long)blockIdx.x * kStatsSlices + threadIdx.x);
        mn = p[0];
        mx = p[1];
        nan = is_nan_bits(p[2]);
        ab = nan ? 0.0 : p[2];
    }
    stats_block_reduce(mn, mx, ab, nan, out + 3LL * blockIdx.x);
}

__global__ __launch_bounds__(256) void score_stats_partial_kernel(const double *__restrict__ scores, long long n,
                                                                  double *__restrict__ partials)
{
    const long long j = (long long)blockIdx.x * 256 + threadIdx.x;
    const bool valid = j < n;
    const double r = valid ? scores[j] : 0.0;
    const bool nan = valid && is_nan_bits(r);
    const double inf = std::numeric_limits<double>::infinity();
    double mn = (valid && !nan) ? r : inf, mx = (valid && !nan) ? r : -inf, ab = (valid && !nan) ? fabs(r) : 0.0;
#pragma unroll
    for (int off = 32; off > 0; off >>= 1) {
        mn = fmin(mn, __shfl_xor(mn, off));
        mx = fmax(mx, __shfl_xor(mx, off));
        ab += __shfl_xor(ab, off);
    }
    const bool any_nan = __ballot(nan) != 0ull;
    if ((threadIdx.x & 63) == 0) {
        double *p = partials + 3LL * (4LL * blockIdx.x + (threadIdx.x >> 6));
        p[0] = mn;
        p[1] = mx;
        p[2] = any_nan ? __longlong_as_double(0x7FF8000000000000LL) : ab;
    }
}

constexpr int kHalf = 100;

template <typename T>
__global__ __launch_bounds__(64) void median_split_kernel(const T *__restrict__ m, int K, long long n, long long stride,
                                                          double *__restrict__ out)
{
    __shared__ double first[kHalf][64];
    const long long j = (long long)xcd_contiguous_block() * blockDim.x + threadIdx.x;
    if (j >= n) {
        return;
    }
    const double inf = std::numeric_limits<double>::infinity();
    const int pad = 2 * kHalf - K;
    const int n_lo = pad / 2;
    double v[kHalf];
    double sum = 0.0;
#pragma unroll
    for (int k = 0; k < kHalf; ++k) {
        v[k] = (double)m[(long long)k * stride + j];
        sum += v[k];
    }
    bool has_nan = false;
    if (is_nan_bits(sum)) {
#pragma unroll
        for (int k = 0; k < kHalf; ++k) {
            const bool bad = is_nan_bits(v[k]);
            has_nan |= bad;
            v[k] = bad ? inf : v[k];
        }
    }
    select_middle<kHalf>(v);
#pragma unroll
    for (int k = 0; k < kHalf; ++k) {
        first[k][threadIdx.x] = v[k];
    }
    sum = 0.0;
#pragma unroll
    for (int k = 0; k < kHalf; ++k) {
        const int row = min(kHalf + k, K - 1);
        v[k] = (double)m[(long long)row * stride + j];
    }
#pragma unroll
    for (int k = 0; k < kHalf; ++k) {
        const int row = kHalf + k;
        if (row < K) {
            sum += v[k];
        } else {
            v[k] = (row - K < n_lo) ? -inf : inf;
        }
    }
    if (is_nan_bits(sum)) {
#pragma unroll
        for (int k = 0; k < kHalf; ++k) {
            const bool bad = (kHalf + k < K) && is_nan_bits(v[k]);
            has_nan |= bad;
            v[k] = bad ? inf : v[k];
        }
    }
    select_middle<kHalf>(v);
    double lower = -inf, upper = inf;
#pragma unroll
    for (int i = 0; i < kHalf; ++i) {
        const double a = first[i][threadIdx.x], b = v[kHalf - 1 - i];
        lower = fmax(lower, fmin(a, b));
        upper = fmin(upper, fmax(a, b));
    }
    const double r = (K & 1) ? lower : (lower + upper) / 2.0;
    out[j] = has_nan ? __longlong_as_double(0x7FF8000000000000LL) : r;
}

template <typename T, int L, int P, int LANES>
__global__ __launch_bounds__(LANES) void median_parts_kernel(const T *__restrict__ m, int K, long long n, long long stride,
                                                             double *__restrict__ out)
{
    extern __shared__ double parts[];
    const long long j = (long long)xcd_contiguous_block() * blockDim.x + threadIdx.x;
    if (j >= n) {
        return;
    }
    const int lane = threadIdx.x;
    const double inf = std::numeric_limits<double>::infinity();
    const int pad = P * L - K;
    const int n_lo = pad / 2;
    bool has_nan = false;
#pragma unroll 1
    for (int p = 0; p < P; ++p) {
        double v[L];
        double sum = 0.0;
        if ((p + 1) * L <= K) {
            const T *__restrict__ src = m + (long long)(p * L) * stride + j;
#pragma unroll
            for (int k = 0; k < L; ++k) {
                v[k] = (double)src[(long long)k * stride];
            }
#pragma unroll
            for (int k = 0; k < L; ++k) {
                sum += v[k];
            }
        } else {
#pragma unroll
            for (int k = 0; k < L; ++k) {
                const int row = min(p * L + k, K - 1);
                v[k] = (double)m[(long long)row * stride + j];
            }
#pragma unroll
            for (int k = 0; k < L; ++k) {
                const int row = p * L + k;
                if (row < K) {
                    sum += v[k];
                } else {
                    v[k] = (row - K < n_lo) ? -inf : inf;
                }
            }
        }
        if (is_nan_bits(sum)) {
#pragma unroll
            for (int k = 0; k < L; ++k) {
                const bool bad = (p * L + k < K) && is_nan_bits(v[k]);
                has_nan |= bad;
                v[k] = bad ? inf : v[k];
            }
        }
        select_middle<L>(v);
#pragma unroll
        for (int k = 0; k < L; ++k) {
            parts[((size_t)p * L + k) * LANES + lane] = v[k];
        }
    }
    const int total = P * L;
    const int k1 = total / 2;
    int idx[P];
    double head[P];
#pragma unroll
    for (int p = 0; p < P; ++p) {
        idx[p] = 0;
        head[p] = parts[((size_t)p * L) * LANES + lane];
    }
    double first = -inf;
#pragma unroll 2
    for (int step = 0; step < k1; ++step) {
        double mn = head[0];
        int w = 0;
#pragma unroll
        for (int p = 1; p < P; ++p) {
// ... 493 lines not shown
```

rocco_amd/dp.py:

```python
from __future__ import annotations

import ctypes
import functools
import logging
from typing import Dict, Optional, Tuple, Union

import numpy as np

from . import _native

logger = logging.getLogger(__name__)

ArrayLike = Union[np.ndarray, "torch.Tensor", list, tuple]


def _torch():
    import torch

    return torch


def _device_index(device=None) -> int:
    torch = _torch()
    if not torch.cuda.is_available():
# ... 90 lines not shown
    return rec(int(m))


@functools.lru_cache(maxsize=4096)
def sum_constant_like_numpy(value: float, length: int) -> float:
    value = float(value)
    if length <= 0:
        return 0.0
    full, rest = divmod(int(length), _NUMPY_BUFSIZE)
    acc = 0.0
    if full:
        chunk = _pairwise_constant(value, _NUMPY_BUFSIZE)
        for _ in range(full):
            acc = acc + chunk
    if rest:
        acc = acc + _pairwise_constant(value, rest)
    return acc



def build_switch_costs(scores, gamma: float = 1.0) -> np.ndarray:
    if _is_tensor(scores):
        shape = tuple(scores.shape)
        ndim = scores.ndim
    else:
        scores_ = np.asarray(scores, dtype=np.float64)
        shape, ndim = scores_.shape, scores_.ndim
    if ndim != 1:
        raise ValueError("`scores` must be a one-dimensional array")
    if shape[0] <= 1:
        return np.zeros(0, dtype=np.float64)
    return np.full(shape[0] - 1, float(gamma), dtype=np.float64)


def _costs_arg(switch_costs, n: int, device):
    if switch_costs is None:
        raise ValueError("`switch_costs` is required")
    if np.isscalar(switch_costs):
        return None, float(switch_costs)
    t = _to_device_f64(switch_costs, device, name="switch_costs")
    if n > 1 and t.shape[0] != n - 1:
        raise ValueError("`switch_costs` must have length len(scores) - 1")
    if n <= 1:
        return None, 0.0
    return t, 0.0


def objective_value(solution, scores, switch_costs) -> float:
    torch = _torch()
    scores_t = _to_device_f64(scores)
    n = int(scores_t.shape[0])
    if _is_tensor(solution):
        sol_t = solution.to(scores_t.device)
    else:
        sol_t = torch.from_numpy(np.ascontiguousarray(np.asarray(solution) > 0.5, dtype=np.uint8)).to(scores_t.device)
    if sol_t.dtype != torch.uint8:
        sol_t = (sol_t > 0.5).to(torch.uint8)
    sol_t = sol_t.contiguous()
    if sol_t.shape[0] != n:
        raise ValueError("`solution` and `scores` must have the same length")
    costs_t, gamma = _costs_arg(switch_costs, n, scores_t.device)
    solver = _native.solver_for(scores_t.device.index)
    out = ctypes.c_double(0.0)
    _native.check(_native.load().rocco_hip_objective_value_f64(
        solver.handle, sol_t.data_ptr(), scores_t.data_ptr(),
        costs_t.data_ptr() if costs_t is not None else None, gamma, n, ctypes.byref(out),
        _stream_ptr(scores_t)), "rocco_hip_objective_value_f64")
    return float(out.value)


def solve_penalized_chain_device(scores_t, switch_costs, selection_penalty: float, want_solution=True):
    torch = _torch()
    n = int(scores_t.shape[0])
    if n <= 0:
        raise ValueError("`scores` cannot be empty")
    costs_t, gamma = _costs_arg(switch_costs, n, scores_t.device)
    sol_t = torch.empty(n, dtype=torch.uint8, device=scores_t.device) if want_solution else None
    value = ctypes.c_double(0.0)
    count = ctypes.c_longlong(0)
    path = ctypes.c_int(0)
    solver = _native.solver_for(scores_t.device.index)
    _native.check(_native.load().rocco_hip_solve_penalized_chain_f64(
        solver.handle, scores_t.data_ptr(), costs_t.data_ptr() if costs_t is not None else None,
        gamma, n, float(selection_penalty), sol_t.data_ptr() if sol_t is not None else None,
        ctypes.byref(value), ctypes.byref(count), ctypes.byref(path), _stream_ptr(scores_t)),
        "rocco_hip_solve_penalized_chain_f64")
    return sol_t, float(value.value), int(count.value), int(path.value)


def solve_penalized_chain(scores, switch_costs, selection_penalty: float) -> Tuple[np.ndarray, float, int]:
    _native.load()
    if not _is_tensor(scores):
        probe = np.asarray(scores)
        if probe.ndim != 1:
            raise ValueError("`scores` must be one-dimensional")
        if probe.shape[0] <= 0:
            raise ValueError("`scores` cannot be empty")
    if not np.isscalar(switch_costs) and not _is_tensor(switch_costs):
        if np.asarray(switch_costs).ndim != 1:
            raise ValueError("`switch_costs` must be one-dimensional")
    scores_t = _to_device_f64(scores)
    sol_t, value, count, _ = solve_penalized_chain_device(scores_t, switch_costs, selection_penalty)
    return sol_t.cpu().numpy().astype(np.uint8, copy=False), float(value), int(count)


def _sum_costs(n: int, costs_t, gamma: float) -> float:
    if costs_t is None:
        return sum_constant_like_numpy(gamma, n - 1)
    return float(np.sum(costs_t.cpu().numpy()))


def calibrate_selection_penalty_device(scores_t, switch_costs, target_count: int, max_iter: int = 60):
    return calibrate_batch_device([scores_t], [switch_costs], [target_count], max_iter=max_iter)[0]


def _max_iters(max_iter, k: int):
    if np.ndim(max_iter) == 0:
        return [max(0, int(max_iter))] * k
    steps = [max(0, int(m)) for m in max_iter]
    if len(steps) != k:
        raise ValueError("`max_iter` must be an int or hold one int per problem")
    return steps


def calibrate_batch_device(scores_list, switch_costs_list, target_counts, max_iter=60, score_stats=None):
    torch = _torch()
    lib = _native.load()
    k = len(scores_list)
    if k == 0:
        return []
    device = scores_list[0].device
    tasks = (_native.BudgetTask * k)()
    results = (_native.BudgetResult * k)()
    keep = []
    sols = []
    steps = _max_iters(max_iter, k)
    for i, (s_t, costs, target) in enumerate(zip(scores_list, switch_costs_list, target_counts)):
        n = int(s_t.shape[0])
        if n == 0:
            raise ValueError("`scores` cannot be empty")
        costs_t, gamma = _costs_arg(costs, n, device)
        sol_t = torch.empty(n, dtype=torch.uint8, device=device)
        keep.append((s_t, costs_t))
        sols.append(sol_t)
        tasks[i].scores_dev = s_t.data_ptr()
        tasks[i].switch_costs_dev = costs_t.data_ptr() if costs_t is not None else None
        tasks[i].gamma = gamma
        tasks[i].n = n
        tasks[i].target_count = int(target)
        tasks[i].sum_costs = _sum_costs(n, costs_t, gamma)
        tasks[i].max_iter = steps[i]
        tasks[i].solution_dev = sol_t.data_ptr()
    solver = _native.solver_for(device.index)
    if score_stats is not None:
        stats_h = np.ascontiguousarray(score_stats.numpy() if _is_tensor(score_stats) else score_stats, dtype=np.float64)
        if stats_h.shape != (k, 3):
            raise ValueError("`score_stats` must have shape [len(scores_list), 3]")
        _native.check(lib.rocco_hip_solve_budget_batch_stats_f64(solver.handle, k, tasks, stats_h.ctypes.data, results,
                                                                 _stream_ptr(scores_list[0])),
                      "rocco_hip_solve_budget_batch_stats_f64")
    else:
        _native.check(lib.rocco_hip_solve_budget_batch_f64(solver.handle, k, tasks, results,
                                                           _stream_ptr(scores_list[0])),
                      "rocco_hip_solve_budget_batch_f64")
    out = []
    for i in range(k):
        r = results[i]
        out.append((float(r.selection_penalty), sols[i], float(r.penalized_value), int(r.selected_count),
                    {"evaluations": int(r.evaluations), "path": int(r.path), "passes": int(r.passes),
                     "zone_iters": int(r.zone_iters), "n_diff": int(r.n_diff), "maps": int(r.maps)}))
    return out


def calibrate_selection_penalty(scores, switch_costs, target_count: int,
                                max_iter: int = 60) -> Tuple[float, np.ndarray, float, int]:
    _native.load()
    if not _is_tensor(scores) and np.asarray(scores).shape[0] == 0:
        raise ValueError("`scores` cannot be empty")
    scores_t = _to_device_f64(scores)
    penalty, sol_t, value, count, _ = calibrate_selection_penalty_device(
        scores_t, switch_costs, target_count, max_iter=max_iter)
    return float(penalty), sol_t.cpu().numpy().astype(np.uint8, copy=False), float(value), int(count)


def solve_chrom_exact_device(scores_t, budget: Optional[float] = None, gamma: float = 1.0,
                             selection_penalty: Optional[float] = None):
    n = int(scores_t.shape[0])
    info: Dict[str, float] = {}
    if selection_penalty is None:
        if budget is None:
            penalty_ = 0.0
            sol_t, penalized, count, path = solve_penalized_chain_device(scores_t, float(gamma), penalty_)
            info = {"path": path}
        else:
            target_count = int(np.floor(n * float(budget)))
            penalty_, sol_t, penalized, count, info = calibrate_selection_penalty_device(
                scores_t, float(gamma), target_count)
    else:
        penalty_ = float(selection_penalty)
        sol_t, penalized, count, path = solve_penalized_chain_device(scores_t, float(gamma), penalty_)
        info = {"path": path}
    objective = objective_value(sol_t, scores_t, float(gamma))
    details = {
        "penalized_objective": float(penalized),
        "selected_count": int(count),
        "selected_fraction": float(count / n),
        "selection_penalty": float(penalty_),
    }
    details.update({f"_{k}": v for k, v in info.items()})
    return sol_t, float(objective), details


def solve_chrom_exact(scores, budget: Optional[float] = None, gamma: float = 1.0,
                      selection_penalty: Optional[float] = None, return_details: bool = False):
    _native.load()
    scores_t = _to_device_f64(scores)
    if scores_t.shape[0] == 0:
        raise ValueError("`scores` cannot be empty")
    sol_t, objective, details = solve_chrom_exact_device(scores_t, budget=budget, gamma=gamma,
                                                         selection_penalty=selection_penalty)
    solution = sol_t.cpu().numpy().astype(np.uint8, copy=False)
    if not return_details:
        return solution, objective
    public = {k: v for k, v in details.items() if not k.startswith("_")}
    return solution, objective, public
```

rocco_amd/pipeline.py:

```python
from __future__ import annotations

import concurrent.futures
import os
import threading
from typing import Dict, List, Optional, Sequence, Tuple

import numpy as np

from . import _native
from . import dp as _dp
from . import rocco as _rocco
from . import shard as _shard

SOLVE_GROUPS = int(os.environ.get("ROCCO_SOLVE_GROUPS", "1"))
SCORE_FIRST = int(os.environ.get("ROCCO_SCORE_FIRST", "0"))
MEDIAN_STATS = bool(int(os.environ.get("ROCCO_MEDIAN_STATS", "0")))
_pool: Optional[concurrent.futures.ThreadPoolExecutor] = None
_group_state: Dict[Tuple[int, int], tuple] = {}
_group_lock = threading.Lock()


def _group_resources(device_index: int, group: int):
    import torch

    key = (int(device_index), int(group))
    if key not in _group_state:
        _group_state[key] = (_native.Solver(int(device_index)), torch.cuda.Stream(device=int(device_index)))
    return _group_state[key]


class ChromWork:

    def __init__(self, name: str, matrix_t, budget: float, gamma: float, step: int = 50, start: int = 0,
                 scoring: str = "median", wls_params: Optional[dict] = None):
        if scoring not in ("median", "wls"):
            raise ValueError("scoring must be 'median' or 'wls'")
        self.name = name
        self.matrix_t = matrix_t
        self.budget = float(budget)
        self.gamma = float(gamma)
        self.step = int(step)
        self.start = int(start)
        self.n = int(matrix_t.shape[1])
        self.scoring = scoring
        self.wls_params = dict(wls_params or {})


def _score_wls(c: ChromWork):
    import torch

    from . import inference as _inference

    s_t, details = _inference.score_loci_wls_device(c.matrix_t.to(torch.float64), **c.wls_params)
    c._effect_mean = details["mean"]
    return s_t


def _solve_group(chroms: Sequence[ChromWork], scores: list, score_stats=None, units: Optional[Sequence[int]] = None) -> list:
    import torch

    if any(s is None for s in scores):
        score_stats = None
    scores = [s if s is not None else _score_wls(c) for c, s in zip(chroms, scores)]
    targets = [int(np.floor(c.n * c.budget)) for c in chroms]
    solved = _dp.calibrate_batch_device(scores, [c.gamma for c in chroms], targets, score_stats=score_stats)
    out = []
    units = list(range(len(chroms))) if units is None else [int(u) for u in units]
    tables, hosts, offsets = [], [], [0]
    for at in range(0, len(chroms), 48):
        part = solved[at:at + 48]
        selected = sum(int(count) for (_p, _s, _v, count, _i) in part)
        part_t, part_off, part_host = _rocco.decode_runs_table_device(
            [sol_t for (_p, sol_t, _v, _c, _i) in part], units=units[at:at + 48], capacity_rows=max(1024, selected // 2 + 64),
            eager_rows=max(4096, selected // 5))
        tables.append(part_t)
        hosts.append(part_host if len(chroms) <= 48 else part_host.copy())
        offsets += [offsets[-1] + o for o in part_off[1:]]
    table_t = tables[0] if len(tables) == 1 else torch.cat(tables, dim=0)
    host_rows = hosts[0] if len(hosts) == 1 else np.concatenate(hosts, axis=0)
    runs = [(table_t[offsets[i]:offsets[i + 1], 1], table_t[offsets[i]:offsets[i + 1], 2]) for i in range(len(chroms))]
    for i, (c, s_t, (penalty, sol_t, value, count, info), (begin_t, end_t)) in enumerate(zip(chroms, scores, solved, runs)):
        out.append({
            "name": c.name, "n": c.n, "selected_count": count, "selection_penalty": penalty,
            "penalized_objective": value, "path": info["path"], "info": info,
            "begin": begin_t, "end": end_t, "solution": sol_t, "step": c.step, "start": c.start,
            "effect_mean": getattr(c, "_effect_mean", None), "scores": s_t,
            "rows": table_t, "rows_host": host_rows, "row_range": (offsets[i], offsets[i + 1]),
        })
    return out


def _group_chunks(order: List[int], n_groups: int) -> List[List[int]]:
    k = len(order)
    base, extra = divmod(k, n_groups)
    out, at = [], 0
    for g in range(n_groups):
        size = base + (1 if g < extra else 0)
        out.append(order[at:at + size])
        at += size
    return [c for c in out if c]


def solve_rank(chroms: Sequence[ChromWork], scores_out: Optional[list] = None, groups: Optional[int] = None,
               median_timing: Optional[list] = None, units: Optional[Sequence[int]] = None):
    import torch

    global _pool
    if len(chroms) == 0:
        return []
    device = chroms[0].matrix_t.device
    n_groups = max(1, min(int(groups if groups is not None else SOLVE_GROUPS), len(chroms), _native.max_side_streams()))
    out: List[Optional[dict]] = [None] * len(chroms)
    units = list(range(len(chroms))) if units is None else [int(u) for u in units]

    def score_all(members: Sequence[ChromWork]):
        med = [c for c in members if c.scoring != "wls"]
        if median_timing is not None and med:
            ev0, ev1 = torch.cuda.Event(enable_timing=True), torch.cuda.Event(enable_timing=True)
            ev0.record(torch.cuda.current_stream(device))
        outs, stats_d = [], None
        if med and MEDIAN_STATS:
            outs, stats_d = _rocco.score_central_tendency_chrom_batch_device([c.matrix_t for c in med], with_stats=True)
        elif med:
            outs = _rocco.score_central_tendency_chrom_batch_device([c.matrix_t for c in med])
        got = dict(zip((id(c) for c in med), outs))
        if median_timing is not None and med:
            ev1.record(torch.cuda.current_stream(device))
            nbytes = sum((c.matrix_t.element_size() * int(c.matrix_t.shape[0]) + 8) * c.n for c in med)
            median_timing.append((ev0, ev1, nbytes))
        stats_h = None
        if stats_d is not None and len(med) == len(members):
            stats_h = torch.empty((len(med), 3), dtype=torch.float64, pin_memory=True)
            stats_h.copy_(stats_d, non_blocking=True)
        for c in med:
            c._effect_mean = got[id(c)]
        return [got.get(id(c)) for c in members], stats_h

    if n_groups == 1:
        scores, stats_h = score_all(chroms)
        if stats_h is not None:
            torch.cuda.current_stream(device).synchronize()
        out = _solve_group(chroms, scores, stats_h, units)
    else:
        order = sorted(range(len(chroms)), key=lambda i: -chroms[i].n)
        members = _group_chunks(order, n_groups)
        with torch.cuda.device(device):
            caller_stream = torch.cuda.current_stream(device)

            def work(group: int, idx: List[int], scores: list, scored, stats_h=None, stats_rows=None):
                solver, stream = _group_resources(device.index, group)
                with torch.cuda.device(device), torch.cuda.stream(stream), _native.use_solver(solver):
                    if stats_h is not None:
                        scored.synchronize()
                        if stats_rows is not None:
                            stats_h = stats_h[stats_rows]
                    else:
                        stream.wait_event(scored)
                    res = _solve_group([chroms[i] for i in idx], scores, stats_h, [units[i] for i in idx])
                    stream.synchronize()
                    kept = None if not res or res[0]["rows_host"] is None else res[0]["rows_host"].copy()
                    for r in res:
                        r["rows_host"] = kept
                for r in res:
                    for key in ("begin", "end", "solution", "scores", "effect_mean", "rows"):
                        t = r.get(key)
                        if t is not None and hasattr(t, "record_stream"):
                            t.record_stream(caller_stream)
                return idx, res

            with _group_lock:
                if _pool is None:
                    _pool = concurrent.futures.ThreadPoolExecutor(max_workers=max(1, _native.max_side_streams()),
                                                                  thread_name_prefix="rocco-solve")
                futures = []
                if SCORE_FIRST:
                    every, stats_all = score_all([chroms[i] for i in order])
                    by_index = dict(zip(order, every))
                    row = {i: k for k, i in enumerate(order)}
                    scored = torch.cuda.Event()
                    scored.record(caller_stream)
                    for g, idx in enumerate(members):
                        rows = [row[i] for i in idx] if stats_all is not None else None
                        futures.append(_pool.submit(work, g, idx, [by_index[i] for i in idx], scored, stats_all, rows))
                else:
                    for g, idx in enumerate(members):
                        scores, stats_h = score_all([chroms[i] for i in idx])
                        scored = torch.cuda.Event()
                        scored.record(caller_stream)
                        futures.append(_pool.submit(work, g, idx, scores, scored, stats_h))
                first_error = None
                for f in futures:
                    try:
                        idx, res = f.result()
                        for i, r in zip(idx, res):
                            out[i] = r
                    except BaseException as exc:
                        if first_error is None:
                            first_error = exc
                if first_error is not None:
                    raise first_error
    if scores_out is not None:
        scores_out.extend(r["scores"] for r in out)
    return out


def interval_rows(results: Sequence[dict], host: bool = True):
    import torch

    tables, seen = [], set()
    for r in results:
        t = r["rows_host"] if host else r["rows"]
        if id(t) not in seen:
            seen.add(id(t))
            tables.append(t)
    if len(tables) == 1:
        return tables[0]
    if host:
        return np.concatenate(tables, axis=0) if tables else np.zeros((0, 3), dtype=np.int64)
    return torch.cat(tables, dim=0)


def runs_to_records(result: dict, min_length_bp: Optional[int] = None) -> List[Tuple[str, int, int]]:
    b = result["begin"].cpu().numpy()
    e = result["end"].cpu().numpy()
    step, start = result["step"], result["start"]
    recs = []
    for bi, ei in zip(b.tolist(), e.tolist()):
        s_bp, e_bp = start + bi * step, start + ei * step
        if min_length_bp is None or (e_bp - s_bp) >= int(min_length_bp):
            recs.append((result["name"], int(s_bp), int(e_bp)))
    return recs


def summit_offsets(result: dict, min_length_bp: Optional[int] = None) -> List[Tuple[str, int]]:
    import torch

    records = runs_to_records(result, min_length_bp=min_length_bp)
    if not records:
        return []
    dev = result["begin"].device
    n, step, start = result["n"], result["step"], result["start"]
    intervals_t = start + step * torch.arange(n, dtype=torch.int64, device=dev)
    starts_t = torch.tensor([r[1] for r in records], dtype=torch.int64, device=dev)
    ends_t = torch.tensor([r[2] for r in records], dtype=torch.int64, device=dev)
    mean_t = result["effect_mean"].to(torch.float64).contiguous()
    off = _rocco.narrowpeak_summit_offsets_device(intervals_t, mean_t, starts_t, ends_t).cpu().numpy().tolist()
    return [(f"{c}_{s}_{e}", int(o)) for (c, s, e), o in zip(records, off)]
```

Baseline: 5.693 billion.

## Keep per-row score statistics on device and feed them directly to chain search

Score statistics (min, max, abs-sum) computed during median scoring now stay in device memory and pass through a new device-stats batch entry point into the chain search kernel. This removes the pinned host copy, the stream synchronization before solving, and the redundant stats recompute kernel in the chain path. A fallback copies the stats to the host if chain search does not run or the stats look invalid. Separately, the wave-level min/max/sum reductions use DPP row operations plus readlane instead of shuffle loops.

After: 5.610 billion. 1.5% lower.

```diff
diff --git a/include/rocco_hip.h b/include/rocco_hip.h
--- a/include/rocco_hip.h
+++ b/include/rocco_hip.h
@@ -99,6 +99,10 @@
 int rocco_hip_solve_budget_batch_stats_f64(rocco_hip_solver *solver, size_t n_tasks,
                                            const rocco_hip_budget_task *tasks, const double *score_stats_host,
                                            rocco_hip_budget_result *results, void *stream);
+
+int rocco_hip_solve_budget_batch_device_stats_f64(rocco_hip_solver *solver, size_t n_tasks,
+                                                  const rocco_hip_budget_task *tasks, const double *score_stats_dev,
+                                                  rocco_hip_budget_result *results, void *stream);
 
 typedef struct {
     long long count;
@@ -246,6 +250,7 @@
 long long rocco_hip_solver_device_bytes(const rocco_hip_solver *solver);
 void rocco_hip_model_chain_counters(long long out[4]);
 void rocco_hip_model_chain_written_counters(long long out[2]);
+void rocco_hip_statistics_counters(long long out[3]);
 
 int rocco_hip_pcg64_standard_normal_f64(rocco_hip_solver *solver, unsigned long long state_hi, unsigned long long state_lo,
                                         unsigned long long inc_hi, unsigned long long inc_lo, size_t count, double *values_dev,
diff --git a/rocco_amd/_native.py b/rocco_amd/_native.py
--- a/rocco_amd/_native.py
+++ b/rocco_amd/_native.py
@@ -116,6 +116,9 @@
      [ctypes.c_void_p, ctypes.c_size_t, ctypes.POINTER(BudgetTask), ctypes.POINTER(BudgetResult),
       ctypes.c_void_p]),
     ("rocco_hip_solve_budget_batch_stats_f64", ctypes.c_int,
+     [ctypes.c_void_p, ctypes.c_size_t, ctypes.POINTER(BudgetTask), ctypes.c_void_p, ctypes.POINTER(BudgetResult),
+      ctypes.c_void_p]),
+    ("rocco_hip_solve_budget_batch_device_stats_f64", ctypes.c_int,
      [ctypes.c_void_p, ctypes.c_size_t, ctypes.POINTER(BudgetTask), ctypes.c_void_p, ctypes.POINTER(BudgetResult),
       ctypes.c_void_p]),
     ("rocco_hip_delta_model_lean_f64", ctypes.c_int,
@@ -241,6 +244,7 @@
     ("rocco_hip_whittaker_seam_repairs", ctypes.c_longlong, []),
     ("rocco_hip_model_chain_counters", None, [ctypes.POINTER(ctypes.c_longlong)]),
     ("rocco_hip_model_chain_written_counters", None, [ctypes.POINTER(ctypes.c_longlong)]),
+    ("rocco_hip_statistics_counters", None, [ctypes.POINTER(ctypes.c_longlong)]),
     ("rocco_hip_solver_device_bytes", ctypes.c_longlong, [ctypes.c_void_p]),
     ("rocco_hip_pcg64_standard_normal_f64", ctypes.c_int,
      [ctypes.c_void_p, ctypes.c_ulonglong, ctypes.c_ulonglong, ctypes.c_ulonglong, ctypes.c_ulonglong, ctypes.c_size_t,
diff --git a/rocco_amd/csrc/api.hip b/rocco_amd/csrc/api.hip
--- a/rocco_amd/csrc/api.hip
+++ b/rocco_amd/csrc/api.hip
@@ -384,6 +384,22 @@
     return solve_budget_batch(solver, n_tasks, tasks, results, (hipStream_t)stream, score_stats_host);
 }
 
+int rocco_hip_solve_budget_batch_device_stats_f64(rocco_hip_solver *solver, size_t n_tasks, const rocco_hip_budget_task *tasks,
+                                                  const double *score_stats_dev, rocco_hip_budget_result *results, void *stream)
+{
+    if (solver == nullptr || (n_tasks > 0 && (tasks == nullptr || results == nullptr))) {
+        return ROCCO_HIP_EINVAL;
+    }
+    for (size_t t = 0; t < n_tasks; ++t) {
+        if (tasks[t].scores_dev == nullptr || tasks[t].n == 0 || tasks[t].n >= ((size_t)1 << 31) ||
+            tasks[t].solution_dev == nullptr || tasks[t].max_iter < 0) {
+            return ROCCO_HIP_EINVAL;
+        }
+    }
+    ROCCO_HIP_TRY(hipSetDevice(solver->device)); (void)hipGetLastError();
+    return solve_budget_batch(solver, n_tasks, tasks, results, (hipStream_t)stream, nullptr, score_stats_dev);
+}
+
 int rocco_hip_delta_model_lean_f64(rocco_hip_solver *solver, const double *scores_dev, double gamma, size_t n,
                                    const uint8_t *emap_dev, const double *lambdas, size_t n_lambdas, long long *counts_out,
                                    long long *open_out, void *stream)
@@ -1049,6 +1065,13 @@
     }
 }
 
+void rocco_hip_statistics_counters(long long out[3])
+{
+    if (out != nullptr) {
+        rocco::statistics_counters(out);
+    }
+}
+
 void rocco_hip_model_chain_written_counters(long long out[2])
 {
     if (out != nullptr) {
diff --git a/rocco_amd/csrc/budget.h b/rocco_amd/csrc/budget.h
--- a/rocco_amd/csrc/budget.h
+++ b/rocco_amd/csrc/budget.h
@@ -10,7 +10,8 @@
                         hipStream_t stream);
 
 int solve_budget_batch(rocco_hip_solver *solver, size_t n_tasks, const rocco_hip_budget_task *tasks,
-                       rocco_hip_budget_result *results, hipStream_t stream, const double *score_stats_host = nullptr);
+                       rocco_hip_budget_result *results, hipStream_t stream, const double *score_stats_host = nullptr,
+                       const double *score_stats_dev = nullptr);
 
 }
 
@@ -44,5 +45,6 @@
 
 void model_chain_counters(long long out[4]);
 void model_chain_written_counters(long long out[2]);
+void statistics_counters(long long out[3]);
 
 }
diff --git a/rocco_amd/csrc/budget.hip b/rocco_amd/csrc/budget.hip
--- a/rocco_amd/csrc/budget.hip
+++ b/rocco_amd/csrc/budget.hip
@@ -105,6 +105,7 @@
 }
 
 std::atomic<long long> g_model_chain_counters[6];
+std::atomic<long long> g_statistics_counters[3];
 
 class HipEvaluator : public Evaluator {
 public:
@@ -2032,6 +2033,7 @@
         ROCCO_HIP_TRY(hipMemcpyAsync(dv, h, bytes_tasks + bytes_map, hipMemcpyHostToDevice, stream_));
         double *d_part = (double *)(dv + bytes_tasks + bytes_map);
         double *d_out = (double *)(dv + bytes_tasks + bytes_map + bytes_part);
+        g_statistics_counters[0].fetch_add(1, std::memory_order_relaxed);
         if ((rc = launch_stats((const StatsTask *)dv, (int)B, (const int2 *)(dv + bytes_tasks), (int)nbt, d_part,
                                d_out, stream_)) != ROCCO_HIP_OK) {
             return rc;
@@ -2042,9 +2044,25 @@
         return ROCCO_HIP_OK;
     }
 
+    int fetch_stats(const double *stats_dev, std::vector<double> &out)
+    {
+        const size_t B = probs.size();
+        out.assign(3 * B, 0.0);
+        if (B == 0) {
+            return ROCCO_HIP_OK;
+        }
+        int rc;
+        if ((rc = solver_->host_back.reserve(B * 3 * sizeof(double))) != ROCCO_HIP_OK) return rc;
+        g_statistics_counters[2].fetch_add(1, std::memory_order_relaxed);
+        ROCCO_HIP_TRY(hipMemcpyAsync(solver_->host_back.ptr, stats_dev, B * 3 * sizeof(double), hipMemcpyDeviceToHost, stream_));
+        ROCCO_HIP_TRY(hipStreamSynchronize(stream_));
+        std::memcpy(out.data(), solver_->host_back.ptr, B * 3 * sizeof(double));
+        return ROCCO_HIP_OK;
+    }
+
     int chain_rounds_run = 0;
     int chain_search(const std::vector<ChainProblem> &problems, const SearchOptions &opt, std::vector<double> &stats_out,
-                     std::vector<Presearch> &pre, bool &ran)
+                     std::vector<Presearch> &pre, bool &ran, const double *stats_dev = nullptr, bool *stats_unusable = nullptr)
     {
         ran = false;
         const double tc0 = now_us();
@@ -2100,7 +2118,7 @@
         const int R = std::max(1, env_int("ROCCO_HIP_CHAIN_ROUNDS", 12));
 
         std::vector<int2> blockmap;
-        for (size_t b = 0; b < B; ++b) {
+        for (size_t b = 0; stats_dev == nullptr && b < B; ++b) {
             const int nb = (int)((probs[b].n + kFastBlockLoci - 1) / kFastBlockLoci);
             for (int k = 0; k < nb; ++k) {
                 blockmap.push_back(make_int2((int)b, k));
@@ -2151,9 +2169,14 @@
         }
         std::memcpy(h + o_bmap, blockmap.data(), nbt * sizeof(int2));
         ROCCO_HIP_TRY(hipMemcpyAsync(dv, h, up_bytes, hipMemcpyHostToDevice, stream_));
-        if ((rc = launch_stats((const StatsTask *)(dv + o_stasks), (int)B, (const int2 *)(dv + o_bmap), (int)nbt, (double *)(dv + o_part),
-                               (double *)(dv + o_stats), stream_)) != ROCCO_HIP_OK) {
-            return rc;
+        if (stats_dev == nullptr) {
+            g_statistics_counters[0].fetch_add(1, std::memory_order_relaxed);
+            if ((rc = launch_stats((const StatsTask *)(dv + o_stasks), (int)B, (const int2 *)(dv + o_bmap), (int)nbt,
+                                   (double *)(dv + o_part), (double *)(dv + o_stats), stream_)) != ROCCO_HIP_OK) {
+                return rc;
+            }
+        } else {
+            g_statistics_counters[1].fetch_add(1, std::memory_order_relaxed);
         }
 
         const long long rec_cap = 8 * (tiles0 + (long long)tune.wgs) + 64 * (long long)B;
@@ -2167,7 +2190,8 @@
         A.hot = (ChainHot *)(dv + o_hot);
         A.pilot = (ChainPilot *)(dv + o_pilot);
         A.evals = (ChainEvals *)(dv + o_evals);
-        A.stats = (const double *)(dv + o_stats);
+        A.stats = (double *)(dv + o_stats);
+        A.stats_given = stats_dev;
         A.ctl = (LeanRoundCtl *)(dv + o_ctl);
         A.tasks = (LeanTask *)(dv + o_tasks);
         A.points = (double *)(dv + o_points);
@@ -2262,6 +2286,15 @@
         }
         stats_out.assign(hstats, hstats + 5 * B);
         pre.assign(B, Presearch());
+        for (size_t b = 0; stats_dev != nullptr && b < B; ++b) {
+            const double smin = hstats[5 * b + 0], smax = hstats[5 * b + 1], sabs_sum = hstats[5 * b + 4];
+            if (!std::isfinite(smin) || !std::isfinite(smax) || !(smin <= smax) || std::isnan(sabs_sum)) {
+                if (stats_unusable != nullptr) {
+                    *stats_unusable = true;
+                }
+                return ROCCO_HIP_OK;
+            }
+        }
         const bool debug = env_set("ROCCO_HIP_DEBUG");
         const bool chain_debug = env_set("ROCCO_HIP_CHAIN_DEBUG");
         bool grid_ok = true;
@@ -2892,6 +2925,13 @@
     }
 }
 
+void statistics_counters(long long out[3])
+{
+    for (int k = 0; k < 3; ++k) {
+        out[k] = g_statistics_counters[k].load(std::memory_order_relaxed);
+    }
+}
+
 void model_chain_written_counters(long long out[2])
 {
     out[0] = g_model_chain_counters[4].load(std::memory_order_relaxed);
@@ -3109,7 +3149,8 @@
 }
 
 int solve_budget_batch(rocco_hip_solver *solver, size_t n_tasks, const rocco_hip_budget_task *tasks,
-                       rocco_hip_budget_result *results, hipStream_t stream, const double *score_stats_host)
+                       rocco_hip_budget_result *results, hipStream_t stream, const double *score_stats_host,
+                       const double *score_stats_dev)
 {
     HipEvaluator ev(solver, stream);
     std::vector<ChainProblem> problems(n_tasks);
@@ -3159,8 +3200,29 @@
     std::vector<double> chain_stats;
     std::vector<Presearch> presearch;
     bool chained = false;
+    std::vector<double> stats_fetched;
+    if (score_stats_host != nullptr) {
+        score_stats_dev = nullptr;
+    }
+    for (size_t t = 0; score_stats_dev != nullptr && t < n_tasks; ++t) {
+        if (ev.probs[t].costs != nullptr) {
+            score_stats_dev = nullptr;
+        }
+    }
     if (score_stats_host == nullptr) {
-        if ((rc = ev.chain_search(problems, opt, chain_stats, presearch, chained)) != ROCCO_HIP_OK) return rc;
+        bool stats_unusable = false;
+        if ((rc = ev.chain_search(problems, opt, chain_stats, presearch, chained, score_stats_dev, &stats_unusable)) != ROCCO_HIP_OK) return rc;
+        if (score_stats_dev != nullptr && (!chained || stats_unusable)) {
+            chained = false;
+            if ((rc = ev.fetch_stats(score_stats_dev, stats_fetched)) != ROCCO_HIP_OK) return rc;
+            for (size_t t = 0; t < n_tasks; ++t) {
+                if (!(stats_fetched[3 * t] <= stats_fetched[3 * t + 1])) {
+                    set_last_error("score statistics in device memory: a row's minimum is not <= its maximum");
+                    return ROCCO_HIP_EINVAL;
+                }
+            }
+            score_stats_host = stats_fetched.data();
+        }
     }
     const double tp0 = HipEvaluator::now_us();
     ev.mark("threshold chain parsed");
diff --git a/rocco_amd/csrc/chain.h b/rocco_amd/csrc/chain.h
--- a/rocco_amd/csrc/chain.h
+++ b/rocco_amd/csrc/chain.h
@@ -116,7 +116,8 @@
     ChainHot *hot;
     ChainPilot *pilot;
     ChainEvals *evals;
-    const double *stats;
+    double *stats;
+    const double *stats_given = nullptr;
     LeanRoundCtl *ctl;
     LeanTask *tasks;
     double *points;
diff --git a/rocco_amd/csrc/chain.hip b/rocco_amd/csrc/chain.hip
--- a/rocco_amd/csrc/chain.hip
+++ b/rocco_amd/csrc/chain.hip
@@ -50,7 +50,21 @@
 __device__ void init_problem(const ChainArgs &A, int b, ChainHot &H)
 {
     const ChainInput in = A.inputs[b];
-    const double smin = A.stats[5 * b + 0], smax = A.stats[5 * b + 1], sabs_sum = A.stats[5 * b + 4];
+    double smin, smax, sabs_sum;
+    if (A.stats_given != nullptr) {
+        smin = A.stats_given[3 * b + 0];
+        smax = A.stats_given[3 * b + 1];
+        sabs_sum = A.stats_given[3 * b + 2];
+        A.stats[5 * b + 0] = smin;
+        A.stats[5 * b + 1] = smax;
+        A.stats[5 * b + 2] = INFINITY;
+        A.stats[5 * b + 3] = -INFINITY;
+        A.stats[5 * b + 4] = sabs_sum;
+    } else {
+        smin = A.stats[5 * b + 0];
+        smax = A.stats[5 * b + 1];
+        sabs_sum = A.stats[5 * b + 4];
+    }
     H.scores = in.scores;
     H.n = in.n;
     H.gamma = in.gamma;
@@ -98,7 +112,8 @@
     }
     const double c = in.gamma;
     const double sabs = fmax(fabs(smin), fabs(smax));
-    if (!(c >= 1.0e-3) || !(c <= 1.0e6) || !isfinite(smin) || !isfinite(smax) || !(smax - smin <= 1.0e9) || !(sabs <= 1.0e12)) {
+    if (!(c >= 1.0e-3) || !(c <= 1.0e6) || !isfinite(smin) || !isfinite(smax) || !(smin <= smax) || !(smax - smin <= 1.0e9) ||
+        !(sabs <= 1.0e12)) {
         return;
     }
     const double lambda = smin - 1.0;
diff --git a/rocco_amd/csrc/median.hip b/rocco_amd/csrc/median.hip
--- a/rocco_amd/csrc/median.hip
+++ b/rocco_amd/csrc/median.hip
@@ -10,6 +10,39 @@
 namespace rocco {
 
 namespace {
+
+template <int CTRL>
+__device__ __forceinline__ double dpp_f64(double x)
+{
+    const long long bits = __double_as_longlong(x);
+    const int lo = __builtin_amdgcn_update_dpp(0, (int)(bits & 0xFFFFFFFFLL), CTRL, 0xF, 0xF, false);
+    const int hi = __builtin_amdgcn_update_dpp(0, (int)(bits >> 32), CTRL, 0xF, 0xF, false);
+    return __longlong_as_double(((long long)hi << 32) | (unsigned int)lo);
+}
+
+__device__ __forceinline__ double read_lane_f64(double x, int src)
+{
+    const long long bits = __double_as_longlong(x);
+    const int lo = __builtin_amdgcn_readlane((int)(bits & 0xFFFFFFFFLL), src);
+    const int hi = __builtin_amdgcn_readlane((int)(bits >> 32), src);
+    return __longlong_as_double(((long long)hi << 32) | (unsigned int)lo);
+}
+
+__device__ __forceinline__ void wave_stats_reduce(double &mn, double &mx, double &ab)
+{
+#define ROCCO_STATS_STEP(CTRL)                \
+    mn = fmin(mn, dpp_f64<CTRL>(mn));         \
+    mx = fmax(mx, dpp_f64<CTRL>(mx));         \
+    ab += dpp_f64<CTRL>(ab);
+    ROCCO_STATS_STEP(0xB1)
+    ROCCO_STATS_STEP(0x4E)
+    ROCCO_STATS_STEP(0x141)
+    ROCCO_STATS_STEP(0x140)
+#undef ROCCO_STATS_STEP
+    mn = fmin(fmin(read_lane_f64(mn, 0), read_lane_f64(mn, 16)), fmin(read_lane_f64(mn, 32), read_lane_f64(mn, 48)));
+    mx = fmax(fmax(read_lane_f64(mx, 0), read_lane_f64(mx, 16)), fmax(read_lane_f64(mx, 32), read_lane_f64(mx, 48)));
+    ab = (read_lane_f64(ab, 0) + read_lane_f64(ab, 16)) + (read_lane_f64(ab, 32) + read_lane_f64(ab, 48));
+}
 
 template <typename T, int KP, bool EXACT>
 __device__ __forceinline__ double median_column(const T *__restrict__ m, int K_runtime, long long n, long long stride,
@@ -96,12 +129,7 @@
         const bool nan = valid && is_nan_bits(r);
         const double inf = std::numeric_limits<double>::infinity();
         double mn = (valid && !nan) ? r : inf, mx = (valid && !nan) ? r : -inf, ab = (valid && !nan) ? fabs(r) : 0.0;
-#pragma unroll
-        for (int off = 32; off > 0; off >>= 1) {
-            mn = fmin(mn, __shfl_xor(mn, off));
-            mx = fmax(mx, __shfl_xor(mx, off));
-            ab += __shfl_xor(ab, off);
-        }
+        wave_stats_reduce(mn, mx, ab);
         const bool any_nan = __ballot(nan) != 0ull;
         if ((threadIdx.x & 63) == 0) {
             double *p = task.partials + 3LL * (4LL * (logical - task.block_begin) + (threadIdx.x >> 6));
@@ -124,12 +152,7 @@
 __device__ __forceinline__ void stats_block_reduce(double mn, double mx, double ab, bool nan, double *__restrict__ out)
 {
     __shared__ double red[4][3];
-#pragma unroll
-    for (int off = 32; off > 0; off >>= 1) {
-        mn = fmin(mn, __shfl_xor(mn, off));
-        mx = fmax(mx, __shfl_xor(mx, off));
-        ab += __shfl_xor(ab, off);
-    }
+    wave_stats_reduce(mn, mx, ab);
     const bool any_nan = __syncthreads_or(nan ? 1 : 0) != 0;
     const int lane = threadIdx.x & 63, wave = threadIdx.x >> 6;
     if (lane == 0) {
@@ -189,12 +212,7 @@
     const bool nan = valid && is_nan_bits(r);
     const double inf = std::numeric_limits<double>::infinity();
     double mn = (valid && !nan) ? r : inf, mx = (valid && !nan) ? r : -inf, ab = (valid && !nan) ? fabs(r) : 0.0;
-#pragma unroll
-    for (int off = 32; off > 0; off >>= 1) {
-        mn = fmin(mn, __shfl_xor(mn, off));
-        mx = fmax(mx, __shfl_xor(mx, off));
-        ab += __shfl_xor(ab, off);
-    }
+    wave_stats_reduce(mn, mx, ab);
     const bool any_nan = __ballot(nan) != 0ull;
     if ((threadIdx.x & 63) == 0) {
         double *p = partials + 3LL * (4LL * blockIdx.x + (threadIdx.x >> 6));
diff --git a/rocco_amd/dp.py b/rocco_amd/dp.py
--- a/rocco_amd/dp.py
+++ b/rocco_amd/dp.py
@@ -266,7 +266,18 @@
         tasks[i].max_iter = steps[i]
         tasks[i].solution_dev = sol_t.data_ptr()
     solver = _native.solver_for(device.index)
-    if score_stats is not None:
+    if score_stats is not None and _is_tensor(score_stats) and score_stats.is_cuda:
+        if tuple(score_stats.shape) != (k, 3):
+            raise ValueError("`score_stats` must have shape [len(scores_list), 3]")
+        if score_stats.dtype != torch.float64:
+            raise ValueError("`score_stats` on the device must be float64")
+        if score_stats.device != device:
+            raise ValueError("`score_stats` must be on the scores' device (or on the host)")
+        stats_t = score_stats.contiguous()
+        _native.check(lib.rocco_hip_solve_budget_batch_device_stats_f64(solver.handle, k, tasks, stats_t.data_ptr(), results,
+                                                                        _stream_ptr(scores_list[0])),
+                      "rocco_hip_solve_budget_batch_device_stats_f64")
+    elif score_stats is not None:
         stats_h = np.ascontiguousarray(score_stats.numpy() if _is_tensor(score_stats) else score_stats, dtype=np.float64)
         if stats_h.shape != (k, 3):
             raise ValueError("`score_stats` must have shape [len(scores_list), 3]")
diff --git a/rocco_amd/pipeline.py b/rocco_amd/pipeline.py
--- a/rocco_amd/pipeline.py
+++ b/rocco_amd/pipeline.py
@@ -128,35 +128,28 @@
             ev1.record(torch.cuda.current_stream(device))
             nbytes = sum((c.matrix_t.element_size() * int(c.matrix_t.shape[0]) + 8) * c.n for c in med)
             median_timing.append((ev0, ev1, nbytes))
-        stats_h = None
-        if stats_d is not None and len(med) == len(members):
-            stats_h = torch.empty((len(med), 3), dtype=torch.float64, pin_memory=True)
-            stats_h.copy_(stats_d, non_blocking=True)
+        if len(med) != len(members):
+            stats_d = None
         for c in med:
             c._effect_mean = got[id(c)]
-        return [got.get(id(c)) for c in members], stats_h
+        return [got.get(id(c)) for c in members], stats_d
 
     if n_groups == 1:
-        scores, stats_h = score_all(chroms)
-        if stats_h is not None:
-            torch.cuda.current_stream(device).synchronize()
-        out = _solve_group(chroms, scores, stats_h, units)
+        scores, stats_d = score_all(chroms)
+        out = _solve_group(chroms, scores, stats_d, units)
     else:
         order = sorted(range(len(chroms)), key=lambda i: -chroms[i].n)
         members = _group_chunks(order, n_groups)
         with torch.cuda.device(device):
             caller_stream = torch.cuda.current_stream(device)
 
-            def work(group: int, idx: List[int], scores: list, scored, stats_h=None, stats_rows=None):
+            def work(group: int, idx: List[int], scores: list, scored, stats_d=None, stats_rows=None):
                 solver, stream = _group_resources(device.index, group)
                 with torch.cuda.device(device), torch.cuda.stream(stream), _native.use_solver(solver):
-                    if stats_h is not None:
-                        scored.synchronize()
-                        if stats_rows is not None:
-                            stats_h = stats_h[stats_rows]
-                    else:
-                        stream.wait_event(scored)
-                    res = _solve_group([chroms[i] for i in idx], scores, stats_h, [units[i] for i in idx])
+                    stream.wait_event(scored)
+                    if stats_d is not None and stats_rows is not None:
+                        stats_d = stats_d.index_select(0, torch.tensor(stats_rows, dtype=torch.int64, device=device))
+                    res = _solve_group([chroms[i] for i in idx], scores, stats_d, [units[i] for i in idx])
                     stream.synchronize()
                     kept = None if not res or res[0]["rows_host"] is None else res[0]["rows_host"].copy()
                     for r in res:
@@ -184,10 +177,10 @@
                         futures.append(_pool.submit(work, g, idx, [by_index[i] for i in idx], scored, stats_all, rows))
                 else:
                     for g, idx in enumerate(members):
-                        scores, stats_h = score_all([chroms[i] for i in idx])
+                        scores, stats_d = score_all([chroms[i] for i in idx])
                         scored = torch.cuda.Event()
                         scored.record(caller_stream)
-                        futures.append(_pool.submit(work, g, idx, scores, scored, stats_h))
+                        futures.append(_pool.submit(work, g, idx, scores, scored, stats_d))
                 first_error = None
                 for f in futures:
                     try:
```
